# mpieva/network-aware-bwa

Hardware: AMD Instinct MI355X
Metric: aligned reads/s to GRCh38 (100 bp SE), FM-index search (bwa_cal_sa_reg_gap), bit-exact vs CPU (higher is better)
Workload: dtype u32

## Files before the change

include/nabwa.h:

```cpp
#ifndef NABWA_H
#define NABWA_H
#include <stdint.h>
#include <stddef.h>

#ifdef __cplusplus
extern "C" {
#endif

#define NABWA_OK        0
#define NABWA_ENODEV   -1
#define NABWA_EINVAL   -2
#define NABWA_EIO      -3
#define NABWA_ENOMEM   -4
#define NABWA_ECAP     -5
#define NABWA_EHITS    -6
#define NABWA_EDATA    -7

typedef struct {
	int s_mm, s_gapo, s_gape;
	int mode;
	int indel_end_skip, max_del_occ, max_entries;
	float fnr;
	int max_diff, max_gapo, max_gape;
	int max_seed_diff, seed_len;
	int n_threads;
	int max_top2;
	int trim_qual;
} nabwa_gap_opt_t;

#define NABWA_MODE_GAPE     0x01
#define NABWA_MODE_COMPREAD 0x02
#define NABWA_MODE_LOGGAP   0x04
#define NABWA_MODE_NONSTOP  0x10

typedef struct { uint32_t info; uint32_t k, l; int32_t score; } nabwa_aln1_t;

typedef struct nabwa_index nabwa_index_t;

const char *nabwa_last_error(void);
int nabwa_device_count(void);

void nabwa_gap_init_opt(nabwa_gap_opt_t *opt);
int nabwa_cal_maxdiff(int len, double err, double thres);

int nabwa_index_load(const char *prefix, int device, int with_sa, int with_pac, nabwa_index_t **out);

int nabwa_index_from_arrays(int device, int is_device, const uint32_t *bwt0, uint64_t n_words0,
							const uint32_t *bwt1, uint64_t n_words1, const uint32_t *sa0, uint64_t n_sa_words0,
							const uint32_t *sa1, uint64_t n_sa_words1, nabwa_index_t **out);
void nabwa_index_destroy(nabwa_index_t *ix);
uint32_t nabwa_index_seq_len(const nabwa_index_t *ix, int which);
uint64_t nabwa_index_device_bytes(const nabwa_index_t *ix);

int nabwa_cal_sa_reg_gap(nabwa_index_t *ix, const nabwa_gap_opt_t *opt, int n, const int64_t *off,
						 const uint8_t *seq, const uint8_t *rseq, int per_read,
						 int32_t *n_aln, nabwa_aln1_t *aln_out, int64_t aln_cap, int64_t *n_rows,
						 int32_t *max_entries);

typedef struct nabwa_batch nabwa_batch_t;
int nabwa_batch_create(nabwa_index_t *ix, const nabwa_gap_opt_t *opt, int n, const int64_t *off,
					   const uint8_t *seq, const uint8_t *rseq, int per_read, nabwa_batch_t **out);
int nabwa_batch_run(nabwa_batch_t *b);
int nabwa_batch_sync(nabwa_batch_t *b, int *n_second_pass);
float nabwa_batch_last_kernel_ms(nabwa_batch_t *b);
float nabwa_batch_last_width_ms(nabwa_batch_t *b);
float nabwa_batch_last_deep_ms(nabwa_batch_t *b);
int nabwa_batch_count_touches(nabwa_batch_t *b, uint64_t *n_bucket, uint64_t *n_bucket_width);
int nabwa_batch_fetch(nabwa_batch_t *b, int32_t *n_aln, nabwa_aln1_t *aln_out, int64_t aln_cap, int64_t *n_rows,
					  int32_t *max_entries);
int nabwa_batch_width_records(nabwa_batch_t *b, int first, int n, uint32_t *w_out, uint8_t *bid_out, uint8_t *seed_bid_out);
int nabwa_batch_checksum(nabwa_batch_t *b, uint64_t *sum, int64_t *n_rows);
typedef struct {
	int32_t n, min_len, max_len;
	int32_t deep_only;
	int32_t ns1, ns_wide;
	int32_t w_sync;
	int32_t trip_budget, trip_budget_hard;
	int32_t n_sync;
	int32_t hard_budget;
	int32_t cls[3];
	int32_t coop_lanes;
	int32_t lds_rd;
} nabwa_batch_config_t;
int nabwa_batch_config(nabwa_batch_t *b, nabwa_batch_config_t *out);
int nabwa_batch_sure0_stats(nabwa_batch_t *b, uint64_t out[4]);
int nabwa_batch_sure0_stats_ex(nabwa_batch_t *b, uint64_t out[8]);
int nabwa_batch_dedup_stats(nabwa_batch_t *b, uint64_t out[4]);
int nabwa_batch_dedup_stats_ex(nabwa_batch_t *b, uint64_t out[8]);
int nabwa_index_dedup_cache_stats(nabwa_index_t *ix, uint64_t out[8]);
int nabwa_index_dedup_cache_clear(nabwa_index_t *ix);
void nabwa_batch_destroy(nabwa_batch_t *b);

typedef struct { double avg, std, ap_prior; uint32_t low, high, high_bayesian; } nabwa_isize_t;
int nabwa_isize_infer(const uint16_t *hist, double ap_prior, int64_t L, nabwa_isize_t *out);
int nabwa_isize_bin(int kind, int mapq0, int mapq1, uint32_t pos0, int len0, uint32_t pos1, int len1);
typedef struct { uint32_t pos; int32_t strand, mapQ, seQ, len, full_len, n_mm, n_gapo, n_gape, score, extra_flag; } nabwa_pe_end_t;
int nabwa_pairing(nabwa_pe_end_t p[2], int n_hits, uint64_t *hits, const nabwa_aln1_t *rows0, const nabwa_aln1_t *rows1,
				  int max_isize, int s_mm, const nabwa_isize_t *ii);

typedef struct {
	char *name;
	uint8_t *seq, *rseq, *qual;
	uint32_t bits0, bits1;
	int32_t score, clip_len;
	int32_t n_aln; int32_t pad0;
	nabwa_aln1_t *aln;
	int32_t n_multi; int32_t pad1;
	void *multi;
	uint32_t sa, pos;
	uint64_t c1c2seq;
	int32_t n_cigar; int32_t pad2;
	uint16_t *cigar;
	int32_t tid;
	char bc[64];
	uint32_t lenbits;
	char *md;
	int32_t max_entries; int32_t pad3;
} nabwa_bwa_seq_t;

int nabwa_bwa_cal_sa_reg_gap(nabwa_index_t *ix, int n_seqs, nabwa_bwa_seq_t *seqs, const nabwa_gap_opt_t *opt);

int nabwa_encode_read(int full_len, const uint8_t *codes, const uint8_t *qual, int reverse, int trim_qual, int is_comp,
					  uint8_t *seq_out, uint8_t *rseq_out);

int nabwa_sa_lookup(nabwa_index_t *ix, int n, const uint8_t *which, const uint32_t *k, uint32_t *sa_out);

int nabwa_global_align(int device, int n, const int64_t *ref_off, const uint8_t *ref, const int64_t *qry_off,
					   const uint8_t *qry, int gap_open, int gap_ext, int gap_end, const int *matrix25, int band,
					   int32_t *score, int32_t *n_cigar, uint32_t *cigar32, int max_cigar);

void nabwa_dp_scratch_release(int device);

void nabwa_dp_form_counts(uint64_t *out, int n);

int nabwa_extend_align(int device, int n, const int64_t *ref_off, const uint8_t *ref, const int64_t *qry_off,
					   const uint8_t *qry, int gap_open, int gap_ext, const int *matrix25, int band, const int32_t *G0,
					   int32_t *score, int32_t *n_cigar, uint32_t *cigar32, int max_cigar);

int nabwa_local_align(int device, int n, const int64_t *ref_off, const uint8_t *ref, const int64_t *qry_off,
					  const uint8_t *qry, int gap_open, int gap_ext, const int *matrix25, int band, int thres,
					  int32_t *score, int32_t *coords, int32_t *subo, int32_t *n_cigar, uint32_t *cigar32, int max_cigar);

#define NABWA_MAX_CIGAR 64
#define NABWA_MAX_MD    512
#define NABWA_MAX_MULTI 16
typedef struct { uint32_t pos; int32_t gap, mm, strand, n_cigar; uint16_t cigar[NABWA_MAX_CIGAR]; } nabwa_multi_t;
typedef struct {
	int32_t type, strand, n_mm, n_gapo, n_gape, score;
	uint32_t sa, pos, c1, c2;
	int32_t mapQ, seQ, len, full_len, clip_len;
	int32_t n_cigar; uint16_t cigar[NABWA_MAX_CIGAR];
	int32_t nm; char md[NABWA_MAX_MD];
	int32_t n_multi; nabwa_multi_t multi[NABWA_MAX_MULTI];
	int32_t flag, seqid, nn; int64_t rpos; char xt;
} nabwa_se_t;

int nabwa_index_attach_reference(nabwa_index_t *ix, const char *prefix);
int nabwa_index_n_contigs(const nabwa_index_t *ix);
int nabwa_index_contig(const nabwa_index_t *ix, int i, char *name, int name_cap, int64_t *offset, int32_t *len);
int nabwa_index_reference_info(const nabwa_index_t *ix, int64_t *l_pac, uint32_t *seed);
int nabwa_index_set_reference(nabwa_index_t *ix, int64_t l_pac, uint32_t seed, int n_seqs, const char *const *names,
							  const int64_t *offsets, const int32_t *lens, int n_holes, const int64_t *hole_off,
							  const int32_t *hole_len, const char *hole_amb, const uint8_t *pac);

int nabwa_se_finish(nabwa_index_t *ix, const nabwa_gap_opt_t *opt, int n, const int64_t *off, const uint8_t *seq,
					const uint8_t *rseq, const int32_t *full_len, const int32_t *n_aln, const nabwa_aln1_t *aln,
					int n_occ, uint64_t *rng48, nabwa_se_t *out);

int nabwa_se_posn(nabwa_index_t *ix, const nabwa_gap_opt_t *opt, int n, const int64_t *off, const int32_t *full_len,
				  const int32_t *n_aln, const nabwa_aln1_t *aln, int n_occ, uint64_t *rng48, nabwa_se_t *out);
int nabwa_se_refine(nabwa_index_t *ix, int n, const int64_t *off, const uint8_t *seq, const uint8_t *rseq, nabwa_se_t *inout);
int nabwa_se_posn_v(nabwa_index_t *ix, const nabwa_gap_opt_t *opt, int n, const int64_t *off, const int32_t *full_len,
					const int32_t *n_aln, const nabwa_aln1_t *aln, const uint8_t *n_occ_v, uint64_t *rng48, nabwa_se_t *out);

int nabwa_refine_gapped_core(nabwa_index_t *ix, int which_ref, int is_end_correct, int n, const int64_t *qry_off, const uint8_t *qry,
                             const int32_t *ext, uint32_t *pos, int32_t *n_cigar, uint16_t *cigar, int max_cigar);
int nabwa_cal_md(nabwa_index_t *ix, int which_ref, int n, const int64_t *qry_off, const uint8_t *qry, const uint32_t *pos,
                 const int32_t *n_cigar, const uint16_t *cigar, int max_cigar, int32_t *nm, int64_t *md_off, char *md, int64_t md_cap);
void nabwa_finish_counts(uint64_t out[4]);

typedef struct {
	int32_t max_isize, force_isize, max_occ, max_occ_se, n_multi, N_multi, type, is_sw, is_preload;
	double ap_prior;
} nabwa_pe_opt_t;
void nabwa_pe_opt_default(nabwa_pe_opt_t *po);

typedef struct {
	nabwa_se_t se;
	int32_t extra_flag, m_seqid, am;
	int32_t mapQ_paired;
	int64_t m_rpos, isize;
} nabwa_pe_t;

int nabwa_pe_posn(nabwa_index_t *ix, const nabwa_gap_opt_t *opt, int n_pairs, const int64_t *off, const int32_t *full_len,
				  const int32_t *n_aln, const nabwa_aln1_t *aln, uint64_t *rng48, nabwa_pe_t *out);

int nabwa_isize_add_pairs(int n_pairs, const nabwa_pe_t *recs, uint16_t *hist);
int nabwa_pe_finish(nabwa_index_t *ix, const nabwa_gap_opt_t *opt, const nabwa_pe_opt_t *popt, const nabwa_isize_t *ii,
					int n_pairs, const int64_t *off, const uint8_t *seq, const uint8_t *rseq, const int32_t *n_aln,
					const nabwa_aln1_t *aln, nabwa_pe_t *inout, uint64_t n_tot[2], uint64_t n_mapped[2]);
typedef struct nabwa_poscache nabwa_poscache_t;
nabwa_poscache_t *nabwa_poscache_create(void);
void nabwa_poscache_destroy(nabwa_poscache_t *c);
int64_t nabwa_poscache_size(const nabwa_poscache_t *c);
int nabwa_pe_finish_cached(nabwa_index_t *ix, const nabwa_gap_opt_t *opt, const nabwa_pe_opt_t *popt, const nabwa_isize_t *ii,
						   int n_pairs, const int64_t *off, const uint8_t *seq, const uint8_t *rseq, const int32_t *n_aln,
						   const nabwa_aln1_t *aln, nabwa_pe_t *inout, uint64_t n_tot[2], uint64_t n_mapped[2], nabwa_poscache_t *cache);

int nabwa_bwa_posn_se(nabwa_index_t *ix, const nabwa_gap_opt_t *opt, int max_occ_se, int n, nabwa_bwa_seq_t *seqs, uint64_t *rng48);
int nabwa_bwa_refine_gapped(nabwa_index_t *ix, int n, nabwa_bwa_seq_t *seqs);
int nabwa_bwa_posn_pe(nabwa_index_t *ix, const nabwa_gap_opt_t *opt, int n_pairs, nabwa_bwa_seq_t *seqs, uint64_t *rng48);
int nabwa_bwa_finish_pe(nabwa_index_t *ix, const nabwa_gap_opt_t *opt, const nabwa_pe_opt_t *popt, const nabwa_isize_t *ii,
						int n_pairs, nabwa_bwa_seq_t *seqs, uint64_t n_tot[2], uint64_t n_mapped[2]);
int nabwa_bwa_finish_pe_cached(nabwa_index_t *ix, const nabwa_gap_opt_t *opt, const nabwa_pe_opt_t *popt, const nabwa_isize_t *ii,
							   int n_pairs, nabwa_bwa_seq_t *seqs, uint64_t n_tot[2], uint64_t n_mapped[2], nabwa_poscache_t *cache);

typedef struct nabwa_isize_table nabwa_isize_table_t;
typedef struct nabwa_bam_batch nabwa_bam_batch_t;
nabwa_isize_table_t *nabwa_isize_table_create(double ap_prior, int64_t genome_len);
void nabwa_isize_table_destroy(nabwa_isize_table_t *t);
int nabwa_isize_table_infer_all(nabwa_isize_table_t *t);
int nabwa_isize_table_get(const nabwa_isize_table_t *t, const char *rg, nabwa_isize_t *out);
int nabwa_isize_table_merge(nabwa_isize_table_t *t, const nabwa_isize_table_t *other);
int64_t nabwa_isize_table_encode(const nabwa_isize_table_t *t, uint8_t *out, int64_t cap);
int nabwa_isize_table_decode(nabwa_isize_table_t *t, const uint8_t *in, int64_t n);
int nabwa_bam_batch_create(nabwa_index_t *ix, const nabwa_gap_opt_t *opt, const nabwa_pe_opt_t *popt, int n_rec,
						   const uint8_t *in, const int64_t *in_off, nabwa_bam_batch_t **out);
#define NABWA_BAM_BROKEN_INPUT    1u
#define NABWA_BAM_DROP_ALIGNED    2u
#define NABWA_BAM_SKIP_DUPLICATES 4u
#define NABWA_BAM_DEBUG           8u
#define NABWA_BAM_ONLY_ALIGNED    16u
#define NABWA_BAM_ALL_FLAGS       31u
int nabwa_bam_batch_create_ex(nabwa_index_t *ix, const nabwa_gap_opt_t *opt, const nabwa_pe_opt_t *popt, uint32_t flags, int n_rec,
							  const uint8_t *in, const int64_t *in_off, nabwa_bam_batch_t **out);
int nabwa_bam_batch_search(nabwa_bam_batch_t *b);
int nabwa_bam_batch_pass1(nabwa_bam_batch_t *b, uint64_t *rng48, nabwa_isize_table_t *tab);
int nabwa_bam_batch_pass2(nabwa_bam_batch_t *b, const nabwa_isize_table_t *tab, uint64_t n_tot[2], uint64_t n_mapped[2]);
int nabwa_bam_batch_output(const nabwa_bam_batch_t *b, uint8_t *out, int64_t cap, int64_t *out_off, int64_t *n_bytes);
int nabwa_bam_batch_counts(const nabwa_bam_batch_t *b, int *n_records, int *n_logical);
int nabwa_bam_batch_kinds(const nabwa_bam_batch_t *b, uint8_t *kind_out);
void nabwa_bam_batch_destroy(nabwa_bam_batch_t *b);

#define NABWA_KIND_EOF 0
#define NABWA_KIND_SINGLE 1
#define NABWA_KIND_PAIR 2
#define NABWA_PHASE_PRISTINE 0
#define NABWA_PHASE_ALIGNED 1
#define NABWA_PHASE_POSITIONED 2
#define NABWA_PHASE_FINISHED 3
typedef struct {
	uint8_t core[32];
	int32_t data_len; const uint8_t *data;
	uint8_t strand, type, n_mm, n_gapo, n_gape, seQ, mapQ;
	int32_t len, clip_len, score; uint32_t sa, c1, c2, pos;
	int32_t n_multi; const uint8_t *multi;
	int32_t max_entries, n_aln; const uint8_t *aln;
} nabwa_wire_read_t;
typedef struct { uint64_t recno; uint8_t kind, phase; nabwa_wire_read_t read[2]; } nabwa_wire_rec_t;
int64_t nabwa_wire_size(const nabwa_wire_rec_t *r);
int64_t nabwa_wire_encode(const nabwa_wire_rec_t *r, uint8_t *out, int64_t cap);
int nabwa_wire_decode(const uint8_t *msg, int64_t len, nabwa_wire_rec_t *out);
void nabwa_wire_core_from_bam(const uint8_t bam_core[32], uint8_t wire_core[32]);
void nabwa_wire_core_to_bam(const uint8_t wire_core[32], uint8_t bam_core[32]);
int64_t nabwa_wire_config_encode(const nabwa_gap_opt_t *opt, const nabwa_pe_opt_t *popt, const char *prefix, uint8_t *out, int64_t cap);
int nabwa_wire_config_decode(const uint8_t *msg, int64_t len, nabwa_gap_opt_t *opt, nabwa_pe_opt_t *popt, char *prefix, int prefix_cap);

int nabwa_bam_batch_positioned(nabwa_bam_batch_t *b, nabwa_wire_read_t *out);
int nabwa_bam_batch_restore(nabwa_bam_batch_t *b, const nabwa_wire_read_t *in);

typedef struct nabwa_worker nabwa_worker_t;
int nabwa_worker_create(nabwa_index_t *ix, const nabwa_gap_opt_t *opt, const nabwa_pe_opt_t *popt, nabwa_worker_t **out);
void nabwa_worker_destroy(nabwa_worker_t *w);
int nabwa_worker_set_isize(nabwa_worker_t *w, const uint8_t *blob, int64_t n);
typedef int (*nabwa_send_fn)(void *ctx, const uint8_t *msg, int64_t len);
typedef int (*nabwa_recv_fn)(void *ctx, const uint8_t **msg, int64_t *len, int timeout_ms);
int nabwa_worker_process(nabwa_worker_t *w, int n_msg, const uint8_t *const *msgs, const int64_t *lens, nabwa_send_fn send, void *ctx);
typedef struct { int32_t max_batch, linger_ms, idle_timeout_ms; } nabwa_worker_opt_t;
int nabwa_worker_core(nabwa_worker_t *w, nabwa_recv_fn recv, nabwa_send_fn send, void *ctx, const nabwa_worker_opt_t *wo);
void nabwa_worker_counts(const nabwa_worker_t *w, uint64_t out[4]);

int nabwa_index_export(const nabwa_index_t *ix, int which, int what, uint64_t first, uint64_t n, uint32_t *out);

int nabwa_occ4(nabwa_index_t *ix, int which, int n, const uint32_t *k, uint32_t *cnt_out );

int64_t nabwa_index_fa2pac(const char *fasta, const char *prefix);
int64_t nabwa_index_fa2cspac(const char *fasta, const char *prefix);
int nabwa_index_build(const char *prefix, int device, int sa_intv, int verbose);
int nabwa_index_build_estimate(uint64_t l_pac, uint64_t *bytes);

#define NABWA_ISIZE_FEW   1
#define NABWA_ISIZE_WEIRD 2
int nabwa_isize_infer_pairs(int n_pairs, const uint32_t *pos, const int32_t *len, const int32_t *mapq, double ap_prior, int64_t L,
							nabwa_isize_t *out, char *log, int log_cap);
int nabwa_pe_finish_sampe(nabwa_index_t *ix, const nabwa_gap_opt_t *opt, const nabwa_pe_opt_t *popt, const nabwa_isize_t *ii,
						  int n_pairs, const int64_t *off, const uint8_t *seq, const uint8_t *rseq, const int32_t *n_aln,
						  const nabwa_aln1_t *aln, nabwa_pe_t *inout, nabwa_poscache_t *cache, int *cnt_chg, uint64_t n_tot[2],
						  uint64_t n_mapped[2]);
int nabwa_index_pac2real(const nabwa_index_t *ix, int64_t pos, int len, int *seqid);

#define NABWA_CS2NT_MAX 1024
int nabwa_cs2nt(int device, int n, const int64_t *off, const uint8_t *nt_ref, const uint8_t *cs_read, uint8_t *out);
int nabwa_index_attach_nt_reference(nabwa_index_t *ix, const char *prefix);
int nabwa_se_finish_cs(nabwa_index_t *ix, const nabwa_gap_opt_t *opt, int n, const int64_t *off, const uint8_t *seq, const uint8_t *rseq,
					   const uint8_t *qual, const int32_t *full_len, const int32_t *n_aln, const nabwa_aln1_t *aln, int n_occ,
					   uint64_t *rng48, nabwa_se_t *out, uint8_t *nt_seq, uint8_t *nt_rseq, uint8_t *nt_qual, double *times);
int nabwa_pe_finish_sampe_cs(nabwa_index_t *ix, const nabwa_gap_opt_t *opt, const nabwa_pe_opt_t *popt, const nabwa_isize_t *ii,
							 int n_pairs, const int64_t *off, const uint8_t *seq, const uint8_t *rseq, const uint8_t *qual,
							 const int32_t *n_aln, const nabwa_aln1_t *aln, nabwa_pe_t *inout, nabwa_poscache_t *cache, int *cnt_chg,
							 uint8_t *nt_seq, uint8_t *nt_rseq, uint8_t *nt_qual, double *times);
int nabwa_pairing_typed(nabwa_pe_end_t p[2], int n_hits, uint64_t *hits, const nabwa_aln1_t *rows0, const nabwa_aln1_t *rows1,
						int max_isize, int s_mm, const nabwa_isize_t *ii, int type);

typedef struct nabwa_bgzf nabwa_bgzf_t;
int nabwa_bgzf_inflated_size(const uint8_t *in, int64_t n, int64_t *n_out, int64_t *n_blocks);
int nabwa_bgzf_decompress(int device, const uint8_t *in, int64_t n, uint8_t *out, int64_t cap, int64_t *n_out, int64_t *n_blocks);
int nabwa_bgzf_handle_decompress(nabwa_bgzf_t *z, const uint8_t *in, int64_t n, uint8_t *out, int64_t cap, int64_t *n_out, int64_t *n_blocks);
int64_t nabwa_bgzf_bound(int64_t n);
int nabwa_bgzf_compress(int device, const uint8_t *in, int64_t n, uint8_t *out, int64_t cap, int64_t *n_out, int64_t *n_blocks);
int nabwa_bgzf_create(int device, nabwa_bgzf_t **out);
int nabwa_bgzf_handle_compress(nabwa_bgzf_t *z, const uint8_t *in, int64_t n, uint8_t *out, int64_t cap, int64_t *n_out, int64_t *n_blocks);
void nabwa_bgzf_destroy(nabwa_bgzf_t *z);
#define NABWA_BGZF_CODES_FIXED    0
#define NABWA_BGZF_CODES_DYNAMIC  1
int nabwa_bgzf_compress_ex(int device, int codes, const uint8_t *in, int64_t n, uint8_t *out, int64_t cap, int64_t *n_out, int64_t *n_blocks);
int nabwa_bgzf_handle_compress_ex(nabwa_bgzf_t *z, int codes, const uint8_t *in, int64_t n, uint8_t *out, int64_t cap, int64_t *n_out, int64_t *n_blocks);

#define NABWA_BAM_SORT_KEY(tid, pos) (((uint64_t)(uint32_t)(tid) << 32) | (uint32_t)((pos) + 1))
typedef struct nabwa_bam_sort nabwa_bam_sort_t;
int nabwa_bam_sort_create(int device, nabwa_bam_sort_t **out);
void nabwa_bam_sort_destroy(nabwa_bam_sort_t *s);
int nabwa_bam_sort_run(nabwa_bam_sort_t *s, int64_t n_rec, const uint8_t *in, const int64_t *in_off, uint8_t *out, int64_t cap, int64_t *out_off, uint64_t *keys_out);
int nabwa_bam_sort(int device, int64_t n_rec, const uint8_t *in, const int64_t *in_off, uint8_t *out, int64_t cap, int64_t *out_off, uint64_t *keys_out);
int nabwa_bam_sort_times(const nabwa_bam_sort_t *s, float ms[6]);

#define NABWA_DAMAGE_LEN_BINS 1024
#define NABWA_DAMAGE_MAX_POS  256
enum { NABWA_DAMAGE_STAT_SEEN = 0, NABWA_DAMAGE_STAT_COUNTED, NABWA_DAMAGE_STAT_SKIPPED_FLAGS, NABWA_DAMAGE_STAT_SKIPPED_PLACE,
	   NABWA_DAMAGE_STAT_SKIPPED_MAPQ, NABWA_DAMAGE_STAT_SKIPPED_EMPTY, NABWA_DAMAGE_STAT_COLUMNS_COUNTED,
	   NABWA_DAMAGE_STAT_COLUMNS_SKIPPED_READ, NABWA_DAMAGE_STAT_COLUMNS_SKIPPED_REF, NABWA_DAMAGE_N_STATS };
typedef struct { int32_t n_pos; int32_t min_mapq; uint32_t exclude_flags; uint32_t require_flags; int32_t which_ref; int32_t pad; } nabwa_damage_opt_t;
typedef struct nabwa_damage nabwa_damage_t;
void nabwa_damage_default_opt(nabwa_damage_opt_t *o);
int nabwa_damage_create(nabwa_index_t *ix, const nabwa_damage_opt_t *opt, nabwa_damage_t **out);
int nabwa_damage_add(nabwa_damage_t *d, int64_t n_rec, const uint8_t *in, const int64_t *in_off);
int nabwa_damage_fetch(nabwa_damage_t *d, uint64_t *sub5, uint64_t *sub3, uint64_t *len_hist, uint64_t *stats);
int nabwa_damage_clear(nabwa_damage_t *d);
void nabwa_damage_destroy(nabwa_damage_t *d);
int nabwa_damage_times(const nabwa_damage_t *d, float ms[3]);

int nabwa_bam_sort_run_ex(nabwa_bam_sort_t *s, int64_t n_rec, const uint8_t *in, const int64_t *in_off, uint8_t *out, int64_t cap, int64_t *out_off, uint64_t *keys_out, uint32_t *perm_out);
int nabwa_bam_sort_ex(int device, int64_t n_rec, const uint8_t *in, const int64_t *in_off, uint8_t *out, int64_t cap, int64_t *out_off, uint64_t *keys_out, uint32_t *perm_out);

#define NABWA_MARKDUP_ENDS_5P   0
#define NABWA_MARKDUP_ENDS_BOTH 1
enum { NABWA_MARKDUP_STAT_SEEN = 0, NABWA_MARKDUP_STAT_SKIPPED_FLAGS, NABWA_MARKDUP_STAT_ALREADY, NABWA_MARKDUP_STAT_UNMAPPED,
	   NABWA_MARKDUP_STAT_FRAGMENTS, NABWA_MARKDUP_STAT_PAIRS, NABWA_MARKDUP_STAT_ORPHANS, NABWA_MARKDUP_STAT_DUP_FRAGMENTS,
	   NABWA_MARKDUP_STAT_DUP_PAIRS, NABWA_MARKDUP_STAT_DUP_RECORDS, NABWA_MARKDUP_N_STATS };
typedef struct { int32_t min_qual; int32_t single_ends; uint32_t exclude_flags; int32_t pad; } nabwa_markdup_opt_t;
typedef struct nabwa_markdup nabwa_markdup_t;
void nabwa_markdup_default_opt(nabwa_markdup_opt_t *o);
int nabwa_markdup_create(int device, const nabwa_markdup_opt_t *opt, nabwa_markdup_t **out);
int nabwa_markdup_add(nabwa_markdup_t *m, int64_t n_rec, const uint8_t *in, const int64_t *in_off);
int nabwa_markdup_resolve(nabwa_markdup_t *m, uint8_t *dup, int64_t cap, uint64_t *stats);
int nabwa_markdup_clear(nabwa_markdup_t *m);
void nabwa_markdup_destroy(nabwa_markdup_t *m);
int nabwa_markdup_times(const nabwa_markdup_t *m, float ms[5]);

enum { NABWA_BAI_STAT_RECORDS = 0, NABWA_BAI_STAT_PLACED, NABWA_BAI_STAT_NO_COOR, NABWA_BAI_STAT_BINS, NABWA_BAI_STAT_CHUNKS, NABWA_BAI_STAT_WINDOWS,
	   NABWA_BAI_STAT_BYTES, NABWA_BAI_N_STATS };
typedef struct nabwa_bai nabwa_bai_t;
int nabwa_bai_create(int device, int32_t n_ref, nabwa_bai_t **out);
int nabwa_bai_add(nabwa_bai_t *b, int64_t n_rec, const uint8_t *in, const int64_t *in_off, int64_t stream_off);
int nabwa_bai_finish(nabwa_bai_t *b, int64_t n_blk, const int64_t *blk_uoff, const int64_t *blk_coff, uint8_t *out, int64_t cap, int64_t *n_out, uint64_t *stats);
int nabwa_bai_clear(nabwa_bai_t *b);
void nabwa_bai_destroy(nabwa_bai_t *b);
int nabwa_bai_times(const nabwa_bai_t *b, float ms[7]);
int nabwa_bgzf_block_table(const uint8_t *in, int64_t n, int64_t *blk_uoff, int64_t *blk_coff, int64_t cap, int64_t *n_blk);

#ifdef __cplusplus
}
#endif
#endif
```

network-aware-bwa_amd/csrc/fm_search.hip:

```cpp
#include "nabwa_dev.hpp"
#include "fm_search.hpp"
#include "launchers.hpp"

#define STATE_M 0
#define STATE_I 1
#define STATE_D 2
#define STATE_GROUP 3
#define GRP_EXT 0x100u
#define TXM 0xfffffffeu
#define KEYM 0xffffffffu
#define LVO(t_) ((size_t)((((uint64_t)1 << (2 * (t_))) - 4ull) / 3ull))
#ifndef NABWA_W_WAVES
#define NABWA_W_WAVES 5
#endif
#ifndef NABWA_WORK_CHUNK
#define NABWA_WORK_CHUNK 64u
#endif
#ifndef NABWA_RUN_MAX
#define NABWA_RUN_MAX 4
#endif

__device__ __forceinline__ uint32_t byte_of(uint64_t lo, uint64_t hi, uint32_t idx)
{
	asm volatile("" : "+v"(lo), "+v"(hi));
	const uint64_t h = (idx & 8u) ? hi : lo;
	return (uint32_t)(h >> ((idx & 7u) << 3)) & 0xffu;
}
#define WIN_SET(lo_, hi_, a_, b_, c_, d_) do { lo_ = (uint64_t)(b_) << 32 | (a_); hi_ = (uint64_t)(d_) << 32 | (c_); } while (0)

__device__ __forceinline__ void set_word(uint4 &q, uint32_t c, uint32_t v)
{
	q.x = c == 0 ? v : q.x; q.y = c == 1 ? v : q.y; q.z = c == 2 ? v : q.z; q.w = c == 3 ? v : q.w;
}

extern __shared__ uint16_t s_head[];

#ifndef NABWA_MIN_WAVES
#define NABWA_MIN_WAVES 4
#endif

template <bool COUNT>
__global__ __launch_bounds__(NABWA_SEARCH_BLOCK, NABWA_W_WAVES) void fm_width_kernel(const SearchParams P)
{
	const uint32_t lane = threadIdx.x & 63u;
	bool run = false, done = false;
	unsigned int w_next = 0, w_end = 0;
	uint32_t rid = 0, x = 0; int len = 0, phase = 0, wi = 0, n = 0, sbase = 0, nN = 0;
	uint32_t sq_off = 0;
#define WREC (P.wdata + (size_t)rid * P.wstride)
#define BX(f_) (x ? P.bwt[1].f_ : P.bwt[0].f_)
	bool tmode = false; uint32_t tp = 0, twtag = 0xffffffffu; uint2 twin = make_uint2(0u, 0u);
	const bool text_ok = (P.text_mode & 1) && P.bwt[0].sa_full && P.bwt[1].sa_full;
	uint32_t kk = 0, ll = 0, pw = 0; int bid = 0;
	uint32_t wkey = 0xffffffffu; bool tok = false; int tbase = 0;
	const int KT = (int)P.bwt[0].kmer_T, LW = (int)P.bwt[0].kmer_LW;
	__shared__ uint32_t s_pk[2 * NABWA_PK_LEVELS];
	const bool quads = (P.text_mode & TM_W_QUADS) && P.ixtab;
	if (threadIdx.x < 2 * NABWA_PK_LEVELS) s_pk[threadIdx.x] = quads ? P.ixtab[NABWA_IXTAB_WORDS + threadIdx.x] : 0xffffffffu;
	__syncthreads();
	bool nflag = true;
	auto rekey = [&](int from) {
		tok = false; tbase = from;
		if (nflag || from + 4 >= n) return;
		const int PW = P.pack_stride / 2;
		const uint32_t *const pk = P.rd_pack + (size_t)rid * P.pack_stride + x * PW;
		const int q = sbase + from;
		const uint32_t w0 = pk[q >> 4], w1 = pk[(q >> 4) + 1], sh = ((uint32_t)q & 15u) << 1;
		const uint32_t k16 = sh ? (w0 << sh) | (w1 >> (32u - sh)) : w0;
		wkey = k16 >> (2 * (16 - KT)); tok = true;
	};
	uint4 wacc = make_uint4(0, 0, 0, 0); uint64_t blo = 0, bhi = 0, slo = 0, shi = 0; int stag = -1;
	unsigned long long touches = 0;

	for (;;) {
		unsigned long long need = __ballot(!run && !done);
		if (P.w_sync && __ballot(run) != 0ull) need = 0ull;
		if (need) {
			if (w_next == w_end) {
				unsigned int base = 0;
				if (lane == 0) base = atomicAdd(P.work_counter + WC_WIDTH, (unsigned int)NABWA_WORK_CHUNK);
				w_next = __builtin_amdgcn_readfirstlane(base); w_end = w_next + NABWA_WORK_CHUNK;
			}
			const unsigned int rank = (unsigned int)__popcll(need & ((1ull << lane) - 1ull)), avail = w_end - w_next;
			const unsigned int base = w_next;
			w_next += min((unsigned int)__popcll(need), avail);
			if (!run && !done && rank < avail) {
				const unsigned int idx = base + rank;
				if (idx < 2u * (unsigned int)P.n) {
					rid = P.ids ? (uint32_t)P.ids[idx >> 1] : idx >> 1; x = idx & 1u;
					const int64_t o = P.poff[rid];
					len = P.rd_len[rid];
					sq_off = (uint32_t)o;
					nN = 0; stag = -1;
					if (P.w_skip_clean && P.n_aln[rid] == 0) {  }
					else if (len > 0) {
						run = true; phase = 0; wi = 0; n = len; sbase = 0; tmode = false;
						if (KT) { wkey = P.rd_key[6 * (size_t)rid + 2 + x]; tok = wkey != 0xffffffffu; }
						nflag = !KT || !P.rd_pack || P.rd_pack[(size_t)rid * P.pack_stride + (x + 1u) * (uint32_t)(P.pack_stride / 2) - 1u] != 0u;
						tbase = 0;
						kk = 0; ll = BX(seq_len); bid = 0; pw = 0; blo = bhi = 0;
					} else { if (x == 0u) P.rd_nN[rid] = 0; if (P.rd_cls) P.rd_cls[2 * (size_t)rid + x] = 0; }
				} else done = true;
			}
		}
		if (__ballot(!done) == 0ull) break;
		auto out_pos = [&](int p, bool last) {
			uint8_t *const rec = WREC;
			if (last) ++bid;
			const uint32_t wv = last ? 0u : ll - kk + 1u;
			const uint32_t bv = (uint32_t)(bid > 127 ? 127 : bid) | ((p > 0 && wv == pw) ? 128u : 0u);
			set_word(wacc, (uint32_t)p & 3u, wv);
			{ const uint64_t sh = (uint64_t)bv << (((uint32_t)p & 7u) << 3); if (p & 8) bhi |= sh; else blo |= sh; }
			pw = wv;
			if (phase == 0 && ((p & 3) == 3 || last)) *(uint4*)((uint32_t*)rec + x * P.WL + (p & ~3)) = wacc;
			if ((p & 15) == 15 || last) {
				*(uint4*)(rec + (phase ? P.woff_sbid + x * P.SLB : P.woff_bid + x * P.WLB) + (p & ~15)) =
					make_uint4((uint32_t)blo, (uint32_t)(blo >> 32), (uint32_t)bhi, (uint32_t)(bhi >> 32));
				blo = bhi = 0;
			}
		};
		bool bulk = run && phase == 0 && tmode && (wi & 15) == 0 && wi + 16 < n && tp >= 16u && pw == 1u;
		if (bulk) {
			if ((wi >> 4) != stag) { const uint4 q = *(const uint4*)((x ? P.rseq : P.seq) + sq_off + wi); WIN_SET(slo, shi, q.x, q.y, q.z, q.w); stag = wi >> 4; }
			const uint32_t w0 = (tp - 16u) >> 4;
			const uint32_t *const txt = BX(text);
			const uint32_t t0 = txt[w0], t1 = txt[w0 + 1u];
			auto squeeze = [](uint64_t v) -> uint32_t {
				uint64_t y = v & 0x0303030303030303ull;
				y = (y | y >> 6) & 0x000F000F000F000Full; y = (y | y >> 12) & 0x000000FF000000FFull; y = (y | y >> 24) & 0xFFFFull;
				return (uint32_t)y;
			};
			const bool clean = ((slo | shi) & 0xFCFCFCFCFCFCFCFCull) == 0ull;
			const uint32_t rd = squeeze(slo) | squeeze(shi) << 16;
			const uint32_t tx = (uint32_t)(((uint64_t)t1 << 32 | t0) >> (((tp - 16u) & 15u) << 1));
			uint32_t rv = __brev(tx); rv = (rv >> 1 & 0x55555555u) | (rv & 0x55555555u) << 1;
			bulk = clean && rv == rd;
			if (bulk) {
				uint8_t *const rec = WREC;
				uint32_t *const wp = (uint32_t*)rec + x * P.WL + wi;
#pragma unroll
				for (int u = 0; u < 4; ++u) *(uint4*)(wp + 4 * u) = make_uint4(1u, 1u, 1u, 1u);
				const uint32_t b4 = ((uint32_t)(bid > 127 ? 127 : bid) | 128u) * 0x01010101u;
				*(uint4*)(rec + P.woff_bid + x * P.WLB + wi) = make_uint4(b4, b4, b4, b4);
				tp -= 16u; wi += 16;
			}
		}
		if (bulk) {  }
		else if (run && tok && wi - tbase + 4 <= LW && wi + 4 < n) {
			uint2 tv[4];
			const uint2 *const lo = BX(kmer_lo);
			const int t1 = wi - tbase + 1;
			if (quads) {
				uint4 qd[2][2];
#pragma unroll
				for (int h = 0; h < 2; ++h) {
					const int t = t1 + 2 * h;
					const uint4 *const p = (const uint4*)(lo + LVO(t + 1) + 4 * (size_t)(wkey >> (2 * (KT - t))));
					qd[h][0] = p[0]; qd[h][1] = p[1];
				}
#pragma unroll
				for (int h = 0; h < 2; ++h) {
					const int t = t1 + 2 * h;
					const uint32_t ch = wkey >> (2 * (KT - t - 1)), c = ch & 3u;
					const uint4 a = qd[h][0], b = qd[h][1];
					const uint32_t sum = (a.y - a.x) + (a.w - a.z) + (b.y - b.x) + (b.w - b.z) + 4u + ((ch >> 2) == s_pk[x * NABWA_PK_LEVELS + t] ? 1u : 0u);
					tv[2 * h] = make_uint2(1u, sum);
					tv[2 * h + 1] = c == 0u ? make_uint2(a.x, a.y) : (c == 1u ? make_uint2(a.z, a.w) : (c == 2u ? make_uint2(b.x, b.y) : make_uint2(b.z, b.w)));
				}
			} else {
#pragma unroll
				for (int u = 0; u < 4; ++u) {
					const int t = t1 + u;
					tv[u] = (lo + LVO(t))[wkey >> (2 * (KT - t))];
				}
			}
#pragma unroll
			for (int u = 0; u < 4; ++u) {
				kk = tv[u].x; ll = tv[u].y;
				const bool dead = kk > ll;
				if (dead) { kk = 0; ll = BX(seq_len); ++bid; }
				out_pos(wi, false);
				++wi;
				if (dead) { rekey(wi); break; }
			}
		} else if (run) {
			const int pos = sbase + wi;
			if ((pos >> 4) != stag) { const uint4 q = *(const uint4*)((x ? P.rseq : P.seq) + sq_off + (pos & ~15)); WIN_SET(slo, shi, q.x, q.y, q.z, q.w); stag = pos >> 4; }
			const int cc = (int)byte_of(slo, shi, (uint32_t)pos & 15u);
			uint4 qa[4], qb[4]; uint32_t rk = 0, rl = 0, sav = 0; bool kval = false, two = false;
#pragma unroll
			for (int u = 0; u < 4; ++u) { qa[u] = make_uint4(0, 0, 0, 0); qb[u] = make_uint4(0, 0, 0, 0); }
			const bool q = cc < 4 && !tmode;
			if (q) {
				const uint32_t primary = BX(primary), kq = kk - 1u, lq = ll;
				const uint32_t kp = kq - (kq >= primary ? 1u : 0u), lp = lq - (lq >= primary ? 1u : 0u);
				const uint32_t bl = lp / NABWA_INTV; rl = lp - bl * NABWA_INTV;
				kval = kq != 0xffffffffu;
				const uint32_t bkk = kval ? kp / NABWA_INTV : bl; rk = kp - bkk * NABWA_INTV;
				two = bkk != bl;
				const uint4 *const bkt = BX(bk);
				const uint4 *pl = bkt + (size_t)bl * 4, *pk = bkt + (size_t)bkk * 4;
#pragma unroll
				for (int u = 0; u < 4; ++u) qa[u] = pl[u];
				if (two) {
#pragma unroll
					for (int u = 0; u < 4; ++u) qb[u] = pk[u];
				}
				if (COUNT) touches += ref_touches(x ? P.bwt[1] : P.bwt[0], kq, lq, false);
				if (text_ok && kk == ll) sav = BX(sa_full)[kk];
			}
			if (tmode && tp > 0u && ((tp - 1u) >> 5) != twtag) {
				twtag = (tp - 1u) >> 5;
				twin = *(const uint2*)(BX(text) + 2 * (size_t)twtag);
			}
			if (tmode) {
				bool ok = cc < 4 && tp > 0u;
				if (ok) {
					const uint32_t t = tp - 1u, wd = (t & 16u) ? twin.y : twin.x;
					ok = (wd >> ((t & 15u) << 1) & 3u) == (uint32_t)cc;
					if (ok) tp = t;
				}
				if (cc > 3 && x == 0u && phase == 0) ++nN;
				if (!ok) { tmode = false; kk = 0; ll = BX(seq_len); ++bid; rekey(wi + 1); }
			} else {
				const bool was_one = text_ok && cc < 4 && kk == ll;
				if (cc < 4) {
					Occ4 ck, cl;
					ck.c[0] = ck.c[1] = ck.c[2] = ck.c[3] = 0;
					cl = nabwa_count4(qa[0], qa[1], qa[2], qa[3], rl);
					if (kval) {
						const uint4 s0 = two ? qb[0] : qa[0], s1 = two ? qb[1] : qa[1], s2 = two ? qb[2] : qa[2], s3 = two ? qb[3] : qa[3];
						ck = nabwa_count4(s0, s1, s2, s3, rk);
					}
					const uint32_t L2c = cc == 0 ? BX(L2[0]) : (cc == 1 ? BX(L2[1]) : (cc == 2 ? BX(L2[2]) : BX(L2[3])));
					const uint32_t ok = cc == 0 ? ck.c[0] : (cc == 1 ? ck.c[1] : (cc == 2 ? ck.c[2] : ck.c[3]));
					const uint32_t ol = cc == 0 ? cl.c[0] : (cc == 1 ? cl.c[1] : (cc == 2 ? cl.c[2] : cl.c[3]));
					kk = L2c + ok + 1u; ll = L2c + ol;
				} else if (x == 0u && phase == 0) ++nN;
				if (kk > ll || cc > 3) { kk = 0; ll = BX(seq_len); ++bid; rekey(wi + 1); }
				else if (was_one) { tmode = true; tp = sav - 1u; twtag = 0xffffffffu; }
			}
			out_pos(wi, false);
			if (wi + 1 == n) out_pos(wi + 1, true);
			++wi;
			if (wi == n) {
				if (phase == 0 && P.rd_cls) P.rd_cls[2 * (size_t)rid + x] = (uint8_t)(bid - 1 > 4 ? 4 : bid - 1);
				if (phase == 0 && len > P.seed_len) {
					phase = 1; wi = 0; n = P.seed_len; sbase = len - P.seed_len; tmode = false;
					if (KT) { wkey = P.rd_key[6 * (size_t)rid + 4 + x]; tok = wkey != 0xffffffffu; }
					tbase = 0;
					kk = 0; ll = BX(seq_len); bid = 0; pw = 0;
				} else { if (x == 0u) P.rd_nN[rid] = (uint8_t)(nN > 255 ? 255 : nN); run = false; }
			}
		}
	}
	if (COUNT) {
		for (int o = 32; o > 0; o >>= 1) touches += __shfl_down(touches, o);
		if (lane == 0 && P.touch_counter) atomicAdd(P.touch_counter + TS_TOUCH_W, touches);
	}
#undef WREC
#undef BX
}
enum {
	LS_IDLE  = 0,
	LS_POP   = 1,
	LS_HAVE  = 2,
	LS_EXACT = 3,
	LS_EXIT  = 4
};
enum {
	TK_NONE      = 0,
	TK_EXPAND    = 1,
	TK_TAIL      = 2,
	TK_HIT       = 3,
	TK_JUMP      = 4,
	TK_GROUP     = 5,
	TK_ROWS      = 6,
	TK_TEXT_TAIL = 7
};

template <bool COUNT>
__global__ __launch_bounds__(NABWA_SEARCH_BLOCK, NABWA_MIN_WAVES) void fm_search_kernel(const SearchParams P_)
{
	SearchParams P = P_;
	own(P.n); own(P.s_mm); own(P.s_gapo); own(P.s_gape); own(P.mode); own(P.indel_end_skip); own(P.max_del_occ); own(P.max_entries);
	own(P.max_gape); own(P.max_seed_diff); own(P.seed_len); own(P.max_top2);
	const uint32_t NIL = 0xffffu;
	const uint32_t lane = threadIdx.x & 63u;
	const size_t slot = (size_t)blockIdx.x * NABWA_SEARCH_BLOCK + threadIdx.x;
	uint8_t *const sc = P.scratch + slot * P.lane_stride;
	uint4 *const ent = (uint4*)sc;
	const bool gape_mode = P.mode & 0x01, nonstop = P.mode & 0x10, loggap = P.mode & 0x04;

	int st = LS_IDLE;
	unsigned int w_next = 0, w_end = 0; bool w_sync = false;
	uint32_t item = 0; int len = 0; uint32_t mdmg = 0;
	uint32_t sq_off = 0;
	const int KT = (int)P.bwt[0].kmer_T;
	uint32_t budget = P.trip_budget;
	if (!COUNT && P.n_sync && P.trip_budget_hard && 2u * (uint32_t)__builtin_amdgcn_readfirstlane((int)*P.n_sync) > (uint32_t)P.n) budget = P.trip_budget_hard;
#define RID item
#define REC (P.wdata + (size_t)RID * P.wstride)
#define MD_READ ((int)(mdmg & 0xffu))
#define MG_READ ((int)(mdmg >> 8 & 0xfu))
	uint32_t k = 0, l = 0;
	int max_diff = 0, best_score = 0, best_cnt = 0, n_aln = 0, max_ent = 0, n_entries = 0;
	uint32_t bump = 0; uint64_t mask_lo = 0; bool seeded = false; int status = 0;
	int e_i = 0, e_a = 0, e_mm = 0, e_go = 0, e_ge = 0, e_state = 0, e_ldp = 0, e_score = 0, m = 0;
	uint4 pe = make_uint4(0, 0, 0, 0); int p_score = -1;
#define p_valid (p_score >= 0)
	int sq_tag = -1;
	int bw_base = -1, bw_a = -1;
	int sw_base = -1, sw_a = -1;
	unsigned long long touches = 0; uint32_t rd_touch = 0, rd_trips = 0;
	uint32_t rk_kf = 0, rk_row2 = 0, rk_row1 = 0, rk_tx = 0, rk_pop = 0, rk_tail = 0, rk_jump = 0, rk_gap = 0;
	unsigned long long st_trips = 0, st_expand = 0, st_exact = 0, st_ent = 0, st_spec = 0, st_query = 0, st_two = 0, st_exit = 0, st_jump = 0, st_txe = 0, st_txt = 0;
	bool ovf = false;
#define s0f mdmg
#define S0_ON  0x80000000u
#define S0_LAND 0x40000000u
#define S0_WAS 0x8000u
#define S0_PRV 0x1000u

	auto head_get = [&](int score) -> uint32_t {
		return (uint32_t)s_head[score * NABWA_SEARCH_BLOCK + threadIdx.x];
	};
	auto head_set = [&](int score, uint32_t v) {
		s_head[score * NABWA_SEARCH_BLOCK + threadIdx.x] = (uint16_t)v;
	};
	auto mask_has = [&](int score) -> bool { return mask_lo >> score & 1ull; };
	auto mask_set = [&](int score) { mask_lo |= 1ull << score; };
	auto mask_clr = [&](int score) { mask_lo &= ~(1ull << score); };
	auto mask_any = [&]() -> bool { return mask_lo != 0ull; };
	auto mask_first = [&]() -> int {
		return mask_lo ? __ffsll((unsigned long long)mask_lo) - 1 : 0x7fffffff;
	};
	auto never_popped = [&](int score) -> bool { return !nonstop && score > best_score + P.s_mm; };
	auto mk_entry = [&](uint32_t nk, uint32_t nl, int ni, int nldp, int nmm, int ngo, int nge, int nstate, int na) -> uint4 {
		const uint32_t z = (uint32_t)ni | (uint32_t)nldp << 16;
		return make_uint4(nk, nl, z, (uint32_t)nmm << 16 | (uint32_t)ngo << 20 | (uint32_t)nge << 24 | (uint32_t)nstate << 29 | (uint32_t)na << 31);
	};
	auto push_mem = [&](int score, uint4 e) {
		if (ovf || never_popped(score)) return;
		if ((uint32_t)score >= P.NS) { ovf = true; return; }
		if (bump >= P.cap) { ovf = true; return; }
		const uint32_t s = bump++;
		const uint32_t prev = mask_has(score) ? head_get(score) : NIL;
		e.w |= prev;
		ent[s] = e;
		head_set(score, s);
		mask_set(score);
	};

	uint4 *const s_pf = (uint4*)(s_head + (size_t)P.NS * NABWA_SEARCH_BLOCK);
	uint2 *const s_key = (uint2*)(s_pf + NABWA_SEARCH_BLOCK);
	uint2 *const s_tw = s_key + NABWA_SEARCH_BLOCK;
	uint32_t *const s_bw = (uint32_t*)(s_tw + NABWA_SEARCH_BLOCK), *const s_sw = s_bw + 4 * NABWA_SEARCH_BLOCK, *const s_sq = s_sw + 4 * NABWA_SEARCH_BLOCK;
	uint32_t *const s_fb = s_sq + 4 * NABWA_SEARCH_BLOCK;
	auto win_byte = [&](const uint32_t *W, uint32_t idx) -> uint32_t {
		return (uint32_t)((const uint8_t*)W)[(threadIdx.x << 4) + idx];
	};
	auto win_load = [&](const void *src, uint32_t *W) {
		__builtin_amdgcn_global_load_lds((const void __attribute__((address_space(1)))*)src,
										 (void __attribute__((address_space(3)))*)(W + ((threadIdx.x & ~63u) << 2)), 16, 0, 0);
	};
#define BW_BYTE(i_) win_byte(s_bw, (uint32_t)(i_))
#define SW_BYTE(i_) win_byte(s_sw, (uint32_t)(i_))
#define SQ_BYTE(i_) win_byte(s_sq, (uint32_t)(i_))
	const bool kf_ok = KT > 0 && (int)P.bwt[0].kmer_LW == KT && (int)P.bwt[1].kmer_LW == KT && (P.text_mode & 4);
	const bool text_ok = (P.text_mode & 2) && P.bwt[0].sa_full && P.bwt[1].sa_full && P.bwt[0].seq_len < 0xfffffff0u;
	uint32_t pf_slot = NIL;
	bool finish = false;
	auto unpack = [&](const uint4 &r) {
		k = r.x; l = r.y; e_i = (int)(r.z & 0xffffu); e_ldp = (int)(r.z >> 16);
		e_mm = (int)(r.w >> 16 & 15u); e_go = (int)(r.w >> 20 & 15u); e_ge = (int)(r.w >> 24 & 31u);
		e_state = (int)(r.w >> 29 & 3u); e_a = (int)(r.w >> 31);
	};
	auto take_entry = [&](const uint4 &r_ent) {
		unpack(r_ent);
		const uint32_t nx = r_ent.w & 0xffffu;
		head_set(e_score, nx);
		if (nx == NIL) mask_clr(e_score);
		--n_entries;
		if (!nonstop && e_score > best_score + P.s_mm) finish = true;
	};

	for (;;) {
		finish = false;
		unsigned long long need = __ballot(st == LS_IDLE);
		const bool any_busy = __ballot(st != LS_IDLE && st != LS_EXIT) != 0ull;
		if ((P.sync_refill || w_sync) && any_busy) need = 0ull;
		if (need) {
			if (w_next == w_end) {
				unsigned int b0 = 0;
				if (lane == 0) b0 = atomicAdd(P.work_counter + WC_SEARCH, (unsigned int)NABWA_WORK_CHUNK);
				w_next = __builtin_amdgcn_readfirstlane(b0); w_end = w_next + NABWA_WORK_CHUNK;
				w_sync = P.n_sync && (w_next >= *P.n_sync || w_next < P.n_sync[NCLS_SIZE + 2 - NCLS_FIRST0]);
			}
			const unsigned int rank = (unsigned int)__popcll(need & ((1ull << lane) - 1ull)), avail = w_end - w_next;
			const unsigned int base = w_next;
			w_next += min((unsigned int)__popcll(need), avail);
			if (st == LS_IDLE && rank < avail) {
				const unsigned int idx = base + rank;
				if (idx < (unsigned int)P.n) {
					const uint32_t rid = P.ids ? (uint32_t)P.ids[idx] : idx;
					item = rid;
					const int64_t o = P.poff[rid];
					len = P.rd_len[rid];
					sq_off = (uint32_t)o;
					mdmg = (uint32_t)P.rd_maxdiff[rid] | (uint32_t)P.rd_maxgapo[rid] << 8;
					if (KT) {
						s_key[threadIdx.x] = *(const uint2*)(P.rd_key + 6 * (size_t)rid);
						uint32_t fb = 0xffffu;
						if (len > KT) { const uint8_t *const bb = REC + P.woff_bid + (len - KT - 1); fb = (uint32_t)(bb[0] & 127u) | (uint32_t)(bb[P.WLB] & 127u) << 8; }
						s_fb[threadIdx.x] = fb;
					}
					n_aln = 0; max_ent = 0; status = NABWA_ST_OK; rd_touch = 0; rd_trips = 0; ovf = false;
					rk_kf = rk_row2 = rk_row1 = rk_tx = rk_pop = rk_tail = rk_jump = rk_gap = 0;
					sq_tag = -1; bw_a = -1; sw_a = -1; p_score = -1; pf_slot = NIL;
					if (text_ok) s_tw[threadIdx.x] = make_uint2(0u, 0x7fffffffu);
					if (!COUNT && P.sure0 && P.rd_cls && !nonstop && P.s_gapo > P.s_mm && MD_READ >= 1 && len > 0 && 2 + 4 * len <= P.max_entries) {
						const uint32_t cw = *(const uint16_t*)(P.rd_cls + 2 * (size_t)rid);
						if ((cw & 0xffu) == 0u || (cw >> 8) == 0u) {
							s0f |= P.sure0 > 1 ? S0_ON | S0_LAND | S0_WAS : S0_ON | S0_WAS;
							if (P.sure0 > 2) s0f |= ((cw & 0xffu) == 0u ? S0_PRV : 0u) | ((cw >> 8) == 0u ? S0_PRV << 1 : 0u);
						}
					}
					if (len > 0 && (int)P.rd_nN[rid] <= MD_READ) {
						seeded = len > P.seed_len;
						max_diff = MD_READ;
						best_score = (s0f & S0_ON) ? 0 : (MD_READ + 1) * P.s_mm + (MG_READ + 1) * P.s_gapo + (P.max_gape + 1) * P.s_gape;
						best_cnt = 0;
						bump = 0; mask_lo = 0ull;
						push_mem(0, mk_entry(0u, kf_ok ? KEYM : P.bwt[0].seq_len, len, 0, 0, 0, 0, STATE_M, 0));
						pe = mk_entry(0u, kf_ok ? KEYM : P.bwt[0].seq_len, len, 0, 0, 0, 0, STATE_M, 1); p_score = 0;
						n_entries = 2;
						st = LS_POP;
					} else { P.n_aln[item] = 0; P.max_ent[item] = 0; P.status[item] = NABWA_ST_OK; }
				} else st = LS_EXIT;
			}
		}
		if (__ballot(st != LS_EXIT) == 0ull) break;

		bool want_ent = false; uint32_t ent_slot = 0;
		bool have = st == LS_HAVE;
		if (st == LS_POP) {
			if (n_entries == 0) finish = true;
			else {
				if (max_ent < n_entries) max_ent = n_entries;
				if (n_entries > P.max_entries) finish = true;
				else if (!COUNT && P.trip_budget && rd_trips > budget) { status = NABWA_ST_OVERFLOW; finish = true; }
			}
			if (!finish) {
				const int best_mem = mask_first();
				if (p_valid && p_score <= best_mem) {
					unpack(pe);
					e_score = p_score; p_score = -1;
					--n_entries;
					if (!nonstop && e_score > best_score + P.s_mm) finish = true;
					else have = true;
				} else if (best_mem == 0x7fffffff) {
					finish = true;
				} else {
					if (p_valid) { push_mem(p_score, pe); p_score = -1; }
					if (ovf) { status = NABWA_ST_OVERFLOW; finish = true; }
					else {
						ent_slot = head_get(best_mem); e_score = best_mem;
						if (ent_slot == pf_slot) {
							const uint4 r = s_pf[threadIdx.x];
							take_entry(r);
							pf_slot = NIL;
							if (!finish) have = true;
						} else want_ent = true;
					}
				}
			}
		}
		int kind = TK_NONE;
		bool need_win = false, spec = false, forced = false; int win_hi = 0;
		int grp_c = 0, mlev = -1, mpost = 0; uint32_t midx = 0; bool kx = false;
		if (have && !finish && e_state == STATE_GROUP) {
			const uint32_t mk = (uint32_t)e_ldp & 0x1fu, ext = (uint32_t)e_ldp & GRP_EXT, more = (uint32_t)e_ldp >> 9;
			const int j = 31 - __clz((int)mk);
			const uint32_t rest = mk & ~(1u << j);
			if (rest) push_mem(e_score, mk_entry(k, l, e_i, (int)(rest | ext | more << 9), e_mm, e_go, e_ge, STATE_GROUP, e_a));
			else if (more) push_mem(e_score, mk_entry(k + 1u, l, e_i + 1, (int)(3u | (more - 1u) << 9), e_mm, e_go, e_ge, STATE_GROUP, e_a));
			if (ovf) { status = NABWA_ST_OVERFLOW; finish = true; }
			if (ext) ++e_ge; else ++e_go;
			if (l == KEYM) {
				const int dp = len - e_i - 1;
				kind = TK_ROWS; st = LS_POP; have = false;
				if (j == 0) { mpost = 1; mlev = dp; midx = k; } else { mpost = 2; mlev = dp + 1; midx = k * 4u + (uint32_t)(j - 1); }
			}
			else if (j == 0) { e_state = STATE_I; e_ldp = e_i; }
			else if (l == TXM) { k -= 1u; e_i += 1; e_state = STATE_D; e_ldp = e_i; }
			else { kind = TK_GROUP; grp_c = j - 1; st = LS_POP; have = false; }
		}
		if (have && !finish) {
			st = LS_POP;
			m = max_diff - (e_mm + e_go); if (gape_mode) m -= e_ge;
			if (m >= 0) {
				const bool kf = l == KEYM;
				const int d = len - e_i;
				if (e_i == 0) { if (kf) { kind = TK_ROWS; mlev = d; midx = k; } else kind = TK_HIT; }
				else {
					const bool tail = m == 0 && (e_state == STATE_M || gape_mode || e_ge == P.max_gape);
					const bool landed = e_state == STATE_M && e_ldp > e_i;
					win_hi = landed ? e_ldp - 1 : e_i - 1;
					const int win_lo = landed ? win_hi : ((tail || e_i < 2) ? e_i - 1 : e_i - 2);
					bool go = true;
					if (bw_a == e_a && win_lo >= bw_base && win_hi < bw_base + 16) {
						if (m < (int)(BW_BYTE(win_hi - bw_base) & 127u)) go = false;
					} else { need_win = true; spec = true; }
					if (go) {
						const bool rdkey_ok = KT && (e_a ? s_key[threadIdx.x].y : s_key[threadIdx.x].x) != 0xffffffffu;
						const bool row_known = l != TXM && !kf && (e_go | e_ge) == 0 && e_state == STATE_M && (e_mm == 0 || (e_mm == 1 && e_ldp == e_i));
						if (tail) {
							kind = TK_TAIL;
							if (l == TXM) kind = TK_TEXT_TAIL;
							else if (kf) { if (rdkey_ok) kind = TK_JUMP; else { kind = TK_ROWS; mlev = d; midx = k; } }
							else if (rdkey_ok && row_known && d <= KT) kind = TK_JUMP;
						}
						else {
							forced = rdkey_ok && d < KT && (kf || row_known) && (int)(s_fb[threadIdx.x] >> (e_a << 3) & 0xffu) == m;
							if (forced) kind = TK_JUMP;
							else if (kf && d >= KT) { kind = TK_ROWS; mlev = d; midx = k; }
							else if (l == TXM && (s0f & S0_ON) && (s0f & S0_PRV << e_a) && e_state == STATE_M && (e_mm | e_go | e_ge) == 0
									 && n_entries + 4 * len <= P.max_entries && k >= (uint32_t)e_i) {
								const int ies = P.indel_end_skip + (loggap ? 1 : 0);
								int hi = e_i - 1;
								if (hi > len - ies) hi = len - ies;
								if (seeded && P.max_seed_diff < 1 && hi > len - P.seed_len) hi = len - P.seed_len;
								const int gl = (MG_READ > 0 && hi >= ies) ? hi - ies + 1 : 0;
								if (P.s0_stats) { atomicAdd(P.s0_stats + S0S_LEAPS, 1ull); atomicAdd(P.s0_stats + S0S_LEAP_LEVELS, (unsigned long long)e_i); }
								n_entries += 2 * gl;
								if (max_ent < n_entries + 1) max_ent = n_entries + 1;
								k -= (uint32_t)e_i; e_i = 0; e_ldp = 0;
								kind = TK_HIT; need_win = false; spec = false;
							}
							else {
								if (P.s0_stats && l == TXM && (s0f & S0_ON) && (s0f & S0_PRV << e_a) && e_state == STATE_M && (e_mm | e_go | e_ge) == 0
									&& n_entries + 4 * len <= P.max_entries) atomicAdd(P.s0_stats + S0S_WALKED, 1ull);
								kind = TK_EXPAND; --e_i; kx = kf;
								if ((s0f & S0_ON) && n_entries + 4 * len > P.max_entries) s0f &= ~S0_ON;
							}
						}
					}
				}
			}
		} else if (st == LS_EXACT) kind = l == TXM ? TK_TEXT_TAIL : TK_TAIL;
		auto rows_arrived = [&](uint32_t nk, uint32_t nl) {
			k = nk; l = nl;
			if (mpost == 1) { e_state = STATE_I; e_ldp = e_i; }
			else if (mpost == 2) { e_i += 1; e_state = STATE_D; e_ldp = e_i; }
			st = LS_HAVE;
		};
		if (kind == TK_ROWS && mlev == 0) { rows_arrived(0u, e_a ? P.bwt[0].seq_len : P.bwt[1].seq_len); kind = TK_NONE; }

		const int qb = 1 - e_a;
		const bool tx = l == TXM && (kind == TK_EXPAND || kind == TK_HIT || kind == TK_TEXT_TAIL);
		const int spos = (kind == TK_TAIL || kind == TK_TEXT_TAIL) ? e_i - 1 : e_i;
		const int stag = (e_a << 20) | (spos >> 4);
		const bool need_seq = (kind == TK_EXPAND || kind == TK_TAIL || kind == TK_TEXT_TAIL) && stag != sq_tag;
		bool query = (kind == TK_EXPAND && !tx && !kx) || kind == TK_TAIL || kind == TK_GROUP;
		uint2 tw = make_uint2(0u, 0u); bool need_tw = false;
		if (tx && kind != TK_HIT && k > 0u) {
			const uint32_t tag = ((k - 1u) >> 4) | (uint32_t)qb << 31;
			tw = s_tw[threadIdx.x];
			need_tw = tw.y != tag;
			tw.y = tag;
		}
		const bool to_text = kind == TK_EXPAND && !tx && !kx && text_ok && k == l;
		if (kind == TK_TAIL && !need_seq && SQ_BYTE((uint32_t)spos & 15u) > 3u) query = false;
		const int ii = e_i - (len - P.seed_len);
		const bool use_seed = kind == TK_EXPAND && e_i > 0 && seeded && ii > 0;
		const bool need_seed = use_seed && !(sw_a == e_a && ii - 1 >= sw_base && ii < sw_base + 16);

		uint4 r_ent = make_uint4(0, 0, 0, 0);
		if (need_win) {
			int base = (win_hi | 7) - 15; if (base < 0) base = 0;
			win_load(REC + P.woff_bid + e_a * P.WLB + base, s_bw); bw_base = base; bw_a = e_a;
		}
		if (need_seq) {
			win_load((e_a ? P.rseq : P.seq) + sq_off + (spos & ~15), s_sq); sq_tag = stag;
		}
		if (need_seed) {
			int base = (ii | 7) - 15; if (base < 0) base = 0;
			win_load(REC + P.woff_sbid + e_a * P.SLB + base, s_sw); sw_base = base; sw_a = e_a;
		}
		uint32_t r_x = 0u;
		if (need_tw) r_x = (qb ? P.bwt[1].text : P.bwt[0].text)[(k - 1u) >> 4];
		else if (tx && kind == TK_HIT) r_x = (qb ? P.bwt[1].isa : P.bwt[0].isa)[k];
		else if (to_text) r_x = (qb ? P.bwt[1].sa_full : P.bwt[0].sa_full)[k];
		uint2 r_km = make_uint2(1u, 0u);
		uint4 a0, a1, a2, a3, b0, b1, b2, b3;
		a0 = a1 = a2 = a3 = b0 = b1 = b2 = b3 = make_uint4(0, 0, 0, 0);
		bool gh = kx && e_i > 0 && (s0f & S0_ON) && (e_mm | e_go | e_ge) == 0 && len - e_i < KT && !need_win && (BW_BYTE(e_i - 1 - bw_base) & 127u) == 0u;
		if (kind == TK_JUMP || gh) {
			uint32_t key = e_a ? s_key[threadIdx.x].y : s_key[threadIdx.x].x, key2 = 0, key3 = 0;
			const int d = len - e_i;
			if (gh) {
				if (key == 0xffffffffu) { gh = false; key = 0; }
				else {
					const uint32_t sh = 2u * (uint32_t)(KT - d), low = key & ((1u << sh) - 1u);
					const uint32_t gh_c = key >> sh & 3u;
					a3.x = 4u | gh_c;
					key = (k * 4u + ((gh_c + 1u) & 3u)) << sh | low; key2 = (k * 4u + ((gh_c + 2u) & 3u)) << sh | low; key3 = (k * 4u + ((gh_c + 3u) & 3u)) << sh | low;
				}
			} else if (l == KEYM) {
				if (d > 0) { const uint32_t sh = 2u * (uint32_t)(KT - d); key = (k << sh) | (sh ? key & ((1u << sh) - 1u) : 0u); }
			} else if (e_mm) {
				const uint32_t c1 = qb ? P.bwt[1].L2[1] : P.bwt[0].L2[1], c2 = qb ? P.bwt[1].L2[2] : P.bwt[0].L2[2], c3 = qb ? P.bwt[1].L2[3] : P.bwt[0].L2[3];
				const uint32_t cs = (k > c1 ? 1u : 0u) + (k > c2 ? 1u : 0u) + (k > c3 ? 1u : 0u);
				const uint32_t sh = 2u * (uint32_t)(KT - d);
				key = (key & ~(3u << sh)) | cs << sh;
			}
			const uint2 *const tab = qb ? P.bwt[1].kmer : P.bwt[0].kmer;
			r_km = tab[key];
			if (gh) { const uint2 g2 = tab[key2], g3 = tab[key3]; a2 = make_uint4(g2.x, g2.y, g3.x, g3.y); }
		}
		if (kind == TK_ROWS) r_km = ((qb ? P.bwt[1].kmer_lo : P.bwt[0].kmer_lo) + LVO(mlev))[midx];
		uint32_t rk = 0, rl = 0; bool kvalid = false, two = false;
		if (kx) {
			const uint4 *const ch = (const uint4*)((qb ? P.bwt[1].kmer_lo : P.bwt[0].kmer_lo) + LVO(len - e_i) + (size_t)k * 4);
			a0 = ch[0]; a1 = ch[1];
		}
		if (query) {
			const uint32_t primary = qb ? P.bwt[1].primary : P.bwt[0].primary;
			const uint4 *bk = qb ? P.bwt[1].bk : P.bwt[0].bk;
			const uint32_t kq = k - 1u, lq = l;
			const uint32_t kp = kq - (kq >= primary ? 1u : 0u), lp = lq - (lq >= primary ? 1u : 0u);
			const uint32_t bl = lp / NABWA_INTV; rl = lp - bl * NABWA_INTV;
			kvalid = kq != 0xffffffffu;
			const uint32_t bkk = kvalid ? kp / NABWA_INTV : bl; rk = kp - bkk * NABWA_INTV;
			two = bkk != bl;
			const uint4 *pl = bk + (size_t)bl * 4;
			a0 = pl[0]; a1 = pl[1]; a2 = pl[2]; a3 = pl[3];
			if (two) { const uint4 *pk = bk + (size_t)bkk * 4; b0 = pk[0]; b1 = pk[1]; b2 = pk[2]; b3 = pk[3]; }
		}

		bool pf_now = false; uint32_t pf_cand = NIL;
		if (want_ent) { pf_cand = ent_slot; pf_now = true; }
		else if ((kind == TK_TAIL || kind == TK_JUMP || kind == TK_TEXT_TAIL) && !p_valid && mask_any()) {
			const int bm = mask_first();
			pf_cand = head_get(bm);
			pf_now = pf_cand != pf_slot;
		}
		if (pf_now) r_ent = ent[pf_cand];
		if (!COUNT && P.trip_budget && st != LS_IDLE && st != LS_EXIT) ++rd_trips;
		if (COUNT && st != LS_IDLE && st != LS_EXIT) {
			++rd_trips;
			if (kind == TK_EXPAND) { if (kx) ++rk_kf; else if (tx) ++rk_tx; else if (two) ++rk_row2; else ++rk_row1; if (e_go | e_ge) ++rk_gap; }
			else if (want_ent) ++rk_pop; else if (kind == TK_TAIL || kind == TK_TEXT_TAIL) ++rk_tail; else if (kind == TK_JUMP) ++rk_jump;
		}
		if (COUNT) {
			const unsigned long long bx = __ballot(kind == TK_EXPAND), be = __ballot(kind == TK_TAIL), bm = __ballot(want_ent),
				bs = __ballot(spec), bq = __ballot(query), b2 = __ballot(query && two), bi = __ballot(st == LS_EXIT), bj = __ballot(kind == TK_JUMP), bt = __ballot(tx && kind == TK_EXPAND), b7 = __ballot(kind == TK_TEXT_TAIL);
			if (lane == 0) {
				st_trips += 1; st_expand += __popcll(bx); st_exact += __popcll(be); st_ent += __popcll(bm); st_spec += __popcll(bs);
				st_query += __popcll(bq); st_two += __popcll(b2); st_exit += __popcll(bi); st_jump += __popcll(bj); st_txe += __popcll(bt); st_txt += __popcll(b7);
			}
		}
		asm volatile("" ::: "memory");
		__builtin_amdgcn_s_waitcnt(0x0F70);
		if (pf_now) { s_pf[threadIdx.x] = r_ent; pf_slot = pf_cand; }
		if (spec && m < (int)(BW_BYTE(win_hi - bw_base) & 127u)) kind = TK_NONE;
		if (need_tw) { tw.x = r_x; s_tw[threadIdx.x] = tw; }
		int c = 4;
		if (kind == TK_EXPAND || kind == TK_TAIL) c = (int)SQ_BYTE((uint32_t)spos & 15u);
		if (kind == TK_TAIL && c > 3) query = false;
		Occ4 ck, cl;
		ck.c[0] = ck.c[1] = ck.c[2] = ck.c[3] = 0; cl = ck;
		if (query && kind != TK_NONE) {
			cl = nabwa_count4(a0, a1, a2, a3, rl);
			if (kvalid) {
				const uint4 s0 = two ? b0 : a0, s1 = two ? b1 : a1, s2 = two ? b2 : a2, s3 = two ? b3 : a3;
				ck = nabwa_count4(s0, s1, s2, s3, rk);
			}
			if (COUNT && kind != TK_GROUP) rd_touch += ref_touches(qb ? P.bwt[1] : P.bwt[0], k - 1u, l, kind == TK_EXPAND);
		}
		if (kx && kind == TK_EXPAND) {
			const uint32_t ek[4] = { a0.x, a0.z, a1.x, a1.z }, el[4] = { a0.y, a0.w, a1.y, a1.w };
#pragma unroll
			for (int j = 0; j < 4; ++j) { const bool ne = ek[j] <= el[j]; ck.c[j] = ne ? k * 4u + (uint32_t)j - 1u : 0u; cl.c[j] = ne ? KEYM : 0u; }
		}
		const bool tx1 = tx && kind == TK_EXPAND;
		if (tx1) {
			const uint32_t b = k > 0u ? (tw.x >> (((k - 1u) & 15u) << 1) & 3u) : 4u;
#pragma unroll
			for (int j = 0; j < 4; ++j) { ck.c[j] = b == (uint32_t)j ? k - 2u : 0u; cl.c[j] = b == (uint32_t)j ? TXM : 0u; }
		}
		const bool syn = tx1 || (kx && kind == TK_EXPAND);
		const uint32_t L2q0 = syn ? 0u : (qb ? P.bwt[1].L2[0] : P.bwt[0].L2[0]), L2q1 = syn ? 0u : (qb ? P.bwt[1].L2[1] : P.bwt[0].L2[1]);
		const uint32_t L2q2 = syn ? 0u : (qb ? P.bwt[1].L2[2] : P.bwt[0].L2[2]), L2q3 = syn ? 0u : (qb ? P.bwt[1].L2[3] : P.bwt[0].L2[3]);
		const uint32_t seqlen_q = qb ? P.bwt[1].seq_len : P.bwt[0].seq_len;
#define L2Q(cc) ((cc) == 0 ? L2q0 : ((cc) == 1 ? L2q1 : ((cc) == 2 ? L2q2 : L2q3)))
#define CK(cc) ((cc) == 0 ? ck.c[0] : ((cc) == 1 ? ck.c[1] : ((cc) == 2 ? ck.c[2] : ck.c[3])))
#define CL(cc) ((cc) == 0 ? cl.c[0] : ((cc) == 1 ? cl.c[1] : ((cc) == 2 ? cl.c[2] : cl.c[3])))

		if (kind == TK_ROWS) rows_arrived(r_km.x, r_km.y);
		else if (kind == TK_GROUP) {
			k = L2Q(grp_c) + CK(grp_c) + 1u; l = L2Q(grp_c) + CL(grp_c);
			e_i += 1; e_state = STATE_D; e_ldp = e_i;
			st = LS_HAVE;
		} else if (kind == TK_JUMP) {
			k = r_km.x; l = r_km.y;
			if (k > l) st = LS_POP;
			else if (forced) { e_i = len - KT; e_ldp = 0; st = LS_HAVE; }
			else { e_i = len - KT; st = LS_EXACT; }
		} else if (kind == TK_TEXT_TAIL) {
			uint32_t pp = k; bool fail = false;
			for (;;) {
				const uint32_t cc = SQ_BYTE((uint32_t)(e_i - 1) & 15u);
				if (cc > 3u || pp == 0u) { fail = true; break; }
				const uint32_t q = pp - 1u;
				if ((tw.x >> ((q & 15u) << 1) & 3u) != cc) { fail = true; break; }
				pp = q; --e_i;
				if (e_i == 0 || (e_i & 15) == 0 || (pp & 15u) == 0u) break;
			}
			k = pp;
			if (fail) st = LS_POP;
			else if (e_i == 0) st = LS_HAVE;
			else st = LS_EXACT;
		} else if (kind == TK_TAIL || kind == TK_HIT) {
			bool hit = false;
			if (kind == TK_HIT && tx) { k = r_x; l = r_x; }
			if (kind == TK_HIT) hit = true;
			else if (c > 3) st = LS_POP;
			else {
				k = L2Q(c) + CK(c) + 1u; l = L2Q(c) + CL(c);
				if (k > l) st = LS_POP;
				else if (--e_i == 0) hit = true;
				else st = LS_EXACT;
			}
			if (hit) {
				st = LS_POP;
				const int score = e_mm * P.s_mm + e_go * P.s_gapo + e_ge * P.s_gape;
				bool do_add = true;
				if (n_aln == 0) {
					if ((s0f & S0_ON) && score != 0) { status = NABWA_ST_OVERFLOW; finish = true; do_add = false; s0f &= ~S0_ON; if (P.s0_stats) atomicAdd(P.s0_stats + S0S_NET, 1ull); }
					best_score = score;
					const int best_diff = e_mm + e_go + (gape_mode ? e_ge : 0);
					if (!nonstop) max_diff = best_diff + 1 > MD_READ ? MD_READ : best_diff + 1;
				}
				if (score == best_score) best_cnt += (int)(l - k + 1u);
				else if (best_cnt > P.max_top2) { finish = true; do_add = false; }
				uint4 *const out = P.aln + (size_t)item * P.aln_cap;
				if (do_add && e_go) {
					for (int j = 0; j < n_aln; ++j) { const uint4 h = out[j]; if (h.y == k && h.z == l) { do_add = false; break; } }
				}
				if (do_add) {
					if (n_aln == P.aln_cap) { status = NABWA_ST_OVERFLOW; finish = true; }
					else {
						const uint32_t x = l - k + 1u, mx = seqlen_q; uint32_t jj = 0, pw = 0;
						uint8_t *const rec = REC;
						uint32_t *const wp = (uint32_t*)rec + e_a * P.WL; uint8_t *const bp = rec + P.woff_bid + e_a * P.WLB;
						for (int t0 = 0; t0 <= e_ldp && e_ldp > 0; t0 += 8) {
							const uint4 w0 = *(const uint4*)(wp + t0), w1 = *(const uint4*)(wp + t0 + 4);
							const uint2 bq = *(const uint2*)(bp + t0);
							uint32_t wv[8] = { w0.x, w0.y, w0.z, w0.w, w1.x, w1.y, w1.z, w1.w };
							uint32_t bb[2] = { bq.x, bq.y };
#pragma unroll
							for (int u = 0; u < 8; ++u) {
								const int t = t0 + u;
								uint32_t bv = bb[u >> 2] >> ((u & 3) * 8) & 0xffu;
								if (t < e_ldp) {
									if (wv[u] > x) wv[u] -= x;
									else if (wv[u] == x) { bv = (bv & 128u) | 1u; wv[u] = mx - (++jj); }
								}
								if (t <= e_ldp) {
									bv = (bv & 127u) | ((t > 0 && wv[u] == pw) ? 128u : 0u);
									bb[u >> 2] = (bb[u >> 2] & ~(0xffu << ((u & 3) * 8))) | bv << ((u & 3) * 8);
								}
								pw = wv[u];
							}
							*(uint4*)(wp + t0) = make_uint4(wv[0], wv[1], wv[2], wv[3]);
							*(uint4*)(wp + t0 + 4) = make_uint4(wv[4], wv[5], wv[6], wv[7]);
							*(uint2*)(bp + t0) = make_uint2(bb[0], bb[1]);
						}
						bw_a = -1;
						if (KT && e_ldp > len - KT - 1) s_fb[threadIdx.x] |= 0xffu << (e_a << 3);
						out[n_aln] = make_uint4((uint32_t)e_mm | (uint32_t)e_go << 8 | (uint32_t)e_ge << 16 | (uint32_t)e_a << 24,
												k, l, (uint32_t)score);
						++n_aln;
					}
				}
			}
		} else if (kind == TK_EXPAND) {
			const uint32_t occ = tx1 ? 1u : l - k + 1u;
			bool match_child = false;
			bool allow_diff = true, allow_M = true, mm_dead = false;
			if (e_i > 0) {
				const uint32_t B1 = BW_BYTE(e_i - 1 - bw_base), B0 = BW_BYTE(e_i - bw_base);
				const int b1 = (int)(B1 & 127u), b0v = (int)(B0 & 127u);
				mm_dead = (s0f & S0_ON) && b1 > 0;
				if (b1 > m - 1) allow_diff = false;
				else if (b1 == m - 1 && b0v == m - 1 && (B0 & 128u)) allow_M = false;
				if (use_seed) {
					const uint32_t S1 = SW_BYTE(ii - 1 - sw_base), S0 = SW_BYTE(ii - sw_base);
					const int s1 = (int)(S1 & 127u), s0 = (int)(S0 & 127u);
					const int m_seed = m - max_diff + P.max_seed_diff;
					if (s1 > m_seed - 1) allow_diff = false;
					else if (s1 == m_seed - 1 && s0 == m_seed - 1 && (S0 & 128u)) allow_M = false;
				}
			}
			auto emit = [&](int score, uint32_t nk, uint32_t nl, int ni, int nldp, int nmm, int ngo, int nge, int nstate, int count) {
				if (p_valid) push_mem(p_score, pe);
				pe = mk_entry(nk, nl, ni, nldp, nmm & 0xff, ngo & 0xff, nge & 0xff, nstate, e_a); p_score = score;
				n_entries += count;
			};
			const int sc0 = e_mm * P.s_mm + e_go * P.s_gapo + e_ge * P.s_gape;
			int tmp = e_go + e_ge;
			if (loggap) { const uint32_t v = (uint32_t)(e_ge + e_go); tmp = (v ? 31 - __clz((int)v) : 0) / 2 + 1; }
			bool ran = false;
			if (tx1 && e_state == STATE_M && n_entries + 64 <= P.max_entries) {
				const int ies = P.indel_end_skip + tmp, seed_lo = len - P.seed_len;
				const int m_seed = m - max_diff + P.max_seed_diff;
				int n = 0, icur = e_i, ilast = e_i; uint32_t pcur = k; bool grp_run = false;
				for (;;) {
					const uint32_t cc = SQ_BYTE((uint32_t)icur & 15u);
					if (cc > 3u || pcur == 0u) break;
					const uint32_t q = pcur - 1u;
					if ((tw.x >> ((q & 15u) << 1) & 3u) != cc) break;
					bool ad = true;
					const bool us = seeded && icur > 0 && icur - seed_lo > 0;
					if (icur > 0) {
						if ((int)(BW_BYTE(icur - 1 - bw_base) & 127u) > m - 1) ad = false;
						if (us && (int)(SW_BYTE(icur - seed_lo - 1 - sw_base) & 127u) > m_seed - 1) ad = false;
					}
					const bool g = ad && icur >= ies && len - icur >= ies && e_go < MG_READ;
					if (n == 0) grp_run = g; else if (g != grp_run) break;
					++n; pcur = q; ilast = icur;
					if (n == NABWA_RUN_MAX || icur == 0) break;
					if (m < (int)(BW_BYTE(icur - 1 - bw_base) & 127u)) break;
					if ((icur & 15) == 0 || (q & 15u) == 0u) break;
					if (icur - 1 > 0 && icur - 2 < bw_base) break;
					if (seeded && icur - 1 > 0 && icur - 1 - seed_lo > 0 && icur - 1 - seed_lo - 1 < sw_base) break;
					--icur;
				}
				if (n) {
					ran = true;
					if (grp_run) emit(sc0 + P.s_gapo, k - (uint32_t)(n - 1), TXM, ilast, (int)(3u | (uint32_t)(n - 1) << 9), e_mm, e_go, e_ge, STATE_GROUP, 2 * n);
					emit(sc0, pcur, TXM, ilast, 0, e_mm, e_go, e_ge, STATE_M, 1);
				}
			}
			if (ran) {  }
			else if (allow_diff && e_i >= P.indel_end_skip + tmp && len - e_i >= P.indel_end_skip + tmp) {
				uint32_t dm = 0;
#pragma unroll
				for (int j = 0; j < 4; ++j) { const uint32_t nk = L2Q(j) + CK(j) + 1u, nl = L2Q(j) + CL(j); if (nk <= nl) dm |= 2u << j; }
				if (e_state == STATE_M) {
					if (e_go < MG_READ) emit(sc0 + P.s_gapo, k, l, e_i, (int)(dm | 1u), e_mm, e_go, e_ge, STATE_GROUP, __popc(dm) + 1);
				} else if (e_state == STATE_I) {
					if (e_ge < P.max_gape) emit(sc0 + P.s_gape, k, l, e_i, e_i, e_mm, e_go, e_ge + 1, STATE_I, 1);
				} else if (e_ge < P.max_gape) {
					if ((e_ge + e_go < max_diff || occ < (uint32_t)P.max_del_occ) && dm)
						emit(sc0 + P.s_gape, k, l, e_i, (int)(dm | GRP_EXT), e_mm, e_go, e_ge, STATE_GROUP, __popc(dm));
				}
			}
			if (ran) {  }
			else if (allow_diff && allow_M) {
#pragma unroll
				for (int j = 1; j <= 4; ++j) {
					const int cc = (c + j) & 3; const bool is_mm = (j != 4 || c > 3);
					const uint32_t nk = L2Q(cc) + CK(cc) + 1u, nl = L2Q(cc) + CL(cc);
					if (nk <= nl) {
						uint32_t ek = nk, el = nl; int ei = e_i; bool dead = is_mm && mm_dead;
						if (kx && is_mm && !dead && a3.x == (4u | (uint32_t)c)) {
							const uint32_t gk = j == 1 ? r_km.x : (j == 2 ? a2.x : a2.z), gl = j == 1 ? r_km.y : (j == 2 ? a2.y : a2.w);
							if (gk > gl) { dead = true; s0f += 1u << 16; }
							else if (s0f & S0_LAND) {
								ek = gk; el = gl; ei = len - KT; s0f += 1u << 23;
							}
						}
						if (dead) ++n_entries;
						else emit(sc0 + (is_mm ? P.s_mm : 0), ek, el, ei, is_mm ? e_i : 0, e_mm + (is_mm ? 1 : 0), e_go, e_ge, STATE_M, 1);
						if (!is_mm) match_child = true;
					}
				}
			} else if (c < 4) {
				const uint32_t nk = L2Q(c) + CK(c) + 1u, nl = L2Q(c) + CL(c);
				if (nk <= nl) { emit(sc0, nk, nl, e_i, 0, e_mm, e_go, e_ge, STATE_M, 1); match_child = true; }
			}
			if (to_text && match_child) { pe.x = r_x - 1u; pe.y = TXM; }
			if (ovf) { status = NABWA_ST_OVERFLOW; finish = true; }
		}
#undef L2Q
#undef CK
#undef CL

		if (finish) {
			const bool net = (s0f & S0_ON) && status == NABWA_ST_OK && n_aln == 0;
			if (net) status = NABWA_ST_OVERFLOW;
			if (P.s0_stats && (s0f & S0_WAS)) atomicAdd(P.s0_stats + S0S_READS, 1ull);
			if (P.s0_stats && (s0f >> 16 & 0x3fffu)) {
				atomicAdd(P.s0_stats + S0S_KF_EMPTY, (unsigned long long)(s0f >> 16 & 0x7fu)); atomicAdd(P.s0_stats + S0S_KF_LANDED, (unsigned long long)(s0f >> 23 & 0x7fu));
			}
			if (P.s0_stats && net) atomicAdd(P.s0_stats + S0S_NET, 1ull);
			P.n_aln[item] = n_aln; P.max_ent[item] = (!COUNT && status == NABWA_ST_OVERFLOW) ? (int)rd_trips : max_ent; P.status[item] = (uint8_t)status;
			if (COUNT && status == NABWA_ST_OK) touches += rd_touch;
			if (COUNT && P.touch_counter && rd_trips > 8000u) {
				atomicAdd(P.touch_counter + TS_LONG_READS, 1ull); atomicAdd(P.touch_counter + TS_LONG_TRIPS, (unsigned long long)rd_trips); atomicAdd(P.touch_counter + TS_LONG_KF, (unsigned long long)rk_kf);
				atomicAdd(P.touch_counter + TS_LONG_ROW2, (unsigned long long)rk_row2); atomicAdd(P.touch_counter + TS_LONG_ROW1, (unsigned long long)rk_row1); atomicAdd(P.touch_counter + TS_LONG_TEXT, (unsigned long long)rk_tx);
				atomicAdd(P.touch_counter + TS_LONG_POP, (unsigned long long)rk_pop); atomicAdd(P.touch_counter + TS_LONG_TAIL, (unsigned long long)rk_tail); atomicAdd(P.touch_counter + TS_LONG_JUMP, (unsigned long long)rk_jump); atomicAdd(P.touch_counter + TS_LONG_GAP, (unsigned long long)rk_gap);
			}
			if (COUNT && P.touch_counter) { atomicMax(P.touch_counter + TS_MAX_TRIPS, (unsigned long long)rd_trips); if (rd_trips > 2000u) atomicAdd(P.touch_counter + TS_OVER_2000, 1ull); if (rd_trips > 500u) atomicAdd(P.touch_counter + TS_OVER_500, 1ull); }
			st = LS_IDLE;
		}
	}
	if (COUNT) {
		for (int o = 32; o > 0; o >>= 1) touches += __shfl_down(touches, o);
		if (lane == 0 && P.touch_counter) {
			atomicAdd(P.touch_counter + TS_TOUCH_S, touches);
			atomicAdd(P.touch_counter + TS_TRIPS, st_trips); atomicAdd(P.touch_counter + TS_EXPAND, st_expand); atomicAdd(P.touch_counter + TS_EXACT, st_exact);
			atomicAdd(P.touch_counter + TS_ENT_LOAD, st_ent); atomicAdd(P.touch_counter + TS_SPEC, st_spec); atomicAdd(P.touch_counter + TS_QUERY, st_query);
			atomicAdd(P.touch_counter + TS_TWO, st_two); atomicAdd(P.touch_counter + TS_EXITED, st_exit); atomicAdd(P.touch_counter + TS_JUMP, st_jump); atomicAdd(P.touch_counter + TS_TEXT_EXPAND, st_txe); atomicAdd(P.touch_counter + TS_TEXT_TAIL, st_txt);
		}
	}
}

#undef p_valid
#undef S0_ON
#undef S0_LAND
#undef S0_WAS
#undef S0_PRV
#undef s0f
#undef BW_BYTE
#undef SW_BYTE
#undef SQ_BYTE
#undef RID
#undef REC
#undef MD_READ
#undef MG_READ
extern "C" void nabwa_launch_fm_width(const SearchParams *P, int n_blocks, hipStream_t s)
{
	if (P->touch_counter) hipLaunchKernelGGL((fm_width_kernel<true>), dim3(n_blocks), dim3(NABWA_SEARCH_BLOCK), 0, s, *P);
	else hipLaunchKernelGGL((fm_width_kernel<false>), dim3(n_blocks), dim3(NABWA_SEARCH_BLOCK), 0, s, *P);
}

extern "C" int nabwa_width_occupancy(void)
{
	int nb = 0;
	return hipOccupancyMaxActiveBlocksPerMultiprocessor(&nb, fm_width_kernel<false>, NABWA_SEARCH_BLOCK, 0) == hipSuccess ? nb : 0;
}

extern "C" void nabwa_launch_fm_search(const SearchParams *P, int n_blocks, hipStream_t s)
{
	const size_t lds = (size_t)P->NS * NABWA_SEARCH_BLOCK * 2 + NABWA_SEARCH_BLOCK * 84;
	if (P->touch_counter) hipLaunchKernelGGL((fm_search_kernel<true>), dim3(n_blocks), dim3(NABWA_SEARCH_BLOCK), lds, s, *P);
	else hipLaunchKernelGGL((fm_search_kernel<false>), dim3(n_blocks), dim3(NABWA_SEARCH_BLOCK), lds, s, *P);
}

extern "C" int nabwa_search_occupancy(int ns)
{
	int nb = 0;
	hipError_t e = hipOccupancyMaxActiveBlocksPerMultiprocessor(&nb, fm_search_kernel<false>, NABWA_SEARCH_BLOCK,
																(size_t)ns * NABWA_SEARCH_BLOCK * 2 + NABWA_SEARCH_BLOCK * 84);
	return e == hipSuccess ? nb : 0;
}
```

network-aware-bwa_amd/csrc/fm_search.hpp:

```cpp
#pragma once
#include <stdint.h>
#include "nabwa_dev.hpp"
#include "search_slots.hpp"

#define NABWA_SEARCH_BLOCK 256
#define NABWA_ST_OK        0
#define NABWA_ST_OVERFLOW  1
#define NABWA_ST_WIDE      2
#define NABWA_ST_POOL      3
#define NABWA_ST_HITCAP    4
#define NABWA_ST_GROWN     5

#define TM_W_QUADS 8

struct SearchParams {
	DevBwt bwt[2];
	const uint8_t *seq, *rseq;
	const int64_t *poff;
	const int32_t *rd_len;
	const uint8_t *rd_maxdiff, *rd_maxgapo;
	const int32_t *ids;
	const int32_t *res_slot;
	int n;
	int s_mm, s_gapo, s_gape, mode, indel_end_skip, max_del_occ, max_entries, max_gape, max_seed_diff, seed_len, max_top2;
	uint8_t *wdata;
	size_t wstride;
	uint32_t woff_bid, woff_sbid;
	uint32_t WL, WLB, SLB;
	int text_mode;
	const uint32_t *rd_key;
	uint8_t *rd_nN;
	uint8_t *scratch;
	size_t lane_stride;
	uint32_t cap, NS;
	int32_t *n_aln, *max_ent;
	uint8_t *status;
	uint4 *aln;
	int aln_cap;
	unsigned int *work_counter;
	uint32_t trip_budget;
	uint32_t trip_budget_hard;
	int sync_refill;
	const uint32_t *rd_pack; int pack_stride;
	int w_sync;
	int w_skip_clean;
	uint8_t *rd_cls;
	const unsigned int *n_sync;
	unsigned long long *touch_counter;
	const uint32_t *ixtab;
	int sure0;
	unsigned long long *s0_stats;
};

#define NABWA_IXTAB_STRIDE 24
#define NABWA_IXTAB_WORDS  48
#define NABWA_PK_LEVELS    17
#define NABWA_IXTAB_ALL    (NABWA_IXTAB_WORDS + 2 * NABWA_PK_LEVELS)
#define IX_BK 0
#define IX_KMER 2
#define IX_KMER_LO 4
#define IX_TEXT 6
#define IX_ISA 8
#define IX_SA_FULL 10
#define IX_PRIMARY 12
#define IX_SEQ_LEN 13
#define IX_L2 13
static inline void nabwa_ixtab_fill(uint32_t *tab, const DevBwt *bwt )
{
	for (int q = 0; q < 2; ++q) {
		uint32_t *o = tab + NABWA_IXTAB_STRIDE * q;
		const uint64_t p[6] = { (uint64_t)(uintptr_t)bwt[q].bk, (uint64_t)(uintptr_t)bwt[q].kmer, (uint64_t)(uintptr_t)bwt[q].kmer_lo,
								(uint64_t)(uintptr_t)bwt[q].text, (uint64_t)(uintptr_t)bwt[q].isa, (uint64_t)(uintptr_t)bwt[q].sa_full };
		for (int f = 0; f < 6; ++f) { o[2 * f] = (uint32_t)p[f]; o[2 * f + 1] = (uint32_t)(p[f] >> 32); }
		o[IX_PRIMARY] = bwt[q].primary; o[IX_SEQ_LEN] = bwt[q].seq_len; o[IX_L2 + 1] = bwt[q].L2[1]; o[IX_L2 + 2] = bwt[q].L2[2]; o[IX_L2 + 3] = bwt[q].L2[3];
		for (int f = 17; f < NABWA_IXTAB_STRIDE; ++f) o[f] = 0;
	}
}
```

network-aware-bwa_amd/csrc/launchers.hpp:

```cpp
#pragma once
#include <hip/hip_runtime.h>
#include "fm_deep.hpp"

extern "C" {
void nabwa_launch_repack(const uint32_t *w, uint32_t seq_len, uint32_t n_buckets, uint4 *out, hipStream_t s);
void nabwa_launch_kmer_level(const DevBwt *B, const uint2 *prev, uint2 *cur, uint64_t n_cur, hipStream_t s);
void nabwa_launch_kmer_primary(const uint2 *lv, uint64_t n_keys, uint32_t primary, uint32_t *out, hipStream_t s);
void nabwa_launch_sa_fill(const DevBwt *B, uint32_t *sa_full, uint32_t *isa, uint8_t *text_bytes, hipStream_t s);
void nabwa_launch_text_pack(const uint8_t *bytes, uint32_t n, uint32_t n_words, uint32_t *out, hipStream_t s);
void nabwa_launch_sa_lookup(const DevBwt *B, int n, const uint8_t *which, const uint32_t *k, uint32_t *out, hipStream_t s);
void nabwa_launch_occ4(const DevBwt *B, int n, const uint32_t *k, uint32_t *out, hipStream_t s);
void nabwa_launch_fm_search(const SearchParams *P, int n_blocks, hipStream_t s);
void nabwa_launch_fm_width(const SearchParams *P, int n_blocks, hipStream_t s);
int nabwa_width_occupancy(void);
int nabwa_search_occupancy(int ns);
void nabwa_launch_checksum(int n, const int32_t *map, const uint32_t *cent, const uint8_t *arena, const int32_t *n_aln, const uint4 *aln, int aln_cap, const uint8_t *status,
						   const int32_t *wide_idx, const uint4 *aln2, int aln_cap2, const uint4 *const *grown,
						   unsigned long long *sum, unsigned long long *rows, hipStream_t s);
void nabwa_launch_collect(int n, const uint8_t *status, int32_t *ids, unsigned int *count, int which, hipStream_t s);
void nabwa_launch_collect_keyed(int n, const uint8_t *status, int32_t *ids, unsigned int *count, int which,
								const uint8_t *cls, const uint8_t *md, int max_key, const int32_t *n_aln, int aln_cap, hipStream_t s);
void nabwa_launch_assign_slots(int n2, const int32_t *ids, int32_t *wide_idx, hipStream_t s);
void nabwa_launch_scatter_grown(int n2, const int32_t *ids, const int32_t *n_aln3, const int32_t *max_ent3, const uint8_t *status3,
								 int32_t *n_aln, int32_t *max_ent, uint8_t *status, int32_t *wide_idx, const uint4 *block, size_t cap3,
								 const uint4 **grown, int slot0, hipStream_t s);
void nabwa_launch_scatter_wide(int n2, const int32_t *ids, const int32_t *n_aln2, const int32_t *max_ent2,
							   const uint8_t *status2, int32_t *n_aln, int32_t *max_ent, uint8_t *status,
							   int32_t *wide_idx, hipStream_t s);
void nabwa_launch_gather(int n, const int32_t *map, const uint32_t *cent, const uint8_t *arena, const int32_t *n_aln, const uint32_t *row_off, const uint4 *aln, int aln_cap,
						 const uint8_t *status, const int32_t *wide_idx, const uint4 *aln2, int aln_cap2,
						 const uint4 *const *grown, uint4 *out, hipStream_t s);
void nabwa_launch_partition(int n, const uint8_t *cls, int32_t *ids, unsigned int *cnt, hipStream_t s);
void nabwa_launch_padded_len(int n, const int64_t *off, int64_t *plen, hipStream_t s);
void nabwa_launch_pad_reads(int n, const uint8_t *seq, const uint8_t *rseq, const int64_t *off, const int64_t *poff,
							uint8_t *pseq, uint8_t *prseq, int32_t *rd_len, uint32_t *rd_key, int T, int seed_len, uint32_t *rd_pack, int pack_stride,
							const uint8_t *md_tab, const uint8_t *mg_tab, uint8_t *rd_md, uint8_t *rd_mg, hipStream_t s);
void nabwa_launch_dedup_hash(int n, const uint8_t *seq, const uint8_t *rseq, const int64_t *off, uint64_t mask, uint64_t *keys, uint32_t *ids, hipStream_t s);
void nabwa_launch_dedup_heads(int n, const uint64_t *keys, uint32_t *head, hipStream_t s);
void nabwa_launch_dedup_verify(int n, const uint8_t *seq, const uint8_t *rseq, const int64_t *off, const uint32_t *ids, const uint32_t *head,
							   int32_t *rep, uint32_t *flag, unsigned int *n_coll, hipStream_t s);
void nabwa_launch_dedup_map(int n, const int32_t *rep, const uint32_t *inner, const int64_t *off, int32_t *map, int64_t *clen, unsigned int *stat, hipStream_t s);
void nabwa_launch_dedup_compact(int n, const uint8_t *seq, const uint8_t *rseq, const int64_t *off, const int32_t *rep, const uint32_t *inner,
								const int64_t *coff, uint8_t *cseq, uint8_t *crseq, hipStream_t s);
void nabwa_launch_dedup_expand(int n, const int32_t *map, const int32_t *n_aln, const int32_t *max_ent, const uint32_t *cent, const uint8_t *arena,
							   int32_t *n_aln_out, int32_t *max_ent_out, hipStream_t s);
void nabwa_launch_dcache_lookup(int n, const uint8_t *seq, const uint8_t *rseq, const int64_t *off, const uint64_t *hash, const uint8_t *md_tab, const uint8_t *mg_tab,
								const unsigned long long *slots, uint32_t n_slots, uint64_t mask, const uint8_t *arena, uint32_t *found, uint32_t *flag, hipStream_t s);
void nabwa_launch_dcache_map(int n, const uint32_t *found, const uint32_t *inner, const int64_t *off, int32_t *rep, int32_t *newidx, int64_t *clen, uint32_t *cent,
							 unsigned int *stat, hipStream_t s);
void nabwa_launch_dcache_remap(int n, const int32_t *old, const int32_t *newidx, int32_t *map, hipStream_t s);
void nabwa_launch_dcache_insert(int n, const uint8_t *seq, const uint8_t *rseq, const int64_t *poff, const int32_t *len, const uint8_t *rd_md, const uint8_t *rd_mg,
								const uint8_t *status, const int32_t *n_aln, const int32_t *max_ent, const uint4 *aln, int aln_cap, const int32_t *wide_idx,
								const uint4 *aln2, int aln_cap2, const uint4 *const *grown, int row_cap, uint64_t mask,
								unsigned long long *slots, uint32_t n_slots, uint8_t *arena, uint64_t arena_bytes, unsigned long long *ctr, hipStream_t s);
void nabwa_launch_fm_deep(const DeepParams *P, int n_waves, hipStream_t s);
int nabwa_deep_occupancy(int ns, int lds_rd);
void nabwa_launch_bgzf_deflate(const uint8_t *in, int64_t n, int n_slices, uint8_t *stage, uint32_t *sizes, hipStream_t s);
void nabwa_launch_bgzf_deflate_dyn(const uint8_t *in, int64_t n, int n_slices, uint8_t *stage, uint32_t *sizes, hipStream_t s);
void nabwa_launch_bgzf_pack(const uint8_t *stage, const uint32_t *sizes, int n_slices, uint8_t *packed, int64_t *total, hipStream_t s);
struct BgzfInBlk;
void nabwa_launch_bgzf_inflate(const uint8_t *cmp, const struct BgzfInBlk *blk, int n_blk, uint8_t *plain, uint32_t *status, hipStream_t s);
struct FinRef; struct FinJob; struct FinRec;
void nabwa_launch_refine_window(const uint8_t *pac, const struct FinJob *jobs, int n, const uint8_t *reads0, const uint8_t *reads1, const int64_t *ro,
								const int64_t *qo, uint8_t *ref, uint8_t *qry, hipStream_t s);
void nabwa_launch_refine_cigar(const struct FinJob *jobs, int n, int end_correct, const int32_t *n_c32, const uint32_t *c32, int max_cigar,
							   uint32_t *pos_out, int32_t *n_cigar, uint16_t *rows, unsigned int *n_bad, hipStream_t s);
void nabwa_launch_md_count(const struct FinRef *R, const struct FinRec *recs, int n, const uint8_t *reads0, const uint8_t *reads1, const uint16_t *cigar,
						   int32_t *nm, int32_t *len_out, hipStream_t s);
void nabwa_launch_md_write(const struct FinRef *R, const struct FinRec *recs, int n, const uint8_t *reads0, const uint8_t *reads1, const uint16_t *cigar,
						   const int64_t *md_off, char *md, hipStream_t s);
struct DmgParams;
void nabwa_launch_damage(const struct DmgParams *P, int n_blocks, unsigned long long *call, unsigned int *bad, hipStream_t s);
void nabwa_launch_damage_add(int words, const unsigned long long *call, unsigned long long *total, hipStream_t s);
struct MdParams; struct MdArena;
void nabwa_launch_markdup_sig(const struct MdParams *P, int n_blocks, unsigned int *bad, hipStream_t s);
void nabwa_launch_markdup_emit(const struct MdParams *P, const struct MdArena *A, hipStream_t s);
void nabwa_launch_markdup_iota(int64_t n, uint32_t *idx, hipStream_t s);
void nabwa_launch_markdup_gather(int64_t n, const uint32_t *idx, const uint64_t *src, uint64_t *keys, hipStream_t s);
void nabwa_launch_markdup_mark(int64_t n, const uint32_t *idx, const uint64_t *hi, const uint64_t *lo, const uint64_t *k3, uint8_t *dup, unsigned long long *stats, hipStream_t s);
void nabwa_launch_markdup_prop(int64_t n, const uint8_t *link, uint8_t *dup, unsigned long long *stats, hipStream_t s);
struct BaiParams; struct BaiFin;
enum { NABWA_BAI_STEP_REF = 0, NABWA_BAI_STEP_HEAD, NABWA_BAI_STEP_PLACE, NABWA_BAI_STEP_REFSIZE, NABWA_BAI_STEP_LIN, NABWA_BAI_STEP_WRITE_REF,
	   NABWA_BAI_STEP_WRITE_TUPLE, NABWA_BAI_STEP_WRITE_LIN };
void nabwa_launch_bai_sig(const struct BaiParams *P, int n_blocks, hipStream_t s);
void nabwa_launch_bai_iota(int64_t n, uint32_t *idx, hipStream_t s);
void nabwa_launch_bai_step(int step, const struct BaiFin *F, hipStream_t s);
}
```

network-aware-bwa_amd/csrc/nabwa_batch.hip:

```cpp
#include <hip/hip_runtime.h>
#include <hipcub/hipcub.hpp>
#include <stdio.h>
#include <stdlib.h>
#include <string.h>
#include <memory>
#include <mutex>
#include <vector>
#include "../../include/nabwa.h"
#include "nabwa_batch.hpp"
#include "dedup_cache_body.hpp"
#include "host_util.hpp"

static void layout(SearchParams &P, uint32_t cap, int max_len, int seed_len, uint32_t NS)
{
	P.WL = align_up((uint32_t)max_len + 1, 16);
	P.WLB = P.WL + 16;
	P.SLB = align_up((uint32_t)(max_len > seed_len ? seed_len : 0) + 1, 16) + 16;
	P.woff_bid = 2 * P.WL * 4;
	P.woff_sbid = P.woff_bid + 2 * P.WLB;
	P.wstride = align_up(P.woff_sbid + 2 * P.SLB, 64);
	P.cap = cap; P.NS = NS;
	P.lane_stride = align_up((size_t)cap * 16, 64);
}

extern "C" void nabwa_batch_destroy(nabwa_batch_t *b)
{
	if (!b) return;
	(void)hipSetDevice(b->ix->device);
	if (b->stream) (void)hipStreamSynchronize(b->stream);
	if (b->cache_pinned) { std::lock_guard<std::mutex> lk(b->cache->mu); --b->cache->pins; }
	delete b;
}

namespace {
struct BatchShape {
	int max_len = 0, min_len = 65535; int64_t padded_total = 0;
	std::vector<uint8_t> md_tab, mg_tab;
	uint32_t NS = 1, NS1 = 1;
	bool deep_only = false;
};
}

static int derive_options(const nabwa_gap_opt_t *opt, int n, const int64_t *off, int per_read, BatchShape &s)
{
	bool bad_len = false;
	std::vector<uint8_t> seen(65536, 0);
	{
		const int NT = n >= (1 << 20) ? 4 : 1;
		struct Part { int mx = 0, mn = 65535; int64_t padded = 0; bool bad = false; std::vector<uint8_t> seen; };
		std::vector<Part> part(NT);
		for (Part &q : part) q.seen.assign(65536, 0);
		host_parallel(NT, (size_t)n, [&](int t, size_t i0, size_t i1) {
			Part &q = part[t];
			for (size_t i = i0; i < i1; ++i) {
				const int64_t L = off[i + 1] - off[i];
				if (L < 0 || L > 65535) { q.bad = true; continue; }
				q.seen[L] = 1; q.padded += (L + 15) / 16 * 16;
				if (L > q.mx) q.mx = (int)L;
				if (L < q.mn) q.mn = (int)L;
			}
		});
		for (auto &q : part) {
			bad_len |= q.bad; s.padded_total += q.padded;
			if (q.mx > s.max_len) s.max_len = q.mx;
			if (q.mn < s.min_len) s.min_len = q.mn;
			for (int L = 0; L < 65536; ++L) seen[L] |= q.seen[L];
		}
	}
	if (bad_len) return nabwa_fail(NABWA_EINVAL, "read length outside 0..65535");
	std::vector<int> md_of(s.max_len + 1, opt->max_diff);
	if (opt->fnr > 0.0f) for (int L = 0; L <= s.max_len; ++L) md_of[L] = nabwa_cal_maxdiff(L, 0.02, opt->fnr);
	s.md_tab.assign(s.max_len + 1, 0); s.mg_tab.assign(s.max_len + 1, 0);
	int mdx = 0, mgx = 0;
	for (int L = 0; L <= s.max_len; ++L) {
		if (!seen[L]) continue;
		const int md_sizing = md_of[per_read ? L : s.max_len];
		int g = opt->max_gapo; if (md_sizing < g) g = md_sizing;
		const int d = md_of[L];
		if (d < 0 || d > 126 || g < 0 || g > 255) return nabwa_fail(NABWA_EINVAL, "max_diff > 126 or max_gapo > 255 (unsupported)");
		s.md_tab[L] = (uint8_t)d; s.mg_tab[L] = (uint8_t)g;
		if (d > mdx) mdx = d;
		if (g > mgx) mgx = g;
		const long ns = (long)(md_sizing + 1) * opt->s_mm + (long)(g + 1) * opt->s_gapo + (long)(opt->max_gape + 1) * opt->s_gape;
		if (ns > (long)s.NS) s.NS = (uint32_t)ns;
	}
	{
		const bool gape_counts = opt->mode & NABWA_MODE_GAPE;
		for (int a = 0; a <= mdx + 1; ++a)
			for (int g = 0; g <= mgx; ++g)
				for (int e = 0; e <= (g ? opt->max_gape : 0); ++e) {
					if (a + g + (gape_counts ? e : 0) > mdx + 1) continue;
					const long sc = (long)a * opt->s_mm + (long)g * opt->s_gapo + (long)e * opt->s_gape;
					if (sc + 1 > (long)s.NS1) s.NS1 = (uint32_t)(sc + 1);
				}
		if (s.NS1 > s.NS) s.NS1 = s.NS;
	}
	if (s.NS > 2048 || opt->s_mm < 0 || opt->s_gapo < 0 || opt->s_gape < 0 || opt->max_gape < 0 || opt->max_gape > 255)
		return nabwa_fail(NABWA_EINVAL, "option block needs more than 2048 score levels (the reference's own limit)");
	s.deep_only = mdx > 14 || mgx > 15 || opt->max_gape > 31 || s.NS1 > 64;
	if (opt->seed_len < 0) return nabwa_fail(NABWA_EINVAL, "negative seed_len");
	if (opt->s_mm < 1 || opt->s_gapo < 1 || opt->s_gape < 1) return nabwa_fail(NABWA_EINVAL, "s_mm, s_gapo and s_gape must be >= 1 (-M / -O / -E 0 are not supported)");
	return NABWA_OK;
}

namespace { struct DedupMax { __host__ __device__ uint32_t operator()(uint32_t a, uint32_t c) const { return a > c ? a : c; } }; }

static int dedup_reads(nabwa_batch *b, int bits, PoolBuf<uint8_t> &raw_s, PoolBuf<uint8_t> &raw_r, PoolBuf<int64_t> &raw_off, size_t nb, bool timing)
{
	nabwa_index *ix = b->ix;
	const int n = b->n_given;
	hipStream_t st = b->stream;
	PoolBuf<uint64_t> kA, kB; PoolBuf<uint32_t> vA, vB, head, flag, inner; PoolBuf<int32_t> rep, map; PoolBuf<unsigned int> d_stat;
	PoolBuf<int64_t> coff; PoolBuf<uint8_t> c_s, c_r; PoolBuf<void> d_tmp;
	DevEvent e0, e1;
	StreamDrain drain{ st };
	const size_t n1 = (size_t)n + 1;
	HIP_CHECK(kA.get(ix, n1 * 8)); HIP_CHECK(kB.get(ix, n1 * 8)); HIP_CHECK(vA.get(ix, n1 * 4)); HIP_CHECK(vB.get(ix, n1 * 4));
	HIP_CHECK(head.get(ix, n1 * 4)); HIP_CHECK(rep.get(ix, n1 * 4)); HIP_CHECK(flag.get(ix, n1 * 4)); HIP_CHECK(inner.get(ix, n1 * 4));
	HIP_CHECK(map.get(ix, n1 * 4)); HIP_CHECK(d_stat.get(ix, 8));
	int64_t *const clen = (int64_t*)kA.p;
	size_t tmp_bytes = 16, need = 0;
	hipcub::DoubleBuffer<uint64_t> dk(kA.p, kB.p); hipcub::DoubleBuffer<uint32_t> dv(vA.p, vB.p);
	HIP_CHECK(hipcub::DeviceRadixSort::SortPairs(nullptr, need, dk, dv, n, 0, 64, st)); if (need > tmp_bytes) tmp_bytes = need;
	HIP_CHECK(hipcub::DeviceScan::InclusiveScan(nullptr, need, head.p, head.p, DedupMax(), n, st)); if (need > tmp_bytes) tmp_bytes = need;
	HIP_CHECK(hipcub::DeviceScan::ExclusiveSum(nullptr, need, flag.p, inner.p, n + 1, st)); if (need > tmp_bytes) tmp_bytes = need;
	HIP_CHECK(hipcub::DeviceScan::ExclusiveSum(nullptr, need, clen, clen, n + 1, st)); if (need > tmp_bytes) tmp_bytes = need;
	HIP_CHECK(d_tmp.get(ix, tmp_bytes));
	if (timing) { HIP_CHECK(hipEventCreate(&e0.e)); HIP_CHECK(hipEventCreate(&e1.e)); HIP_CHECK(hipEventRecord(e0, st)); }
	HIP_CHECK(hipMemsetAsync(d_stat, 0, 8, st));
	nabwa_launch_dedup_hash(n, raw_s, raw_r, raw_off, bits >= 64 ? ~0ull : (1ull << bits) - 1ull, kA, vA, st);
	need = tmp_bytes;
	HIP_CHECK(hipcub::DeviceRadixSort::SortPairs(d_tmp.p, need, dk, dv, n, 0, 64, st));
	nabwa_launch_dedup_heads(n, dk.Current(), head, st);
	need = tmp_bytes;
	HIP_CHECK(hipcub::DeviceScan::InclusiveScan(d_tmp.p, need, head.p, head.p, DedupMax(), n, st));
	nabwa_launch_dedup_verify(n, raw_s, raw_r, raw_off, dv.Current(), head, rep, flag, d_stat, st);
	need = tmp_bytes;
	HIP_CHECK(hipcub::DeviceScan::ExclusiveSum(d_tmp.p, need, flag.p, inner.p, n + 1, st));
	nabwa_launch_dedup_map(n, rep, inner, raw_off, map, clen, d_stat, st);
	unsigned int stat[2] = { 0, 0 };
	HIP_CHECK(hipMemcpyAsync(stat, d_stat, 8, hipMemcpyDeviceToHost, st));
	HIP_CHECK(hipStreamSynchronize(st));
	HIP_CHECK(hipGetLastError());
	const int n_u = (int)stat[1];
	if (n_u < 1 || n_u > n) return nabwa_fail(NABWA_EIO, "NABWA_DEDUP: the stage counted more distinct reads than reads, or none");
	b->dedup_coll = stat[0];
	if (n_u < n) {
		HIP_CHECK(coff.get(ix, ((size_t)n_u + 1) * 8)); HIP_CHECK(c_s.get(ix, nb)); HIP_CHECK(c_r.get(ix, nb));
		need = tmp_bytes;
		HIP_CHECK(hipcub::DeviceScan::ExclusiveSum(d_tmp.p, need, clen, coff.p, n_u + 1, st));
		nabwa_launch_dedup_compact(n, raw_s, raw_r, raw_off, rep, inner, coff, c_s, c_r, st);
	}
	if (timing) HIP_CHECK(hipEventRecord(e1, st));
	HIP_CHECK(hipStreamSynchronize(st));
	HIP_CHECK(hipGetLastError());
	if (timing) {
		float ms = 0.f;
		HIP_CHECK(hipEventElapsedTime(&ms, e0, e1));
		fprintf(stderr, "[nabwa] dedup: %d reads given, %d searched, %u hash collisions, stage %.3f ms\n", n, n_u, stat[0], ms);
	}
	if (n_u < n) {
		raw_s = std::move(c_s); raw_r = std::move(c_r); raw_off = std::move(coff);
		b->d_map = std::move(map);
		b->n = n_u;
	}
	return NABWA_OK;
}

static uint64_t option_signature(const nabwa_gap_opt_t *o)
{
	uint32_t fnr; memcpy(&fnr, &o->fnr, 4);
	const uint32_t w[14] = { (uint32_t)o->s_mm, (uint32_t)o->s_gapo, (uint32_t)o->s_gape, (uint32_t)o->mode, (uint32_t)o->indel_end_skip, (uint32_t)o->max_del_occ,
							 (uint32_t)o->max_entries, fnr, (uint32_t)o->max_diff, (uint32_t)o->max_gapo, (uint32_t)o->max_gape, (uint32_t)o->max_seed_diff,
							 (uint32_t)o->seed_len, (uint32_t)o->max_top2 };
	uint64_t h = 0xcbf29ce484222325ULL;
	for (uint32_t x : w) for (int k = 0; k < 4; ++k) { h ^= (x >> (8 * k)) & 0xffu; h *= 0x100000001b3ULL; }
	return h;
}

static int cache_lookup(nabwa_batch *b, const BatchShape &s, PoolBuf<uint8_t> &raw_s, PoolBuf<uint8_t> &raw_r, PoolBuf<int64_t> &raw_off, size_t nb, bool timing)
{
	nabwa_index *ix = b->ix;
	nabwa_dedup_cache *c = b->cache;
	const int n = b->n, max_len = s.max_len;
	hipStream_t st = b->stream;
	std::lock_guard<std::mutex> lk(c->mu);
	if (c->has_sig && c->sig != b->cache_sig) {
		if (c->pins) { ++c->bypasses; b->cache = nullptr; b->cache_bypass = 1; return NABWA_OK; }
		if (int r = nabwa_dcache_reset(ix, c)) return r;
		++c->flushes;
	}
	c->sig = b->cache_sig; c->has_sig = true;
	PoolBuf<uint64_t> hash; PoolBuf<uint32_t> ids, found, flag, inner, cent; PoolBuf<int32_t> rep, newidx, map; PoolBuf<int64_t> clen, coff; PoolBuf<unsigned int> d_stat;
	PoolBuf<uint8_t> d_tab, c_s, c_r; PoolBuf<void> d_tmp;
	DevEvent e0, e1;
	StreamDrain drain{ st };
	const size_t n1 = (size_t)n + 1;
	HIP_CHECK(hash.get(ix, n1 * 8)); HIP_CHECK(ids.get(ix, n1 * 4)); HIP_CHECK(found.get(ix, n1 * 4)); HIP_CHECK(flag.get(ix, n1 * 4)); HIP_CHECK(inner.get(ix, n1 * 4));
	HIP_CHECK(cent.get(ix, n1 * 4)); HIP_CHECK(rep.get(ix, n1 * 4)); HIP_CHECK(newidx.get(ix, n1 * 4)); HIP_CHECK(clen.get(ix, n1 * 8)); HIP_CHECK(d_stat.get(ix, 8));
	HIP_CHECK(d_tab.get(ix, 2 * (size_t)(max_len + 1)));
	size_t tmp_bytes = 16, need = 0;
	HIP_CHECK(hipcub::DeviceScan::ExclusiveSum(nullptr, need, flag.p, inner.p, n + 1, st)); if (need > tmp_bytes) tmp_bytes = need;
	HIP_CHECK(hipcub::DeviceScan::ExclusiveSum(nullptr, need, clen.p, clen.p, n + 1, st)); if (need > tmp_bytes) tmp_bytes = need;
	HIP_CHECK(d_tmp.get(ix, tmp_bytes));
	HIP_CHECK(hipEventCreate(&e0.e)); HIP_CHECK(hipEventCreate(&e1.e)); HIP_CHECK(hipEventRecord(e0, st));
	HIP_CHECK(hipMemcpyAsync(d_tab, s.md_tab.data(), max_len + 1, hipMemcpyHostToDevice, st));
	HIP_CHECK(hipMemcpyAsync(d_tab + max_len + 1, s.mg_tab.data(), max_len + 1, hipMemcpyHostToDevice, st));
	nabwa_launch_dedup_hash(n, raw_s, raw_r, raw_off, ~0ull, hash, ids, st);
	nabwa_launch_dcache_lookup(n, raw_s, raw_r, raw_off, hash, d_tab, d_tab + max_len + 1, c->d_slots, c->n_slots, b->cache_mask, c->d_arena, found, flag, st);
	need = tmp_bytes;
	HIP_CHECK(hipcub::DeviceScan::ExclusiveSum(d_tmp.p, need, flag.p, inner.p, n + 1, st));
	nabwa_launch_dcache_map(n, found, inner, raw_off, rep, newidx, clen, cent, d_stat, st);
	unsigned int n_search = 0;
	HIP_CHECK(hipMemcpyAsync(&n_search, d_stat, 4, hipMemcpyDeviceToHost, st));
	HIP_CHECK(hipStreamSynchronize(st));
	HIP_CHECK(hipGetLastError());
	if ((int)n_search < 0 || (int)n_search > n) return nabwa_fail(NABWA_EIO, "NABWA_DEDUP_CACHE: the lookup counted more reads to search than reads");
	const int n_s = (int)n_search, n_served = n - n_s;
	c->lookups += (uint64_t)n; c->served += (uint64_t)n_served;
	if (n_served) {
		HIP_CHECK(coff.get(ix, ((size_t)n_s + 1) * 8)); HIP_CHECK(c_s.get(ix, nb)); HIP_CHECK(c_r.get(ix, nb)); HIP_CHECK(map.get(ix, (size_t)b->n_given * 4));
		if (n_s) {
			need = tmp_bytes;
			HIP_CHECK(hipcub::DeviceScan::ExclusiveSum(d_tmp.p, need, clen.p, coff.p, n_s + 1, st));
			nabwa_launch_dedup_compact(n, raw_s, raw_r, raw_off, rep, inner, coff, c_s, c_r, st);
		} else HIP_CHECK(hipMemsetAsync(coff, 0, 8, st));
		nabwa_launch_dcache_remap(b->n_given, b->d_map, newidx, map, st);
	}
	HIP_CHECK(hipEventRecord(e1, st));
	HIP_CHECK(hipStreamSynchronize(st));
	HIP_CHECK(hipGetLastError());
	HIP_CHECK(hipEventElapsedTime(&b->cache_lookup_ms, e0, e1));
	if (timing) fprintf(stderr, "[nabwa] dedup cache: %d reads looked up, %d to search, %d served, stage %.3f ms\n", n, n_s, n_served, b->cache_lookup_ms);
	if (n_served) {
		raw_s = std::move(c_s); raw_r = std::move(c_r); raw_off = std::move(coff);
		b->d_map = std::move(map); b->d_cent = std::move(cent);
		b->n = n_s; b->n_served = n_served;
		++c->pins; b->cache_pinned = 1;
	}
	return NABWA_OK;
}

static int upload_reads(nabwa_batch *b, const BatchShape &s, const int64_t *off, const uint8_t *seq, const uint8_t *rseq, bool timing, double tc0, int dedup_bits)
{
	nabwa_index *ix = b->ix;
	const int n_given = b->n_given, max_len = s.max_len;
	const size_t nb = (size_t)off[n_given] > 0 ? (size_t)off[n_given] : 1, pnb = (size_t)s.padded_total + 64;
	if ((uint64_t)pnb >= (1ull << 32)) return nabwa_fail(NABWA_EINVAL, "batch holds 4 Gi padded bases or more: split it (lane state keeps a 32-bit read offset)");
	auto read_buffers = [&](int n) -> int {
		HIP_CHECK(b->d_seq.get(ix, pnb)); HIP_CHECK(b->d_rseq.get(ix, pnb));
		HIP_CHECK(b->d_poff.get(ix, (size_t)(n + 1) * 8)); HIP_CHECK(b->d_len.get(ix, (size_t)(n ? n : 1) * 4));
		HIP_CHECK(b->d_md.get(ix, n ? n : 1)); HIP_CHECK(b->d_mg.get(ix, n ? n : 1)); HIP_CHECK(b->d_key.get(ix, (size_t)(n ? n : 1) * 24));
		b->pack_stride = 2 * ((max_len + 15) / 16 + 2);
		HIP_CHECK(b->d_pack.get(ix, (size_t)(n ? n : 1) * b->pack_stride * 4));
		HIP_CHECK(b->d_cls.get(ix, (size_t)(n ? n : 1) * 2)); HIP_CHECK(b->d_perm.get(ix, (size_t)(n ? n : 1) * 4)); HIP_CHECK(b->d_ncls.get(ix, NCLS_WORDS * sizeof(unsigned int)));
		return NABWA_OK;
	};
	const bool dedup = dedup_bits >= 0 && n_given > 0;
	if (!dedup) if (int r = read_buffers(n_given)) return r;
	if (n_given == 0) { HIP_CHECK(hipMemset(b->d_poff, 0, 8)); return NABWA_OK; }
	PoolBuf<uint8_t> raw_s, raw_r, d_tab; PoolBuf<int64_t> raw_off, plen; PoolBuf<void> d_tmp; size_t tmp_bytes = 0;
	StreamDrain drain{ b->stream };
	HIP_CHECK(raw_s.get(ix, nb)); HIP_CHECK(raw_r.get(ix, nb)); HIP_CHECK(raw_off.get(ix, (size_t)(n_given + 1) * 8));
	const UploadJob jobs[3] = { { raw_s, seq, (size_t)off[n_given] }, { raw_r, rseq, (size_t)off[n_given] }, { raw_off, off, (size_t)(n_given + 1) * 8 } };
	const double tu0 = now_s();
	HIP_CHECK(staged_upload(ix, jobs, 3));
	if (timing) fprintf(stderr, "[nabwa] upload of %.2f GB: %.3f s (%.3f s into batch_create)\n", 2e-9 * (double)off[n_given], now_s() - tu0, tu0 - tc0);
	if (dedup) {
		if (int r = dedup_reads(b, dedup_bits, raw_s, raw_r, raw_off, nb, timing)) return r;
		if (b->cache) if (int r = cache_lookup(b, s, raw_s, raw_r, raw_off, nb, timing)) return r;
		if (int r = read_buffers(b->n)) return r;
	}
	const int n = b->n;
	HIP_CHECK(plen.get(ix, (size_t)(n + 1) * 8));
	nabwa_launch_padded_len(n, raw_off, plen, b->stream);
	HIP_CHECK(hipcub::DeviceScan::ExclusiveSum(nullptr, tmp_bytes, plen.p, b->d_poff.p, n + 1, b->stream));
	HIP_CHECK(d_tmp.get(ix, tmp_bytes ? tmp_bytes : 16));
	HIP_CHECK(hipcub::DeviceScan::ExclusiveSum(d_tmp.p, tmp_bytes, plen.p, b->d_poff.p, n + 1, b->stream));
	HIP_CHECK(d_tab.get(ix, 2 * (size_t)(max_len + 1)));
	HIP_CHECK(hipMemcpyAsync(d_tab, s.md_tab.data(), max_len + 1, hipMemcpyHostToDevice, b->stream));
	HIP_CHECK(hipMemcpyAsync(d_tab + max_len + 1, s.mg_tab.data(), max_len + 1, hipMemcpyHostToDevice, b->stream));
	nabwa_launch_pad_reads(n, raw_s, raw_r, raw_off, b->d_poff, b->d_seq, b->d_rseq, b->d_len, b->d_key,
						   ix->bwt[0].kmer_T == ix->bwt[1].kmer_T ? (int)ix->bwt[0].kmer_T : 0, b->opt.seed_len, b->d_pack, b->pack_stride,
						   d_tab, d_tab + max_len + 1, b->d_md, b->d_mg, b->stream);
	HIP_CHECK(hipStreamSynchronize(b->stream));
	if (timing) fprintf(stderr, "[nabwa] re-layout kernel done %.3f s into batch_create\n", now_s() - tc0);
	HIP_CHECK(raw_s.release()); HIP_CHECK(raw_r.release()); HIP_CHECK(raw_off.release());
	HIP_CHECK(plen.release()); HIP_CHECK(d_tmp.release()); HIP_CHECK(d_tab.release());
	return NABWA_OK;
}

static int working_buffers(nabwa_batch *b, const BatchShape &s)
{
	nabwa_index *ix = b->ix;
	const nabwa_gap_opt_t *opt = &b->opt;
	const int n = b->n, max_len = s.max_len;
	SearchParams &P = b->P;
	memset(&P, 0, sizeof(P));
	P.bwt[0] = ix->bwt[0]; P.bwt[1] = ix->bwt[1];
	{
		uint32_t tab[NABWA_IXTAB_ALL];
		nabwa_ixtab_fill(tab, ix->bwt);
		memcpy(tab + NABWA_IXTAB_WORDS, ix->kmer_pk, sizeof ix->kmer_pk);
		HIP_CHECK(b->d_ixtab.get(ix, sizeof tab));
		HIP_CHECK(hipMemcpy(b->d_ixtab, tab, sizeof tab, hipMemcpyHostToDevice));
		P.ixtab = b->d_ixtab;
	}
	P.seq = b->d_seq; P.rseq = b->d_rseq; P.poff = b->d_poff; P.rd_len = b->d_len; P.rd_maxdiff = b->d_md; P.rd_maxgapo = b->d_mg; P.rd_key = b->d_key; P.rd_pack = b->d_pack; P.pack_stride = b->pack_stride;
	P.text_mode = env_int("NABWA_TEXT_KERNELS", 7) & 7;
	if (env_int("NABWA_W_QUADS", 1)) P.text_mode |= TM_W_QUADS;
	if (ix->bwt[0].kmer_T != ix->bwt[1].kmer_T) P.bwt[0].kmer_T = P.bwt[1].kmer_T = 0;
	P.ids = 0; P.n = n;
	P.s_mm = opt->s_mm; P.s_gapo = opt->s_gapo; P.s_gape = opt->s_gape; P.mode = opt->mode;
	P.indel_end_skip = opt->indel_end_skip; P.max_del_occ = opt->max_del_occ; P.max_entries = opt->max_entries;
	P.max_gape = opt->max_gape; P.max_seed_diff = opt->max_seed_diff; P.seed_len = opt->seed_len; P.max_top2 = opt->max_top2;
	int cap1 = env_int("NABWA_CAP1", 4096);
	if (cap1 < 16) cap1 = 16;
	if (cap1 > 65534) cap1 = 65534;
	layout(P, (uint32_t)cap1, max_len, opt->seed_len, s.deep_only ? 1u : s.NS1);
	P.aln_cap = env_int("NABWA_ALNCAP1", 16);
	P.sync_refill = env_int("NABWA_SYNC_REFILL", 0);
	P.trip_budget = (uint32_t)env_int("NABWA_TRIP_BUDGET", max_len > opt->seed_len ? 2000 : 300);
	P.trip_budget_hard = (uint32_t)env_int("NABWA_TRIP_BUDGET_HARD", max_len > opt->seed_len ? 200 : (int)P.trip_budget);
	if (getenv("NABWA_TRIP_BUDGET") && !getenv("NABWA_TRIP_BUDGET_HARD")) P.trip_budget_hard = P.trip_budget;
	b->class_sort = env_int("NABWA_CLASS_SORT", 1);
	P.sure0 = env_int("NABWA_SURE0", 3);
	if (P.sure0 < 0) P.sure0 = 0;
	if (P.sure0 > 3) P.sure0 = 3;
	if (env_int("NABWA_SURE0_STATS", 0)) {
		HIP_CHECK(b->d_s0stats.get(ix, S0S_WORDS * sizeof(unsigned long long)));
		HIP_CHECK(hipMemset(b->d_s0stats, 0, S0S_WORDS * sizeof(unsigned long long)));
		P.s0_stats = b->d_s0stats;
	}
	{
		P.w_sync = (n > 0 && s.min_len == max_len) ? env_int("NABWA_W_SYNC", 1) : 0;
	}
	if (P.aln_cap < 1) P.aln_cap = 1;

	hipDeviceProp_t prop;
	HIP_CHECK(hipGetDeviceProperties(&prop, ix->device));
	int occ = nabwa_search_occupancy(s.deep_only ? 1 : (int)s.NS1);
	if (occ < 1) occ = 1;
	const int occ_env = env_int("NABWA_BLOCKS_PER_CU", 0);
	if (occ_env > 0) occ = occ_env;
	long blocks = (long)prop.multiProcessorCount * occ;
	const long need = ((long)n + NABWA_SEARCH_BLOCK - 1) / NABWA_SEARCH_BLOCK;
	if (blocks > need) blocks = need;
	if (blocks < 1) blocks = 1;
	b->n_blocks = (int)blocks;
	if (getenv("NABWA_TIMING")) fprintf(stderr, "[nabwa] search kernel: %u score levels, %d blocks per CU (LDS %zu B per block), %ld blocks\n", s.NS1, occ,
										(size_t)s.NS1 * NABWA_SEARCH_BLOCK * 2 + NABWA_SEARCH_BLOCK * 80, blocks);
	HIP_CHECK(b->d_scratch.get(ix, (size_t)blocks * NABWA_SEARCH_BLOCK * P.lane_stride));
	int occw = nabwa_width_occupancy(); if (occw < 1) occw = 1;
	long blocks_w = (long)prop.multiProcessorCount * occw;
	if (blocks_w > 2 * need) blocks_w = 2 * need;
	if (blocks_w < 1) blocks_w = 1;
	b->n_blocks_w = (int)blocks_w;
	HIP_CHECK(b->d_wdata.get(ix, (size_t)(n ? n : 1) * P.wstride));
	HIP_CHECK(b->d_nN.get(ix, n ? n : 1));
	P.wdata = b->d_wdata; P.rd_nN = b->d_nN;
	const size_t n1 = n ? n : 1;
	HIP_CHECK(b->d_naln.get(ix, n1 * 4)); HIP_CHECK(b->d_maxent.get(ix, n1 * 4)); HIP_CHECK(b->d_wide_idx.get(ix, n1 * 4));
	HIP_CHECK(b->d_status.get(ix, n1)); HIP_CHECK(b->d_aln.get(ix, n1 * (size_t)P.aln_cap * 16));
	HIP_CHECK(b->d_counter.get(ix, WC_WORDS * sizeof(unsigned int))); HIP_CHECK(b->d_novf.get(ix, 4)); HIP_CHECK(b->d_ovf_ids.get(ix, n1 * 4));
	HIP_CHECK(b->d_sum.get(ix, TS_WORDS * sizeof(unsigned long long)));
	P.scratch = b->d_scratch; P.n_aln = b->d_naln; P.max_ent = b->d_maxent; P.status = b->d_status; P.aln = b->d_aln;
	P.work_counter = b->d_counter;
	return NABWA_OK;
}

extern "C" int nabwa_batch_create(nabwa_index_t *ix, const nabwa_gap_opt_t *opt, int n, const int64_t *off,
								  const uint8_t *seq, const uint8_t *rseq, int per_read, nabwa_batch_t **out)
{
	if (!ix || !opt || !off || !out || n < 0 || (n && (!seq || !rseq))) return nabwa_fail(NABWA_EINVAL, "null argument");
	HIP_CHECK(hipSetDevice(ix->device));
	const bool timing = getenv("NABWA_TIMING") != 0;
	const double tc0 = now_s();
	int dedup_bits = -1;
	if (const char *e = getenv("NABWA_DEDUP")) {
		if (strcmp(e, "0") && strcmp(e, "1")) return nabwa_fail(NABWA_EINVAL, "NABWA_DEDUP: 0 or 1");
		if (e[0] == '1') {
			dedup_bits = 64;
			if (const char *k = getenv("NABWA_DEDUP_HASH_BITS")) {
				char *end = 0;
				const long v = strtol(k, &end, 10);
				if (end == k || *end || v < 0 || v > 64) return nabwa_fail(NABWA_EINVAL, "NABWA_DEDUP_HASH_BITS: 0..64");
				dedup_bits = (int)v;
			}
		}
	}
	nabwa_dedup_cache *cache = nullptr;
	if (const char *e = getenv("NABWA_DEDUP_CACHE")) {
		char *end = 0;
		const long v = strtol(e, &end, 10);
		if (end == e || *end || v < 0) return nabwa_fail(NABWA_EINVAL, "NABWA_DEDUP_CACHE: a number of MiB, 0 for off");
		if (v > 0 && dedup_bits < 0) return nabwa_fail(NABWA_EINVAL, "NABWA_DEDUP_CACHE needs NABWA_DEDUP=1: the cache sits behind the in-batch stage");
		if (v > 0) if (int r = nabwa_dcache_get(ix, v, &cache)) return r;
	}
	BatchShape s;
	if (int r = derive_options(opt, n, off, per_read, s)) return r;

	const double tc1 = now_s();
	std::unique_ptr<nabwa_batch, void (*)(nabwa_batch*)> b(new nabwa_batch(), nabwa_batch_destroy);
	b->ix = ix; b->opt = *opt; b->n = b->n_given = n; b->dedup_on = dedup_bits >= 0; b->deep_only = s.deep_only ? 1 : 0;
	b->max_len = s.max_len; b->min_len = n ? s.min_len : 0; b->NS1 = s.NS1; b->NS_wide = s.NS; b->deep_coop = -1;
	if (cache) { b->cache = cache; b->cache_on = 1; b->cache_sig = option_signature(opt); b->cache_mask = dedup_bits >= 64 ? ~0ull : (1ull << dedup_bits) - 1ull; }
	if (env_int("NABWA_STREAM_BLOCKING", 0)) HIP_CHECK(hipStreamCreate(&b->stream.s));
	else HIP_CHECK(hipStreamCreateWithFlags(&b->stream.s, hipStreamNonBlocking));
	for (DevEvent *e : { &b->ev0, &b->ev1, &b->evw, &b->evd0, &b->evd1 }) HIP_CHECK(hipEventCreate(&e->e));
	if (int r = upload_reads(b.get(), s, off, seq, rseq, timing, tc0, dedup_bits)) return r;

	const double tc2 = now_s();
	if (int r = working_buffers(b.get(), s)) return r;
	*out = b.release();
	if (timing) fprintf(stderr, "[nabwa] batch_create %d reads: host option derivation %.3f s, read upload + device layout %.3f s, working buffers %.3f s\n", n, tc1 - tc0, tc2 - tc1, now_s() - tc2);
	return NABWA_OK;
}

extern "C" int nabwa_batch_run(nabwa_batch_t *b)
{
	if (!b) return nabwa_fail(NABWA_EINVAL, "null batch");
	HIP_CHECK(hipSetDevice(b->ix->device));
	b->unresolved = 0;
	if (b->n == 0) return NABWA_OK;
	if (b->n_grown) {
		HIP_CHECK(hipStreamSynchronize(b->stream));
		for (int t = 0; t < b->n_grown; ++t) HIP_CHECK(b->grown[t].release());
		b->n_grown = 0; b->grown_used = 0;
	}
	HIP_CHECK(hipMemsetAsync(b->d_counter, 0, WC_WORDS * sizeof(unsigned int), b->stream));
	HIP_CHECK(hipMemsetAsync(b->d_novf, 0, 4, b->stream));
	HIP_CHECK(hipEventRecord(b->evw, b->stream));
	SearchParams PW = b->P; PW.ids = 0; PW.rd_cls = b->class_sort ? b->d_cls : 0;
	nabwa_launch_fm_width(&PW, b->n_blocks_w, b->stream);
	if (b->class_sort) {
		HIP_CHECK(hipMemsetAsync(b->d_ncls, 0, NCLS_WORDS * sizeof(unsigned int), b->stream));
		nabwa_launch_partition(b->n, b->d_cls, b->d_perm, b->d_ncls, b->stream);
	}
	HIP_CHECK(hipEventRecord(b->ev0, b->stream));
	SearchParams PS = b->P; PS.ids = b->class_sort ? b->d_perm : 0; PS.n_sync = b->class_sort ? b->d_ncls + NCLS_FIRST0 : 0;
	PS.rd_cls = b->class_sort ? b->d_cls : 0;
	if (!b->deep_only) nabwa_launch_fm_search(&PS, b->n_blocks, b->stream);
	else {
		HIP_CHECK(hipMemsetAsync(b->d_status, NABWA_ST_OVERFLOW, b->n, b->stream));
		HIP_CHECK(hipMemsetAsync(b->d_naln, 0, (size_t)b->n * 4, b->stream));
	}
	HIP_CHECK(hipEventRecord(b->ev1, b->stream));
	if (b->class_sort && env_int("NABWA_DEEP_ORDER", 1)) nabwa_launch_collect_keyed(b->n, b->d_status, b->d_ovf_ids, b->d_novf, NABWA_ST_OVERFLOW, b->d_cls, b->d_md, 7, b->d_naln, b->P.aln_cap, b->stream);
	else nabwa_launch_collect(b->n, b->d_status, b->d_ovf_ids, b->d_novf, NABWA_ST_OVERFLOW, b->stream);
	HIP_CHECK(hipGetLastError());
	b->ran = 1;
	return NABWA_OK;
}


void rebuild_widths(nabwa_batch *b, const SearchParams &Q, unsigned int cnt, bool after_first_pass)
{
	SearchParams QW = Q; QW.touch_counter = 0; QW.rd_cls = 0; QW.n_sync = 0; QW.w_sync = 0;
	QW.w_skip_clean = after_first_pass && env_int("NABWA_W_SKIP_CLEAN", 1) ? 1 : 0;
	QW.n_aln = b->d_naln; QW.max_ent = b->d_maxent; QW.status = b->d_status; QW.aln = b->d_aln; QW.aln_cap = b->P.aln_cap;
	long bw2 = (2 * (long)cnt + NABWA_SEARCH_BLOCK - 1) / NABWA_SEARCH_BLOCK;
	if (bw2 > b->n_blocks_w) bw2 = b->n_blocks_w;
	(void)hipMemsetAsync(b->d_counter, 0, WC_WORDS * sizeof(unsigned int), b->stream);
	nabwa_launch_fm_width(&QW, (int)bw2, b->stream);
}

int recollect(nabwa_batch *b, int which, unsigned int *left)
{
	HIP_CHECK(hipMemsetAsync(b->d_novf, 0, 4, b->stream));
	nabwa_launch_collect(b->n, b->d_status, b->d_ovf_ids, b->d_novf, which, b->stream);
	HIP_CHECK(hipMemcpyAsync(left, b->d_novf, 4, hipMemcpyDeviceToHost, b->stream));
	HIP_CHECK(hipStreamSynchronize(b->stream));
	return NABWA_OK;
}

static int tier_a_rerun(nabwa_batch *b, unsigned int *cur, bool timing)
{
	const double tt0 = now_s();
	SearchParams Q = b->P;
	layout(Q, 65534u, b->max_len, b->opt.seed_len, b->P.NS);
	long blocks = ((long)*cur + NABWA_SEARCH_BLOCK - 1) / NABWA_SEARCH_BLOCK;
	size_t budget = (size_t)env_int("NABWA_WIDE_GB", 32) << 30;
	const long fit = (long)(budget / ((size_t)NABWA_SEARCH_BLOCK * Q.lane_stride));
	if (blocks > fit) blocks = fit < 1 ? 1 : fit;
	const size_t need = (size_t)blocks * NABWA_SEARCH_BLOCK * Q.lane_stride;
	if (b->scratch2_bytes < need) {
		b->scratch2_bytes = 0;
		HIP_CHECK(b->d_scratch2.release());
		HIP_CHECK(b->d_scratch2.get(b->ix, need));
		b->scratch2_bytes = need;
	}
	Q.scratch = b->d_scratch2; Q.ids = b->d_ovf_ids; Q.n = (int)*cur; Q.n_sync = 0; Q.w_sync = 0;
	rebuild_widths(b, Q, *cur, false);
	HIP_CHECK(hipMemsetAsync(b->d_counter, 0, WC_WORDS * sizeof(unsigned int), b->stream));
	nabwa_launch_fm_search(&Q, (int)blocks, b->stream);
	HIP_CHECK(hipGetLastError());
	unsigned int left = 0;
	if (int r = recollect(b, NABWA_ST_OVERFLOW, &left)) return r;
	if (timing) fprintf(stderr, "[nabwa] first-pass kernel again, arena of 65534 entries: %u reads on %ld blocks, %u left, %.3f s\n", *cur, blocks, left, now_s() - tt0);
	*cur = left;
	return NABWA_OK;
}

static int cache_insert(nabwa_batch *b)
{
	nabwa_dedup_cache *c = b->cache;
	hipStream_t st = b->stream;
	std::lock_guard<std::mutex> lk(c->mu);
	b->cache_inserted = 1;
	if (!c->has_sig) { c->sig = b->cache_sig; c->has_sig = true; }
	if (c->sig != b->cache_sig) { b->n_not_inserted = (uint64_t)b->n; return NABWA_OK; }
	int row_cap = env_int("NABWA_DEDUP_CACHE_ROWS", 1024);
	if (row_cap < b->P.aln_cap) row_cap = b->P.aln_cap;
	unsigned long long c0[DC_WORDS], c1[DC_WORDS];
	DevEvent e0, e1;
	StreamDrain drain{ st };
	HIP_CHECK(hipEventCreate(&e0.e)); HIP_CHECK(hipEventCreate(&e1.e)); HIP_CHECK(hipEventRecord(e0, st));
	HIP_CHECK(hipMemcpyAsync(c0, c->d_ctr, sizeof c0, hipMemcpyDeviceToHost, st));
	nabwa_launch_dcache_insert(b->n, b->d_seq, b->d_rseq, b->d_poff, b->d_len, b->d_md, b->d_mg, b->d_status, b->d_naln, b->d_maxent, b->d_aln, b->P.aln_cap, b->d_wide_idx,
							   b->d_aln2, b->aln_cap2, b->d_grown_tab, row_cap, b->cache_mask, c->d_slots, c->n_slots, c->d_arena, c->arena_bytes, c->d_ctr, st);
	HIP_CHECK(hipMemcpyAsync(c1, c->d_ctr, sizeof c1, hipMemcpyDeviceToHost, st));
	HIP_CHECK(hipEventRecord(e1, st));
	HIP_CHECK(hipStreamSynchronize(st));
	HIP_CHECK(hipGetLastError());
	HIP_CHECK(hipEventElapsedTime(&b->cache_insert_ms, e0, e1));
	c->used = c1[DC_USED]; c->entries = c1[DC_ENTRIES];
	b->n_inserted = c1[DC_ENTRIES] - c0[DC_ENTRIES];
	b->n_not_inserted = (c1[DC_FULL] - c0[DC_FULL]) + (c1[DC_SKIPPED] - c0[DC_SKIPPED]);
	if (getenv("NABWA_TIMING")) fprintf(stderr, "[nabwa] dedup cache: %d reads searched, %llu entered, %llu not (cache full or over %d rows), stage %.3f ms; %llu entries, %llu bytes\n",
										b->n, (unsigned long long)b->n_inserted, (unsigned long long)b->n_not_inserted, row_cap, b->cache_insert_ms, c1[DC_ENTRIES], c1[DC_USED]);
	return NABWA_OK;
}

static int sync_searches(nabwa_batch_t *b, int *n_second_pass);

extern "C" int nabwa_batch_sync(nabwa_batch_t *b, int *n_second_pass)
{
	if (!b) return nabwa_fail(NABWA_EINVAL, "null batch");
	HIP_CHECK(hipSetDevice(b->ix->device));
	if (n_second_pass) *n_second_pass = 0;
	if (b->n == 0) return NABWA_OK;
	if (int r = sync_searches(b, n_second_pass)) return r;
	return b->cache && b->ran && !b->cache_inserted ? cache_insert(b) : NABWA_OK;
}

static int sync_searches(nabwa_batch_t *b, int *n_second_pass)
{
	unsigned int novf = 0;
	HIP_CHECK(hipMemcpyAsync(&novf, b->d_novf, 4, hipMemcpyDeviceToHost, b->stream));
	HIP_CHECK(hipStreamSynchronize(b->stream));
	HIP_CHECK(hipEventElapsedTime(&b->last_ms, b->ev0, b->ev1));
	HIP_CHECK(hipEventElapsedTime(&b->last_ms_w, b->evw, b->ev0));
	if (n_second_pass) *n_second_pass = (int)novf;
	if (novf == 0) return NABWA_OK;
	const bool timing = getenv("NABWA_TIMING") != 0;
	unsigned int cur = novf;
	b->deep_ran = 0; b->last_ms_deep = 0.f;
	if (env_int("NABWA_TIER_A", 0) && b->P.cap < 65534 && b->deep_only == 0)
		if (int r = tier_a_rerun(b, &cur, timing)) return r;
	return cur ? deep_searches(b, cur, timing) : NABWA_OK;
}

extern "C" float nabwa_batch_last_kernel_ms(nabwa_batch_t *b) { return b ? b->last_ms : 0.f; }
extern "C" float nabwa_batch_last_width_ms(nabwa_batch_t *b) { return b ? b->last_ms_w : 0.f; }
extern "C" float nabwa_batch_last_deep_ms(nabwa_batch_t *b) { return b ? b->last_ms_deep : 0.f; }

extern "C" int nabwa_batch_count_touches(nabwa_batch_t *b, uint64_t *n_bucket, uint64_t *n_bucket_width)
{
	if (!b || !n_bucket) return nabwa_fail(NABWA_EINVAL, "null argument");
	HIP_CHECK(hipSetDevice(b->ix->device));
	HIP_CHECK(hipMemsetAsync(b->d_sum, 0, TS_WORDS * sizeof(unsigned long long), b->stream));
	b->P.touch_counter = b->d_sum;
	const uint32_t kt0 = b->P.bwt[0].kmer_T, kt1 = b->P.bwt[1].kmer_T; const int tm0 = b->P.text_mode;
	const char *ts = getenv("NABWA_TRIP_STATS");
	if (!(ts && strcmp(ts, "jump") == 0)) { b->P.bwt[0].kmer_T = b->P.bwt[1].kmer_T = 0; b->P.text_mode = 0; }
	int r = nabwa_batch_run(b);
	if (r == NABWA_OK) r = nabwa_batch_sync(b, 0);
	b->P.touch_counter = 0;
	b->P.bwt[0].kmer_T = kt0; b->P.bwt[1].kmer_T = kt1; b->P.text_mode = tm0;
	if (r != NABWA_OK) return r;
	unsigned long long t[TS_WORDS];
	HIP_CHECK(hipMemcpy(t, b->d_sum, sizeof t, hipMemcpyDeviceToHost));
	*n_bucket = t[TS_TOUCH_S];
	if (n_bucket_width) *n_bucket_width = t[TS_TOUCH_W];
	if (getenv("NABWA_TRIP_STATS") && b->class_sort) {
		unsigned int c[NCLS_WORDS];
		HIP_CHECK(hipMemcpy(c, b->d_ncls, sizeof c, hipMemcpyDeviceToHost));
		fprintf(stderr, "[nabwa] read classes by restarts 0 / 1 / 2+: %u / %u / %u\n", c[NCLS_SIZE + 0], c[NCLS_SIZE + 1], c[NCLS_SIZE + 2]);
	}
	if (getenv("NABWA_TRIP_STATS")) {
		fprintf(stderr, "[nabwa] search kernel: wave-trips %llu; lane-trips: expand %llu exact %llu entry-load %llu spec %llu query %llu two-bucket %llu exited %llu tail-jump %llu text-expand %llu text-tail %llu; longest read %llu trips, %llu reads over 2000 trips, %llu over 500\n",
				t[TS_TRIPS], t[TS_EXPAND], t[TS_EXACT], t[TS_ENT_LOAD], t[TS_SPEC], t[TS_QUERY], t[TS_TWO], t[TS_EXITED], t[TS_JUMP], t[TS_TEXT_EXPAND], t[TS_TEXT_TAIL],
				t[TS_MAX_TRIPS], t[TS_OVER_2000], t[TS_OVER_500]);
		fprintf(stderr, "[nabwa] the %llu reads over 8000 trips: %llu trips = expansions key-form %llu, rows two-bucket %llu, rows one-bucket %llu, text %llu (of all: %llu with gaps); pops %llu, tail steps %llu, jumps %llu\n",
				t[TS_LONG_READS], t[TS_LONG_TRIPS], t[TS_LONG_KF], t[TS_LONG_ROW2], t[TS_LONG_ROW1], t[TS_LONG_TEXT], t[TS_LONG_GAP], t[TS_LONG_POP], t[TS_LONG_TAIL], t[TS_LONG_JUMP]);
	}
	return NABWA_OK;
}

extern "C" int nabwa_batch_width_records(nabwa_batch_t *b, int first, int n, uint32_t *w_out, uint8_t *bid_out, uint8_t *seed_bid_out)
{
	if (!b || first < 0 || n < 0 || first + n > b->n_given || (n && (!w_out || !bid_out))) return nabwa_fail(NABWA_EINVAL, "bad argument");
	if (n == 0) return NABWA_OK;
	HIP_CHECK(hipSetDevice(b->ix->device));
	if (b->n_served) {
		std::vector<int32_t> m((size_t)n);
		HIP_CHECK(hipMemcpyAsync(m.data(), b->d_map + first, (size_t)n * 4, hipMemcpyDeviceToHost, b->stream));
		HIP_CHECK(hipStreamSynchronize(b->stream));
		for (int32_t v : m) if (v < 0) return nabwa_fail(NABWA_EINVAL, "nabwa_batch_width_records: the range holds a read served from the read cache (NABWA_DEDUP_CACHE), which has no width records");
	}
	HIP_CHECK(hipMemsetAsync(b->d_counter, 0, WC_WORDS * sizeof(unsigned int), b->stream));
	SearchParams PW = b->P; PW.ids = 0; PW.rd_cls = 0; PW.touch_counter = 0;
	nabwa_launch_fm_width(&PW, b->n_blocks_w, b->stream);
	HIP_CHECK(hipGetLastError());
	std::vector<int32_t> src(b->d_map ? (size_t)n : 0);
	const size_t rec0 = b->d_map ? 0 : (size_t)first, n_rec = b->d_map ? (size_t)b->n : (size_t)n;
	std::vector<uint8_t> rec(n_rec * b->P.wstride);
	if (b->d_map) HIP_CHECK(hipMemcpyAsync(src.data(), b->d_map + first, (size_t)n * 4, hipMemcpyDeviceToHost, b->stream));
	HIP_CHECK(hipMemcpyAsync(rec.data(), b->d_wdata + rec0 * b->P.wstride, rec.size(), hipMemcpyDeviceToHost, b->stream));
	HIP_CHECK(hipStreamSynchronize(b->stream));
	const int W = b->max_len + 1, SW = b->opt.seed_len + 1;
	for (int i = 0; i < n; ++i) {
		const uint8_t *r = rec.data() + (size_t)(b->d_map ? src[i] : i) * b->P.wstride;
		for (int x = 0; x < 2; ++x) {
			memcpy(w_out + ((size_t)i * 2 + x) * W, (const uint32_t*)r + x * b->P.WL, 4 * (size_t)W);
			memcpy(bid_out + ((size_t)i * 2 + x) * W, r + b->P.woff_bid + x * b->P.WLB, (size_t)W);
			if (seed_bid_out && b->max_len > b->opt.seed_len && SW <= (int)b->P.SLB) memcpy(seed_bid_out + ((size_t)i * 2 + x) * SW, r + b->P.woff_sbid + x * b->P.SLB, (size_t)SW);
		}
	}
	return NABWA_OK;
}

extern "C" int nabwa_batch_checksum(nabwa_batch_t *b, uint64_t *sum, int64_t *n_rows)
{
	if (!b) return nabwa_fail(NABWA_EINVAL, "null batch");
	HIP_CHECK(hipSetDevice(b->ix->device));
	unsigned long long h[CKS_WORDS] = { 0, 0 };
	HIP_CHECK(hipMemsetAsync(b->d_sum, 0, sizeof h, b->stream));
	nabwa_launch_checksum(b->n_given, b->d_map, b->d_cent, b->cache ? b->cache->d_arena : nullptr, b->d_naln, b->d_aln, b->P.aln_cap, b->d_status, b->d_wide_idx, b->d_aln2, b->aln_cap2, b->d_grown_tab,
						  b->d_sum + CKS_SUM, b->d_sum + CKS_ROWS, b->stream);
	HIP_CHECK(hipMemcpyAsync(h, b->d_sum, sizeof h, hipMemcpyDeviceToHost, b->stream));
	HIP_CHECK(hipStreamSynchronize(b->stream));
	if (sum) *sum = h[CKS_SUM];
	if (n_rows) *n_rows = (int64_t)h[CKS_ROWS];
	return NABWA_OK;
}

extern "C" int nabwa_batch_config(nabwa_batch_t *b, nabwa_batch_config_t *out)
{
	if (!b || !out) return nabwa_fail(NABWA_EINVAL, "null argument");
	memset(out, 0, sizeof(*out));
	out->n = b->n_given; out->min_len = b->min_len; out->max_len = b->max_len;
	out->deep_only = b->deep_only; out->ns1 = (int32_t)b->NS1; out->ns_wide = (int32_t)b->NS_wide;
	out->w_sync = b->P.w_sync; out->trip_budget = (int32_t)b->P.trip_budget; out->trip_budget_hard = (int32_t)b->P.trip_budget_hard;
	out->n_sync = out->hard_budget = -1;
	for (int q = 0; q < NCLS_N; ++q) out->cls[q] = -1;
	if (b->ran && b->class_sort) {
		HIP_CHECK(hipSetDevice(b->ix->device));
		unsigned int c[NCLS_WORDS];
		HIP_CHECK(hipMemcpyAsync(c, b->d_ncls, sizeof c, hipMemcpyDeviceToHost, b->stream));
		HIP_CHECK(hipStreamSynchronize(b->stream));
		for (int q = 0; q < NCLS_N; ++q) out->cls[q] = (int32_t)c[NCLS_SIZE + q];
		out->n_sync = (int32_t)c[NCLS_FIRST0];
		if (!b->deep_only) out->hard_budget = b->P.trip_budget_hard && 2u * c[NCLS_FIRST0] > (uint32_t)b->n ? 1 : 0;
	}
	out->coop_lanes = b->deep_coop;
	out->lds_rd = b->deep_cfg ? (int32_t)b->deep_lds_rd : -1;
	return NABWA_OK;
}

static int sure0_read(nabwa_batch_t *b, uint64_t *out, int n_words)
{
	if (!b || !out) return nabwa_fail(NABWA_EINVAL, "null argument");
	for (int q = 0; q < n_words; ++q) out[q] = 0;
	if (!b->d_s0stats) return NABWA_OK;
	HIP_CHECK(hipSetDevice(b->ix->device));
	unsigned long long v[S0S_WORDS];
	HIP_CHECK(hipMemcpyAsync(v, b->d_s0stats, (size_t)n_words * sizeof v[0], hipMemcpyDeviceToHost, b->stream));
	HIP_CHECK(hipStreamSynchronize(b->stream));
	for (int q = 0; q < n_words; ++q) out[q] = v[q];
	return NABWA_OK;
}

extern "C" int nabwa_batch_dedup_stats(nabwa_batch_t *b, uint64_t out[4])
{
	if (!b || !out) return nabwa_fail(NABWA_EINVAL, "null argument");
	out[0] = (uint64_t)b->n_given; out[1] = (uint64_t)b->n; out[2] = b->dedup_coll; out[3] = b->dedup_on ? 1 : 0;
	return NABWA_OK;
}

extern "C" int nabwa_batch_dedup_stats_ex(nabwa_batch_t *b, uint64_t out[8])
{
	if (int r = nabwa_batch_dedup_stats(b, out)) return r;
	out[4] = (uint64_t)b->n_served; out[5] = b->n_inserted; out[6] = b->n_not_inserted; out[7] = b->cache_bypass ? 1 : 0;
	return NABWA_OK;
}

extern "C" int nabwa_batch_sure0_stats(nabwa_batch_t *b, uint64_t out[4]) { return sure0_read(b, out, 4); }
extern "C" int nabwa_batch_sure0_stats_ex(nabwa_batch_t *b, uint64_t out[8]) { return sure0_read(b, out, S0S_WORDS); }

extern "C" int nabwa_batch_fetch(nabwa_batch_t *b, int32_t *n_aln, nabwa_aln1_t *aln_out, int64_t aln_cap, int64_t *n_rows,
								 int32_t *max_entries)
{
	if (!b || !n_aln) return nabwa_fail(NABWA_EINVAL, "null argument");
	HIP_CHECK(hipSetDevice(b->ix->device));
	if (n_rows) *n_rows = 0;
	if (b->n_given == 0) return NABWA_OK;
	PoolBuf<uint32_t> d_off; PoolBuf<void> d_tmp; size_t tmp_bytes = 0; PoolBuf<uint4> d_rows; PoolBuf<int32_t> d_cnt;
	StreamDrain drain{ b->stream };
	const int n = b->n_given;
	const int32_t *naln = b->d_naln, *maxent = b->d_maxent;
	if (b->d_map) {
		HIP_CHECK(d_cnt.get(b->ix, (size_t)n * 8));
		nabwa_launch_dedup_expand(n, b->d_map, b->d_naln, b->d_maxent, b->d_cent, b->cache ? b->cache->d_arena : nullptr, d_cnt, d_cnt + n, b->stream);
		naln = d_cnt; maxent = d_cnt + n;
	}
	HIP_CHECK(d_off.get(b->ix, (size_t)(n + 1) * 4));
	HIP_CHECK(hipcub::DeviceScan::ExclusiveSum(nullptr, tmp_bytes, (const uint32_t*)naln, d_off.p, n, b->stream));
	HIP_CHECK(d_tmp.get(b->ix, tmp_bytes ? tmp_bytes : 16));
	HIP_CHECK(hipcub::DeviceScan::ExclusiveSum(d_tmp.p, tmp_bytes, (const uint32_t*)naln, d_off.p, n, b->stream));
	uint32_t last_off = 0; int32_t last_n = 0;
	HIP_CHECK(hipMemcpyAsync(&last_off, d_off + (n - 1), 4, hipMemcpyDeviceToHost, b->stream));
	HIP_CHECK(hipMemcpyAsync(&last_n, naln + (n - 1), 4, hipMemcpyDeviceToHost, b->stream));
	HIP_CHECK(hipMemcpyAsync(n_aln, naln, (size_t)n * 4, hipMemcpyDeviceToHost, b->stream));
	if (max_entries) HIP_CHECK(hipMemcpyAsync(max_entries, maxent, (size_t)n * 4, hipMemcpyDeviceToHost, b->stream));
	HIP_CHECK(hipStreamSynchronize(b->stream));
	const int64_t total = (int64_t)last_off + last_n;
	if (n_rows) *n_rows = total;
	int rc = NABWA_OK;
	if (total > aln_cap || (total && !aln_out)) rc = nabwa_fail(NABWA_ECAP, "aln_cap too small");
	else if (total) {
		HIP_CHECK(d_rows.get(b->ix, (size_t)total * 16));
		nabwa_launch_gather(n, b->d_map, b->d_cent, b->cache ? b->cache->d_arena : nullptr, b->d_naln, d_off, b->d_aln, b->P.aln_cap, b->d_status, b->d_wide_idx, b->d_aln2, b->aln_cap2, b->d_grown_tab,
							d_rows, b->stream);
		HIP_CHECK(hipMemcpyAsync(aln_out, d_rows, (size_t)total * 16, hipMemcpyDeviceToHost, b->stream));
		HIP_CHECK(hipStreamSynchronize(b->stream));
		HIP_CHECK(d_rows.release());
	}
	HIP_CHECK(d_off.release()); HIP_CHECK(d_tmp.release()); HIP_CHECK(d_cnt.release());
	return rc;
}
```

network-aware-bwa_amd/csrc/nabwa_batch.hpp:

```cpp
#pragma once
#include "launchers.hpp"
#include "dev_pool.hpp"

#pragma GCC visibility push(hidden)

struct nabwa_batch {
	nabwa_index *ix = nullptr;
	nabwa_gap_opt_t opt = {};
	int n = 0;
	int n_given = 0, dedup_on = 0; unsigned int dedup_coll = 0;
	DevStream stream;
	DevEvent ev0, ev1, evw;
	float last_ms = 0.f;
	PoolBuf<uint8_t> d_seq, d_rseq, d_md, d_mg; PoolBuf<int64_t> d_poff; PoolBuf<int32_t> d_len; PoolBuf<uint32_t> d_key, d_pack; int pack_stride = 0;
	PoolBuf<int32_t> d_map;
	nabwa_dedup_cache *cache = nullptr; uint64_t cache_sig = 0, cache_mask = ~0ull;
	int cache_on = 0, cache_bypass = 0, cache_pinned = 0, cache_inserted = 0, n_served = 0;
	uint64_t n_inserted = 0, n_not_inserted = 0; float cache_lookup_ms = 0.f, cache_insert_ms = 0.f;
	PoolBuf<uint32_t> d_cent;
	PoolBuf<unsigned long long> d_s0stats; PoolBuf<uint8_t> d_cls; PoolBuf<int32_t> d_perm; PoolBuf<unsigned int> d_ncls; int max_len = 0;
	SearchParams P = {}; int class_sort = 0; uint32_t NS_wide = 0; int n_blocks = 0, n_blocks_w = 0; PoolBuf<uint8_t> d_scratch, d_wdata, d_nN; float last_ms_w = 0.f;
	PoolBuf<int32_t> d_naln, d_maxent, d_wide_idx; PoolBuf<uint8_t> d_status; PoolBuf<uint4> d_aln;
	PoolBuf<unsigned int> d_counter, d_novf; PoolBuf<int32_t> d_ovf_ids;
	PoolBuf<uint8_t> grown[8]; int n_grown = 0;
	PoolBuf<const uint4*> d_grown_tab; int grown_cap = 0, grown_used = 0;
	int n2 = 0, aln_cap2 = 0; PoolBuf<uint8_t> d_scratch2; size_t scratch2_bytes = 0; PoolBuf<int32_t> d_naln2, d_maxent2; PoolBuf<uint8_t> d_status2; PoolBuf<uint4> d_aln2;
	int unresolved = 0;
	PoolBuf<unsigned long long> d_sum;
	PoolBuf<uint4> d_pages; PoolBuf<uint32_t> d_page_prev, d_deep_own; PoolBuf<uint4> d_deep_stage; PoolBuf<unsigned long long> d_deep_ctr;
	PoolBuf<uint32_t> d_ixtab;
	size_t deep_pages = 0, deep_own_words = 0, deep_stage_ent = 0;
	DevEvent evd0, evd1; float last_ms_deep = 0.f; int deep_ran = 0, deep_only = 0;
	int deep_cfg = 0; uint32_t deep_K = 0, deep_lds_rd = 0, deep_rd_pl = 0; size_t deep_n_pages = 0; uint64_t deep_cap_pages = 0; long deep_waves_max = 0;
	int min_len = 0, ran = 0, deep_coop = 0; uint32_t NS1 = 0;
};

static inline uint32_t align_up(uint32_t x, uint32_t a) { return (x + a - 1) / a * a; }

void rebuild_widths(nabwa_batch *b, const SearchParams &Q, unsigned int cnt, bool after_first_pass);
int recollect(nabwa_batch *b, int which, unsigned int *left);
int deep_searches(nabwa_batch *b, unsigned int cur, bool timing);

#pragma GCC visibility pop
```

network-aware-bwa_amd/csrc/search_slots.hpp:

```cpp
#pragma once

enum {
	WC_SEARCH = 0,
	WC_WIDTH  = 1,
	WC_WORDS  = 4
};

enum {
	NCLS_N       = 3,
	NCLS_SIZE    = 0,
	NCLS_CURSOR  = 5,
	NCLS_FIRST0  = 10,
	NCLS_WORDS   = 16
};

enum {
	TS_TOUCH_S     = 0,
	TS_TOUCH_W     = 1,
	TS_TRIPS       = 2,
	TS_EXPAND      = 3,
	TS_EXACT       = 4,
	TS_ENT_LOAD    = 5,
	TS_SPEC        = 6,
	TS_QUERY       = 7,
	TS_TWO         = 8,
	TS_EXITED      = 9,
	TS_JUMP        = 10,
	TS_TEXT_EXPAND = 11,
	TS_TEXT_TAIL   = 12,
	TS_MAX_TRIPS   = 13,
	TS_OVER_2000   = 14,
	TS_OVER_500    = 15,
	TS_LONG_READS  = 16,
	TS_LONG_TRIPS  = 17,
	TS_LONG_KF     = 18,
	TS_LONG_ROW2   = 19,
	TS_LONG_ROW1   = 20,
	TS_LONG_TEXT   = 21,
	TS_LONG_POP    = 22,
	TS_LONG_TAIL   = 23,
	TS_LONG_JUMP   = 24,
	TS_LONG_GAP    = 25,
	TS_WORDS       = 32
};

enum {
	CKS_SUM   = 0,
	CKS_ROWS  = 1,
	CKS_WORDS = 2
};

enum {
	S0S_READS       = 0,
	S0S_KF_EMPTY    = 1,
	S0S_KF_LANDED   = 2,
	S0S_NET         = 3,
	S0S_LEAPS       = 4,
	S0S_LEAP_LEVELS = 5,
	S0S_WALKED      = 6,
	S0S_WORDS       = 8
};

enum {
	DS_ROUNDS        = 0,
	DS_CHAINS_RUN    = 1,
	DS_CHAINS_DONE   = 2,
	DS_STEPS         = 3,
	DS_CAREFUL       = 4,
	DS_POOL_FAIL     = 5,
	DS_TAIL_RANK     = 6,
	DS_TAIL_TEXT     = 7,
	DS_PAGE_BUMP     = 8,
	DS_FORCED_ROWS   = 9,
	DS_MAX_CLK       = 10,
	DS_MAX_ROUNDS    = 11,
	DS_SUM_CLK       = 12,
	DS_WAVE_CLK      = 13,
	DS_EMU_COOP      = 14,
	DS_EMU_COOP_LEV  = 15,
	DS_PH_POP        = 16,
	DS_PH_CHAIN      = 17,
	DS_PH_TAIL       = 18,
	DS_PH_COMMIT     = 19,
	DS_PH_HIT        = 20,
	DS_TAIL_TURNS    = 21,
	DS_LANE_STEPS    = 22,
	DS_KEY_EXPAND    = 23,
	DS_KEY_TAIL      = 24,
	DS_RECORDS       = 25,
	DS_CHILDREN      = 26,
	DS_PRUNED        = 27,
	DS_EXPAND        = 28,
	DS_TWO           = 29,
	DS_FORCED_KEY    = 30,
	DS_FORCED_ONE    = 31,
	DS_HIST1         = 32,
	DS_HIST1_BINS    = 32,
	DS_HIST2_ROUNDS  = 32,
	DS_HIST2_STEPS   = 64,
	DS_HIST2_BINS    = 7,
	DS_WORDS         = 128
};

enum {
	ES_TOUCH_W    = 8,
	ES_TOUCH_S    = 9,
	ES_KEY_EXPAND = 10,
	ES_KEY_TAIL   = 11,
	ES_FORCED_KEY = 12,
	ES_FORCED_ONE = 13,
	ES_COOP       = 14,
	ES_COOP_LEV   = 15,
	ES_WORDS      = 16
};
```

Baseline: 110.3 million.

## Add variable-length text-run and 8-step k-mer table paths to width kernel

The width kernel gets two template-selected forms, both on by default through environment flags. The first compares packed read bits against the reference text with a count-leading-zeros so a run of exact matches of any length up to 16 is emitted in one trip, not only aligned 16-position blocks. The second resolves up to 8 positions per trip from the k-mer table, using paired quad loads, instead of 4. The aim is fewer wave trips and less divergence per read, at the cost of more registers, a heavier kernel body and possible occupancy loss. An opt-in stats template variant and a host API for reading the counters are also added.

Result: faster. 116.1 million, median of 6 (+5.3%).

```diff
diff --git a/include/nabwa.h b/include/nabwa.h
--- a/include/nabwa.h
+++ b/include/nabwa.h
@@ -85,6 +85,7 @@
 int nabwa_batch_config(nabwa_batch_t *b, nabwa_batch_config_t *out);
 int nabwa_batch_sure0_stats(nabwa_batch_t *b, uint64_t out[4]);
 int nabwa_batch_sure0_stats_ex(nabwa_batch_t *b, uint64_t out[8]);
+int nabwa_batch_w_stats(nabwa_batch_t *b, unsigned long long out[6]);
 int nabwa_batch_dedup_stats(nabwa_batch_t *b, uint64_t out[4]);
 int nabwa_batch_dedup_stats_ex(nabwa_batch_t *b, uint64_t out[8]);
 int nabwa_index_dedup_cache_stats(nabwa_index_t *ix, uint64_t out[8]);
diff --git a/network-aware-bwa_amd/csrc/fm_search.hip b/network-aware-bwa_amd/csrc/fm_search.hip
--- a/network-aware-bwa_amd/csrc/fm_search.hip
+++ b/network-aware-bwa_amd/csrc/fm_search.hip
@@ -39,7 +39,8 @@
 #define NABWA_MIN_WAVES 4
 #endif
 
-template <bool COUNT>
+#define W_FORMS(tm_) (((tm_) / TM_W_RUNS) & 3)
+template <bool COUNT, int WF, bool STATS = false>
 __global__ __launch_bounds__(NABWA_SEARCH_BLOCK, NABWA_W_WAVES) void fm_width_kernel(const SearchParams P)
 {
 	const uint32_t lane = threadIdx.x & 63u;
@@ -58,10 +59,12 @@
 	const bool quads = (P.text_mode & TM_W_QUADS) && P.ixtab;
 	if (threadIdx.x < 2 * NABWA_PK_LEVELS) s_pk[threadIdx.x] = quads ? P.ixtab[NABWA_IXTAB_WORDS + threadIdx.x] : 0xffffffffu;
 	__syncthreads();
+	constexpr bool w_trip8 = (WF & 2) != 0, w_runs = (WF & 1) != 0;
+	uint32_t st_lt[4] = { 0u, 0u, 0u, 0u }, st_pos[2] = { 0u, 0u }, st_tx1 = 0u, st_item = 0u, st_max = 0u, st_wave = 0u;
 	bool nflag = true;
 	auto rekey = [&](int from) {
 		tok = false; tbase = from;
-		if (nflag || from + 4 >= n) return;
+		if (nflag || from + (w_trip8 ? 0 : 4) >= n) return;
 		const int PW = P.pack_stride / 2;
 		const uint32_t *const pk = P.rd_pack + (size_t)rid * P.pack_stride + x * PW;
 		const int q = sbase + from;
@@ -104,6 +107,7 @@
 			}
 		}
 		if (__ballot(!done) == 0ull) break;
+		if (STATS) { ++st_wave; if (run) ++st_item; }
 		auto out_pos = [&](int p, bool last) {
 			uint8_t *const rec = WREC;
 			if (last) ++bid;
@@ -119,8 +123,86 @@
 				blo = bhi = 0;
 			}
 		};
-		bool bulk = run && phase == 0 && tmode && (wi & 15) == 0 && wi + 16 < n && tp >= 16u && pw == 1u;
-		if (bulk) {
+		auto put_bytes = [&](int p, int cnt, uint64_t nlo, uint64_t nhi, bool fin) {
+			uint8_t *const dst = WREC + (phase ? P.woff_sbid + x * P.SLB : P.woff_bid + x * P.WLB) + (p & ~15);
+			const uint32_t o = (uint32_t)p & 15u, s = (o & 7u) << 3;
+			const uint64_t a0 = nlo << s, a1 = nhi << s | (s ? nlo >> (64u - s) : 0ull), a2 = s ? nhi >> (64u - s) : 0ull;
+			const bool up = (o & 8u) != 0u;
+			const uint64_t q0 = blo | (up ? 0ull : a0), q1 = bhi | (up ? a0 : a1), q2 = up ? a1 : a2, q3 = up ? a2 : 0ull;
+			const uint32_t e = o + (uint32_t)cnt;
+			const bool full = e >= 16u;
+			if (full) *(uint4*)dst = make_uint4((uint32_t)q0, (uint32_t)(q0 >> 32), (uint32_t)q1, (uint32_t)(q1 >> 32));
+			blo = full ? q2 : q0; bhi = full ? q3 : q1;
+			if (fin) {
+				if (e & 15u) *(uint4*)(dst + (full ? 16 : 0)) = make_uint4((uint32_t)blo, (uint32_t)(blo >> 32), (uint32_t)bhi, (uint32_t)(bhi >> 32));
+				blo = bhi = 0;
+			}
+		};
+		auto put_widths = [&](int p, int cnt, const auto &w, bool fin) {
+			constexpr int NW = (int)(sizeof(w) / sizeof(w[0])), NC = (NW + 6) / 4;
+			uint32_t *const dst = (uint32_t*)WREC + x * P.WL + (p & ~3);
+			const uint32_t o = (uint32_t)p & 3u;
+			uint32_t s1[NW + 1], c[4 * NC];
+#pragma unroll
+			for (int j = 0; j <= NW; ++j) { const uint32_t a = j < NW ? w[j] : 0u, b = j ? w[j - 1] : 0u; s1[j] = (o & 1u) ? b : a; }
+#pragma unroll
+			for (int j = 0; j < 4 * NC; ++j) { const uint32_t a = j <= NW ? s1[j] : 0u, b = (j >= 2 && j - 2 <= NW) ? s1[j - 2] : 0u; c[j] = (o & 2u) ? b : a; }
+			c[0] = o > 0u ? wacc.x : c[0]; c[1] = o > 1u ? wacc.y : c[1]; c[2] = o > 2u ? wacc.z : c[2];
+			const uint32_t e = o + (uint32_t)cnt;
+#pragma unroll
+			for (int j = 0; j < NC; ++j)
+				if (4u * j + 4u <= e || (fin && 4u * j < e)) *(uint4*)(dst + 4 * j) = make_uint4(c[4 * j], c[4 * j + 1], c[4 * j + 2], c[4 * j + 3]);
+			uint4 r = make_uint4(c[0], c[1], c[2], c[3]);
+#pragma unroll
+			for (int j = 1; j < NC; ++j) if ((e >> 2) == (uint32_t)j) r = make_uint4(c[4 * j], c[4 * j + 1], c[4 * j + 2], c[4 * j + 3]);
+			wacc = r;
+		};
+		auto put_ones = [&](int p, int cnt, int term, bool fin) {
+			uint32_t *const dst = (uint32_t*)WREC + x * P.WL + (p & ~3);
+			const uint32_t o = (uint32_t)p & 3u, e = o + (uint32_t)cnt;
+			const int t = term - (p & ~3);
+			uint4 c0 = make_uint4(t == 0 ? 0u : 1u, t == 1 ? 0u : 1u, t == 2 ? 0u : 1u, t == 3 ? 0u : 1u);
+			c0.x = o > 0u ? wacc.x : c0.x; c0.y = o > 1u ? wacc.y : c0.y; c0.z = o > 2u ? wacc.z : c0.z;
+			if (4u <= e || fin) *(uint4*)dst = c0;
+#pragma unroll
+			for (int j = 1; j < 5; ++j)
+				if (4u * j + 4u <= e || (fin && 4u * j < e))
+					*(uint4*)(dst + 4 * j) = make_uint4(t == 4 * j ? 0u : 1u, t == 4 * j + 1 ? 0u : 1u, t == 4 * j + 2 ? 0u : 1u, t == 4 * j + 3 ? 0u : 1u);
+			wacc = e < 4u ? c0 : make_uint4(1u, 1u, 1u, 1u);
+		};
+		bool bulk = !w_runs && run && phase == 0 && tmode && (wi & 15) == 0 && wi + 16 < n && tp >= 16u && pw == 1u;
+		if constexpr (w_runs) if (run && tmode && !nflag && pw == 1u && tp > 0u) {
+			const uint32_t *const pk = P.rd_pack + (size_t)rid * P.pack_stride + x * (P.pack_stride / 2);
+			const int q = sbase + wi;
+			const uint32_t r0 = pk[q >> 4], r1 = pk[(q >> 4) + 1], sh = ((uint32_t)q & 15u) << 1;
+			const uint32_t rd = sh ? (r0 << sh) | (r1 >> (32u - sh)) : r0;
+			const uint32_t b0 = tp >= 16u ? tp - 16u : 0u, ts = (b0 & 15u) << 1;
+			const uint32_t *const txt = BX(text);
+			const uint32_t t0 = txt[b0 >> 4], t1 = ts ? txt[(b0 >> 4) + 1u] : 0u;
+			uint32_t tx = (uint32_t)(((uint64_t)t1 << 32 | t0) >> ts);
+			if (tp < 16u) tx <<= (16u - tp) << 1;
+			const uint32_t df = tx ^ rd, same = df ? (uint32_t)__clz((int)df) >> 1 : 16u;
+			const uint32_t left = (uint32_t)(n - wi);
+			uint32_t kmax = min(min(16u, left), tp);
+			if (left == 16u) kmax = min(kmax, 15u);
+			const uint32_t r = min(same, kmax);
+			if (r) {
+				const bool fin = r == left;
+				const uint64_t b8 = (uint64_t)((uint32_t)(bid > 127 ? 127 : bid) | 128u) * 0x0101010101010101ull;
+				const uint64_t mlo = r >= 8u ? ~0ull : (1ull << (r << 3)) - 1ull, mhi = r <= 8u ? 0ull : (r >= 16u ? ~0ull : (1ull << ((r - 8u) << 3)) - 1ull);
+				uint64_t nlo = b8 & mlo, nhi = b8 & mhi;
+				if (fin) {
+					++bid;
+					const uint64_t tb = (uint64_t)(bid > 127 ? 127 : bid);
+					if (r < 8u) nlo |= tb << (r << 3); else nhi |= tb << ((r - 8u) << 3);
+				}
+				if (phase == 0) put_ones(wi, (int)r + (fin ? 1 : 0), fin ? n : -1, fin);
+				put_bytes(wi, (int)r + (fin ? 1 : 0), nlo, nhi, fin);
+				if (STATS) { ++st_lt[0]; st_pos[0] += r; if (phase) ++st_tx1; }
+				tp -= r; wi += (int)r; bulk = true;
+			}
+		}
+		if constexpr (!w_runs) if (bulk) {
 			if ((wi >> 4) != stag) { const uint4 q = *(const uint4*)((x ? P.rseq : P.seq) + sq_off + wi); WIN_SET(slo, shi, q.x, q.y, q.z, q.w); stag = wi >> 4; }
 			const uint32_t w0 = (tp - 16u) >> 4;
 			const uint32_t *const txt = BX(text);
@@ -142,11 +224,74 @@
 				for (int u = 0; u < 4; ++u) *(uint4*)(wp + 4 * u) = make_uint4(1u, 1u, 1u, 1u);
 				const uint32_t b4 = ((uint32_t)(bid > 127 ? 127 : bid) | 128u) * 0x01010101u;
 				*(uint4*)(rec + P.woff_bid + x * P.WLB + wi) = make_uint4(b4, b4, b4, b4);
+				if (STATS) { ++st_lt[0]; st_pos[0] += 16u; if (phase) ++st_tx1; }
 				tp -= 16u; wi += 16;
 			}
 		}
 		if (bulk) {  }
-		else if (run && tok && wi - tbase + 4 <= LW && wi + 4 < n) {
+		else if (w_trip8 && run && tok && wi - tbase < LW) {
+			const int t1 = wi - tbase + 1, m = min(min(8, LW - (wi - tbase)), n - wi);
+			const uint2 *const lo = BX(kmer_lo);
+			uint2 tv[8];
+#pragma unroll
+			for (int u = 0; u < 8; ++u) tv[u] = make_uint2(1u, 0u);
+			if (quads) {
+				uint4 qd[4][2];
+#pragma unroll
+				for (int h = 0; h < 4; ++h) {
+					const int t = t1 + 2 * h;
+					qd[h][0] = qd[h][1] = make_uint4(1u, 0u, 1u, 0u);
+					if (2 * h + 1 < m) {
+						const uint4 *const p = (const uint4*)(lo + LVO(t + 1) + 4 * (size_t)(wkey >> (2 * (KT - t))));
+						qd[h][0] = p[0]; qd[h][1] = p[1];
+					} else if (2 * h < m) {
+						const uint2 v = (lo + LVO(t))[wkey >> (2 * (KT - t))];
+						qd[h][0].x = v.x; qd[h][0].y = v.y;
+					}
+				}
+#pragma unroll
+				for (int h = 0; h < 4; ++h) {
+					const int t = t1 + 2 * h;
+					if (2 * h + 1 < m) {
+						const uint32_t ch = wkey >> (2 * (KT - t - 1)), c = ch & 3u;
+						const uint4 a = qd[h][0], b = qd[h][1];
+						const uint32_t sum = (a.y - a.x) + (a.w - a.z) + (b.y - b.x) + (b.w - b.z) + 4u + ((ch >> 2) == s_pk[x * NABWA_PK_LEVELS + t] ? 1u : 0u);
+						tv[2 * h] = make_uint2(1u, sum);
+						tv[2 * h + 1] = c == 0u ? make_uint2(a.x, a.y) : (c == 1u ? make_uint2(a.z, a.w) : (c == 2u ? make_uint2(b.x, b.y) : make_uint2(b.z, b.w)));
+					} else tv[2 * h] = make_uint2(qd[h][0].x, qd[h][0].y);
+				}
+			} else {
+#pragma unroll
+				for (int u = 0; u < 8; ++u)
+					if (u < m) { const int t = t1 + u; tv[u] = (lo + LVO(t))[wkey >> (2 * (KT - t))]; }
+			}
+			const uint32_t full1 = BX(seq_len) + 1u, bb = (uint32_t)(bid > 127 ? 127 : bid), bb1 = (uint32_t)(bid + 1 > 127 ? 127 : bid + 1);
+			uint32_t wv[9], pv = pw, nk = kk, nl = ll; uint64_t nlo = 0ull; int cnt = 0; bool alive = true, died = false;
+#pragma unroll
+			for (int u = 0; u < 8; ++u) {
+				const bool act = alive && u < m, dead = tv[u].x > tv[u].y;
+				const uint32_t w = dead ? full1 : tv[u].y - tv[u].x + 1u;
+				const uint32_t by = (dead ? bb1 : bb) | ((wi + u > 0 && w == pv) ? 128u : 0u);
+				wv[u] = act ? w : 0u;
+				if (act) { nlo |= (uint64_t)by << (8 * u); pv = w; nk = tv[u].x; nl = tv[u].y; ++cnt; died = dead; }
+				alive = act && !dead;
+			}
+			wv[8] = 0u;
+			const int p0 = wi;
+			if (STATS) { ++st_lt[1]; st_pos[1] += (uint32_t)cnt; }
+			wi += cnt; pw = pv;
+			if (died) { kk = 0; ll = BX(seq_len); ++bid; rekey(wi); } else { kk = nk; ll = nl; }
+			const bool fin = wi == n;
+			uint64_t nhi = 0ull;
+			if (fin) {
+				++bid;
+				const uint64_t tb = (uint64_t)(bid > 127 ? 127 : bid);
+				if (cnt < 8) nlo |= tb << (8 * cnt); else nhi = tb;
+			}
+			if (phase == 0) put_widths(p0, cnt + (fin ? 1 : 0), wv, fin);
+			put_bytes(p0, cnt + (fin ? 1 : 0), nlo, nhi, fin);
+		}
+		else if (!w_trip8 && run && tok && wi - tbase + 4 <= LW && wi + 4 < n) {
 			uint2 tv[4];
 			const uint2 *const lo = BX(kmer_lo);
 			const int t1 = wi - tbase + 1;
@@ -181,8 +326,10 @@
 				if (dead) { kk = 0; ll = BX(seq_len); ++bid; }
 				out_pos(wi, false);
 				++wi;
+				if (STATS) ++st_pos[1];
 				if (dead) { rekey(wi); break; }
 			}
+			if (STATS) ++st_lt[1];
 		} else if (run) {
 			const int pos = sbase + wi;
 			if ((pos >> 4) != stag) { const uint4 q = *(const uint4*)((x ? P.rseq : P.seq) + sq_off + (pos & ~15)); WIN_SET(slo, shi, q.x, q.y, q.z, q.w); stag = pos >> 4; }
@@ -191,6 +338,7 @@
 #pragma unroll
 			for (int u = 0; u < 4; ++u) { qa[u] = make_uint4(0, 0, 0, 0); qb[u] = make_uint4(0, 0, 0, 0); }
 			const bool q = cc < 4 && !tmode;
+			if (STATS) { if (q) ++st_lt[2]; else ++st_lt[3]; }
 			if (q) {
 				const uint32_t primary = BX(primary), kq = kk - 1u, lq = ll;
 				const uint32_t kp = kq - (kq >= primary ? 1u : 0u), lp = lq - (lq >= primary ? 1u : 0u);
@@ -243,15 +391,31 @@
 			out_pos(wi, false);
 			if (wi + 1 == n) out_pos(wi + 1, true);
 			++wi;
-			if (wi == n) {
-				if (phase == 0 && P.rd_cls) P.rd_cls[2 * (size_t)rid + x] = (uint8_t)(bid - 1 > 4 ? 4 : bid - 1);
-				if (phase == 0 && len > P.seed_len) {
-					phase = 1; wi = 0; n = P.seed_len; sbase = len - P.seed_len; tmode = false;
-					if (KT) { wkey = P.rd_key[6 * (size_t)rid + 4 + x]; tok = wkey != 0xffffffffu; }
-					tbase = 0;
-					kk = 0; ll = BX(seq_len); bid = 0; pw = 0;
-				} else { if (x == 0u) P.rd_nN[rid] = (uint8_t)(nN > 255 ? 255 : nN); run = false; }
-			}
+		}
+		if (run && wi == n) {
+			if (phase == 0 && P.rd_cls) P.rd_cls[2 * (size_t)rid + x] = (uint8_t)(bid - 1 > 4 ? 4 : bid - 1);
+			if (phase == 0 && len > P.seed_len) {
+				phase = 1; wi = 0; n = P.seed_len; sbase = len - P.seed_len; tmode = false;
+				if (KT) { wkey = P.rd_key[6 * (size_t)rid + 4 + x]; tok = wkey != 0xffffffffu; }
+				tbase = 0;
+				kk = 0; ll = BX(seq_len); bid = 0; pw = 0;
+			} else {
+				if (x == 0u) P.rd_nN[rid] = (uint8_t)(nN > 255 ? 255 : nN); run = false;
+				if (STATS) { st_max = max(st_max, st_item); st_item = 0u; }
+			}
+		}
+	}
+	if (STATS && P.touch_counter) {
+		unsigned long long v[4] = { (unsigned long long)st_lt[0] << 32 | st_pos[0], (unsigned long long)st_lt[1] << 32 | st_pos[1],
+									(unsigned long long)st_tx1 << 32 | st_lt[2], (unsigned long long)st_lt[3] };
+		for (int o = 32; o > 0; o >>= 1) {
+#pragma unroll
+			for (int u = 0; u < 4; ++u) v[u] += __shfl_down(v[u], o);
+			st_max = max(st_max, (uint32_t)__shfl_down((int)st_max, o));
+		}
+		if (lane == 0) {
+			atomicAdd(P.touch_counter + TS_W_TRIPS, (unsigned long long)st_wave); atomicMax(P.touch_counter + TS_W_MAX, (unsigned long long)st_max);
+			atomicAdd(P.touch_counter + TS_W_TEXT, v[0]); atomicAdd(P.touch_counter + TS_W_TABLE, v[1]); atomicAdd(P.touch_counter + TS_W_RANK, v[2]); atomicAdd(P.touch_counter + TS_W_STEP, v[3]);
 		}
 	}
 	if (COUNT) {
@@ -932,16 +1096,30 @@
 #undef REC
 #undef MD_READ
 #undef MG_READ
+template <bool COUNT, bool STATS = false, typename F> static auto with_width_kernel(int text_mode, F f)
+{
+	switch (W_FORMS(text_mode)) {
+	case 1: return f(fm_width_kernel<COUNT, 1, STATS>);
+	case 2: return f(fm_width_kernel<COUNT, 2, STATS>);
+	case 3: return f(fm_width_kernel<COUNT, 3, STATS>);
+	default: return f(fm_width_kernel<COUNT, 0, STATS>);
+	}
+}
+
 extern "C" void nabwa_launch_fm_width(const SearchParams *P, int n_blocks, hipStream_t s)
 {
-	if (P->touch_counter) hipLaunchKernelGGL((fm_width_kernel<true>), dim3(n_blocks), dim3(NABWA_SEARCH_BLOCK), 0, s, *P);
-	else hipLaunchKernelGGL((fm_width_kernel<false>), dim3(n_blocks), dim3(NABWA_SEARCH_BLOCK), 0, s, *P);
+	auto go = [&](auto k) { hipLaunchKernelGGL(k, dim3(n_blocks), dim3(NABWA_SEARCH_BLOCK), 0, s, *P); return 0; };
+	if ((P->text_mode & TM_W_STATS) && P->touch_counter) with_width_kernel<false, true>(P->text_mode, go);
+	else if (P->touch_counter) with_width_kernel<true>(P->text_mode, go);
+	else with_width_kernel<false>(P->text_mode, go);
 }
 
-extern "C" int nabwa_width_occupancy(void)
+extern "C" int nabwa_width_occupancy(int text_mode)
 {
-	int nb = 0;
-	return hipOccupancyMaxActiveBlocksPerMultiprocessor(&nb, fm_width_kernel<false>, NABWA_SEARCH_BLOCK, 0) == hipSuccess ? nb : 0;
+	return with_width_kernel<false>(text_mode, [](auto k) {
+		int nb = 0;
+		return hipOccupancyMaxActiveBlocksPerMultiprocessor(&nb, k, NABWA_SEARCH_BLOCK, 0) == hipSuccess ? nb : 0;
+	});
 }
 
 extern "C" void nabwa_launch_fm_search(const SearchParams *P, int n_blocks, hipStream_t s)
diff --git a/network-aware-bwa_amd/csrc/fm_search.hpp b/network-aware-bwa_amd/csrc/fm_search.hpp
--- a/network-aware-bwa_amd/csrc/fm_search.hpp
+++ b/network-aware-bwa_amd/csrc/fm_search.hpp
@@ -12,6 +12,9 @@
 #define NABWA_ST_GROWN     5
 
 #define TM_W_QUADS 8
+#define TM_W_RUNS 16
+#define TM_W_TRIP8 32
+#define TM_W_STATS 64
 
 struct SearchParams {
 	DevBwt bwt[2];
diff --git a/network-aware-bwa_amd/csrc/launchers.hpp b/network-aware-bwa_amd/csrc/launchers.hpp
--- a/network-aware-bwa_amd/csrc/launchers.hpp
+++ b/network-aware-bwa_amd/csrc/launchers.hpp
@@ -12,7 +12,7 @@
 void nabwa_launch_occ4(const DevBwt *B, int n, const uint32_t *k, uint32_t *out, hipStream_t s);
 void nabwa_launch_fm_search(const SearchParams *P, int n_blocks, hipStream_t s);
 void nabwa_launch_fm_width(const SearchParams *P, int n_blocks, hipStream_t s);
-int nabwa_width_occupancy(void);
+int nabwa_width_occupancy(int text_mode);
 int nabwa_search_occupancy(int ns);
 void nabwa_launch_checksum(int n, const int32_t *map, const uint32_t *cent, const uint8_t *arena, const int32_t *n_aln, const uint4 *aln, int aln_cap, const uint8_t *status,
 						   const int32_t *wide_idx, const uint4 *aln2, int aln_cap2, const uint4 *const *grown,
diff --git a/network-aware-bwa_amd/csrc/nabwa_batch.hip b/network-aware-bwa_amd/csrc/nabwa_batch.hip
--- a/network-aware-bwa_amd/csrc/nabwa_batch.hip
+++ b/network-aware-bwa_amd/csrc/nabwa_batch.hip
@@ -309,6 +309,8 @@
 	P.seq = b->d_seq; P.rseq = b->d_rseq; P.poff = b->d_poff; P.rd_len = b->d_len; P.rd_maxdiff = b->d_md; P.rd_maxgapo = b->d_mg; P.rd_key = b->d_key; P.rd_pack = b->d_pack; P.pack_stride = b->pack_stride;
 	P.text_mode = env_int("NABWA_TEXT_KERNELS", 7) & 7;
 	if (env_int("NABWA_W_QUADS", 1)) P.text_mode |= TM_W_QUADS;
+	if (env_int("NABWA_W_RUNS", 1)) P.text_mode |= TM_W_RUNS;
+	if (env_int("NABWA_W_TRIP8", 1)) P.text_mode |= TM_W_TRIP8;
 	if (ix->bwt[0].kmer_T != ix->bwt[1].kmer_T) P.bwt[0].kmer_T = P.bwt[1].kmer_T = 0;
 	P.ids = 0; P.n = n;
 	P.s_mm = opt->s_mm; P.s_gapo = opt->s_gapo; P.s_gape = opt->s_gape; P.mode = opt->mode;
@@ -351,7 +353,7 @@
 	if (getenv("NABWA_TIMING")) fprintf(stderr, "[nabwa] search kernel: %u score levels, %d blocks per CU (LDS %zu B per block), %ld blocks\n", s.NS1, occ,
 										(size_t)s.NS1 * NABWA_SEARCH_BLOCK * 2 + NABWA_SEARCH_BLOCK * 80, blocks);
 	HIP_CHECK(b->d_scratch.get(ix, (size_t)blocks * NABWA_SEARCH_BLOCK * P.lane_stride));
-	int occw = nabwa_width_occupancy(); if (occw < 1) occw = 1;
+	int occw = nabwa_width_occupancy(P.text_mode); if (occw < 1) occw = 1;
 	long blocks_w = (long)prop.multiProcessorCount * occw;
 	if (blocks_w > 2 * need) blocks_w = 2 * need;
 	if (blocks_w < 1) blocks_w = 1;
@@ -417,6 +419,31 @@
 	return NABWA_OK;
 }
 
+static int w_stats_arm(nabwa_batch *b, SearchParams &PW)
+{
+	if (!env_int("NABWA_W_STATS", 0) || PW.touch_counter) return NABWA_OK;
+	HIP_CHECK(hipMemsetAsync(b->d_sum + TS_W_TRIPS, 0, 6 * sizeof(unsigned long long), b->stream));
+	PW.touch_counter = b->d_sum; PW.text_mode |= TM_W_STATS; b->w_stats_armed = 1;
+	return NABWA_OK;
+}
+static int w_stats_collect(nabwa_batch *b)
+{
+	if (!b->w_stats_armed) return NABWA_OK;
+	b->w_stats_armed = 0;
+	unsigned long long *t = b->w_stats;
+	HIP_CHECK(hipMemcpy(t, b->d_sum + TS_W_TRIPS, 6 * sizeof(unsigned long long), hipMemcpyDeviceToHost));
+	const unsigned long long lo = 0xffffffffull;
+	fprintf(stderr, "[nabwa] width kernel: wave-trips %llu; lane-trips / positions: text %llu / %llu (in seed passes: %llu trips), table %llu / %llu, step with a rank query %llu, step without %llu; longest item %llu trips\n",
+			t[0], t[2] >> 32, t[2] & lo, t[4] >> 32, t[3] >> 32, t[3] & lo, t[4] & lo, t[5], t[1]);
+	return NABWA_OK;
+}
+extern "C" int nabwa_batch_w_stats(nabwa_batch_t *b, unsigned long long *out)
+{
+	if (!b || !out) return nabwa_fail(NABWA_EINVAL, "bad argument");
+	memcpy(out, b->w_stats, sizeof b->w_stats);
+	return NABWA_OK;
+}
+
 extern "C" int nabwa_batch_run(nabwa_batch_t *b)
 {
 	if (!b) return nabwa_fail(NABWA_EINVAL, "null batch");
@@ -432,6 +459,7 @@
 	HIP_CHECK(hipMemsetAsync(b->d_novf, 0, 4, b->stream));
 	HIP_CHECK(hipEventRecord(b->evw, b->stream));
 	SearchParams PW = b->P; PW.ids = 0; PW.rd_cls = b->class_sort ? b->d_cls : 0;
+	if (int r = w_stats_arm(b, PW)) return r;
 	nabwa_launch_fm_width(&PW, b->n_blocks_w, b->stream);
 	if (b->class_sort) {
 		HIP_CHECK(hipMemsetAsync(b->d_ncls, 0, NCLS_WORDS * sizeof(unsigned int), b->stream));
@@ -549,6 +577,7 @@
 	unsigned int novf = 0;
 	HIP_CHECK(hipMemcpyAsync(&novf, b->d_novf, 4, hipMemcpyDeviceToHost, b->stream));
 	HIP_CHECK(hipStreamSynchronize(b->stream));
+	if (int r = w_stats_collect(b)) return r;
 	HIP_CHECK(hipEventElapsedTime(&b->last_ms, b->ev0, b->ev1));
 	HIP_CHECK(hipEventElapsedTime(&b->last_ms_w, b->evw, b->ev0));
 	if (n_second_pass) *n_second_pass = (int)novf;
@@ -611,6 +640,7 @@
 	}
 	HIP_CHECK(hipMemsetAsync(b->d_counter, 0, WC_WORDS * sizeof(unsigned int), b->stream));
 	SearchParams PW = b->P; PW.ids = 0; PW.rd_cls = 0; PW.touch_counter = 0;
+	if (int r = w_stats_arm(b, PW)) return r;
 	nabwa_launch_fm_width(&PW, b->n_blocks_w, b->stream);
 	HIP_CHECK(hipGetLastError());
 	std::vector<int32_t> src(b->d_map ? (size_t)n : 0);
@@ -619,6 +649,7 @@
 	if (b->d_map) HIP_CHECK(hipMemcpyAsync(src.data(), b->d_map + first, (size_t)n * 4, hipMemcpyDeviceToHost, b->stream));
 	HIP_CHECK(hipMemcpyAsync(rec.data(), b->d_wdata + rec0 * b->P.wstride, rec.size(), hipMemcpyDeviceToHost, b->stream));
 	HIP_CHECK(hipStreamSynchronize(b->stream));
+	if (int r = w_stats_collect(b)) return r;
 	const int W = b->max_len + 1, SW = b->opt.seed_len + 1;
 	for (int i = 0; i < n; ++i) {
 		const uint8_t *r = rec.data() + (size_t)(b->d_map ? src[i] : i) * b->P.wstride;
diff --git a/network-aware-bwa_amd/csrc/nabwa_batch.hpp b/network-aware-bwa_amd/csrc/nabwa_batch.hpp
--- a/network-aware-bwa_amd/csrc/nabwa_batch.hpp
+++ b/network-aware-bwa_amd/csrc/nabwa_batch.hpp
@@ -26,6 +26,7 @@
 	PoolBuf<const uint4*> d_grown_tab; int grown_cap = 0, grown_used = 0;
 	int n2 = 0, aln_cap2 = 0; PoolBuf<uint8_t> d_scratch2; size_t scratch2_bytes = 0; PoolBuf<int32_t> d_naln2, d_maxent2; PoolBuf<uint8_t> d_status2; PoolBuf<uint4> d_aln2;
 	int unresolved = 0;
+	int w_stats_armed = 0; unsigned long long w_stats[6] = { 0, 0, 0, 0, 0, 0 };
 	PoolBuf<unsigned long long> d_sum;
 	PoolBuf<uint4> d_pages; PoolBuf<uint32_t> d_page_prev, d_deep_own; PoolBuf<uint4> d_deep_stage; PoolBuf<unsigned long long> d_deep_ctr;
 	PoolBuf<uint32_t> d_ixtab;
diff --git a/network-aware-bwa_amd/csrc/search_slots.hpp b/network-aware-bwa_amd/csrc/search_slots.hpp
--- a/network-aware-bwa_amd/csrc/search_slots.hpp
+++ b/network-aware-bwa_amd/csrc/search_slots.hpp
@@ -41,6 +41,12 @@
 	TS_LONG_TAIL   = 23,
 	TS_LONG_JUMP   = 24,
 	TS_LONG_GAP    = 25,
+	TS_W_TRIPS     = 26,
+	TS_W_MAX       = 27,
+	TS_W_TEXT      = 28,
+	TS_W_TABLE     = 29,
+	TS_W_RANK      = 30,
+	TS_W_STEP      = 31,
 	TS_WORDS       = 32
 };
 
```
